# mountaindust/Parasitoids

Hardware: AMD Instinct MI355X
Metric: grid-days/sec on 4096^2 fp64 domain (higher is better)
Workload: dtype f64; 1 GPU; C3 synthetic stack: N=4097 (nominal 4096^2), 30 Gaussian day kernels K=2049, reference torus P=5121, FFT size 5184 (fast mode), prob model, one replica stack per GPU; dom_len=4097, ndays=30, P=5121, fft_len=5184, kernels_direct=False, full_column_pipeline=True

## Files before the change

### include/parasitoid_hip.h

```cpp
#ifndef PARASITOID_HIP_H
#define PARASITOID_HIP_H
#include <stdint.h>

#ifdef __cplusplus
extern "C" {
#endif

#define PS_OK 0
#define PS_ERR_NO_DEVICE (-1)
#define PS_ERR_OOM (-2)
#define PS_ERR_BAD_SHAPE (-3)
#define PS_ERR_BAD_ARG (-4)
#define PS_ERR_UNSUPPORTED (-5)
#define PS_ERR_HIP (-6)
#define PS_ERR_HPROB_BOUNDS (-7)
#define PS_ERR_PMF_NEGATIVE (-8)
#define PS_ERR_FLIGHT_PROB (-9)
#define PS_ERR_STATE (-10)
#define PS_ERR_EMPTY (-11)

#define PS_MODE_EXACT 0
#define PS_MODE_FAST 1
#define PS_MODE_FOLD 2
#define PS_MODE_AUTO 3

typedef struct ps_solver ps_solver;
typedef struct ps_model ps_model;

typedef struct ps_day_stats {
  int64_t nnz;
  double sum;
  double delta;
  double padmax;
  int32_t flag;
  int32_t pad_;
} ps_day_stats;

int ps_version(void);
int ps_device_count(void);
const char* ps_last_error(void);
int ps_device_info(int device, char* name, int n, int* cus, int64_t* hbm_bytes);


int ps_solver_create(ps_solver** out, int device, int dom_len, int max_shape, int mode);
int ps_fast_size(int dom_len, int max_shape);
int ps_solver_retarget(ps_solver* s, int max_shape);
int ps_solver_destroy(ps_solver* s);
int ps_solver_info(ps_solver* s, int* dom_len, int* P, int* Pfft, int* H);
int ps_solver_sync(ps_solver* s);
int ps_solver_set_option(ps_solver* s, const char* key, double value);
int ps_solver_get_option(ps_solver* s, const char* key, double* value);
int ps_solver_kernels_direct(ps_solver* s);
int ps_solver_pipeline(ps_solver* s);
int ps_solver_auto_info(ps_solver* s, int* first_fold_day, int* fold_fft);
int ps_solver_auto_route(ps_solver* s, int first, int count, int32_t* owner);

int ps_solver_set_state_coo(ps_solver* s, const int32_t* row, const int32_t* col,
                            const double* val, int64_t nnz);

int ps_solver_fftconv2_coo(ps_solver* s, const int32_t* row, const int32_t* col,
                           const double* val, int64_t nnz, int kshape);

int ps_solver_get_cursol(ps_solver* s, double negval, double stat_scale, int renorm,
                         ps_day_stats* stats);

int ps_solver_back_solve(ps_solver* s, int nfilt, const int64_t* off, const int32_t* row,
                         const int32_t* col, const double* val, double negval,
                         double stat_scale, ps_day_stats* stats);


int ps_chain_set_kernels(ps_solver* s, int nk, const int64_t* off, const int32_t* kshape,
                         const int32_t* row, const int32_t* col, const double* val);
int ps_chain_run(ps_solver* s, int first, int count, double negval, double stat_scale,
                 int renorm);
int ps_chain_stats(ps_solver* s, int first, int count, ps_day_stats* out);

int ps_chain_run_release(ps_solver* s, int first, int count, double negval, int nfilt, int nuse,
                         const double* weights, int* certified);

int ps_chain_block_prefix(ps_solver* s, int first, int count, const void** total_dev, int64_t* total_bytes);
int ps_chain_block_finish(ps_solver* s, int first, int count, int nprev, const void* const* prev_totals,
                          double negval, double stat_scale, int renorm, int* flagged);
int ps_device_copy(void* dst, const void* src, int64_t bytes);

#define PS_REC_CHAIN 0
#define PS_REC_BACK 1
#define PS_REC_STATE 2
#define PS_REC_WSUM 3
int ps_record_stats(ps_solver* s, int kind, int idx, double negval, double stat_scale,
                    int renorm, ps_day_stats* out);
int ps_record_fetch_coo(ps_solver* s, int kind, int idx, double negval, double stat_scale,
                        double delta, double post_scale, int32_t* row, int32_t* col,
                        double* val, int64_t cap, int64_t* nnz_out);
int ps_record_fetch_csr(ps_solver* s, int kind, int idx, double negval, double stat_scale,
                        double delta, double post_scale, int32_t* indptr ,
                        int32_t* indices, double* data, int64_t cap, int64_t* nnz_out);
int ps_record_fetch_dense(ps_solver* s, int kind, int idx, double* out );
int ps_record_gather(ps_solver* s, int kind, int idx, int64_t n, const int32_t* rows,
                     const int32_t* cols, double scale, double negval, double* out);
int ps_record_gather_multi(ps_solver* s, int nrec, const int32_t* kind, const int32_t* idx, int64_t n,
                           const int32_t* rows, const int32_t* cols, double scale, double negval,
                           double* out);
int ps_weighted_sum(ps_solver* s, int n, const int32_t* kind, const int32_t* idx,
                    const double* w);

#define PS_PROF_NCLS 16
int ps_prof_enable(ps_solver* s, int on);
int ps_prof_read(ps_solver* s, int ncls, double* total_ms, int64_t* count);
int ps_prof_read_days(ps_solver* s, int ncls, int64_t* days);
int ps_prof_read_launches(ps_solver* s, int ncls, int64_t* launches);
int ps_prof_read_owner(ps_solver* s, int owner, int ncls, double* total_ms, int64_t* count, int64_t* launches,
                       int64_t* days);
int ps_solver_owner_fft(ps_solver* s, int owner);

int ps_solver_get_spectrum(ps_solver* s, double* out );
int ps_solver_set_spectrum(ps_solver* s, const double* in );

int ps_model_create(ps_model** out, int device);
int ps_model_destroy(ps_model* m);
int ps_model_set_option(ps_model* m, const char* key, double value);
int ps_model_set_wind(ps_model* m, const double* wind, const int32_t* day_keys, int ndays_wind,
                      int T, int test_run);
int ps_model_prob_mass(ps_model* m, int nd, const int32_t* day_idx, const double* start_time,
                       const double* hparams, const double* Dparams, const double* Dlparams,
                       double mu_r, int n_periods, double rad_dist, int rad_res,
                       int32_t* kshape, int64_t* nnz, int32_t* warned, int32_t* status);
int ps_model_fetch_coo(ps_model* m, int i, int32_t* row, int32_t* col, double* val, int64_t cap);
int ps_model_fetch_debug(ps_model* m, int i, double* hprob, int32_t* Hs, double* loss,
                         double* pmfsum);
int ps_model_hflight(ps_model* m, int day_i, const double* hparams, double* out);
int ps_model_mvn_cdf_values(ps_model* m, double cell, double mu_x, double mu_y, double sig_x,
                            double sig_y, double rho, int32_t* H, double* out, int64_t cap);
int ps_chain_set_kernels_from_model(ps_solver* s, ps_model* m, int first, int count);
int ps_solver_set_state_from_model(ps_solver* s, ps_model* m, int i);

int ps_model_export_device(ps_model* m, int first, int count, void* row_dev, void* col_dev, void* val_dev,
                           int64_t cap);
int ps_chain_set_kernels_device(ps_solver* s, int nk, const int64_t* off, const int32_t* kshape,
                                const void* row_dev, const void* col_dev, const void* val_dev);
int ps_solver_set_state_device(ps_solver* s, const void* row_dev, const void* col_dev, const void* val_dev,
                               int64_t nnz, int kshape);

typedef struct ps_summary ps_summary;
int ps_summary_create(int device, int N, int nslot, int nthr, const double* thr, ps_summary** out);
int ps_summary_add(ps_summary* a, ps_solver* s, int nslot, const int32_t* kind, const int32_t* idx,
                   const double* stat_scale, const double* post_scale, const int32_t* use_delta,
                   double negval, uint32_t weight);
int ps_summary_merge(ps_summary* dst, ps_summary* src);
int ps_summary_info(ps_summary* a, double* total_weight, int64_t* members);
int ps_summary_fetch(ps_summary* a, int slot, int what, double* out );
int ps_summary_reset(ps_summary* a);
int ps_summary_prof(ps_summary* a, int enable, double* total_ms, int64_t* launches);
void ps_summary_destroy(ps_summary* a);

typedef struct ps_linspread ps_linspread;
int ps_linspread_create(int device, int N, int nslot, int nparam, int nthr, const double* thr, ps_linspread** out);
int ps_linspread_set_center(ps_linspread* h, ps_solver* s, int nslot, const int32_t* kind, const int32_t* idx,
                            const double* stat_scale, const double* post_scale, const int32_t* use_delta,
                            double negval);
int ps_linspread_add(ps_linspread* h, ps_solver* s, int param, double coef, int nslot, const int32_t* kind,
                     const int32_t* idx, const double* stat_scale, const double* post_scale,
                     const int32_t* use_delta, double negval);
int ps_linspread_finalize(ps_linspread* h, int nparam, int rank, const double* F);
int ps_linspread_fetch(ps_linspread* h, int slot, int what, double* out );
int ps_linspread_info(ps_linspread* h, int* centered, int* finalized, int64_t* adds);
int ps_linspread_reset(ps_linspread* h);
int ps_linspread_prof(ps_linspread* h, int enable, double* add_ms, int64_t* add_launches, double* fin_ms,
                      int64_t* fin_launches);
void ps_linspread_destroy(ps_linspread* h);

typedef struct ps_hist ps_hist;
int ps_hist_create(int device, int N, int nslot, int nedge, const double* edges, ps_hist** out);
int ps_hist_add(ps_hist* h, ps_solver* s, int nslot, const int32_t* kind, const int32_t* idx,
                const double* stat_scale, const double* post_scale, const int32_t* use_delta, double negval,
                uint32_t weight);
int ps_hist_merge(ps_hist* dst, ps_hist* src);
int ps_hist_info(ps_hist* h, double* total_weight, int64_t* members, int* nedge);
int ps_hist_quantile(ps_hist* h, int slot, double p, double* value, double* lower, double* upper);
int ps_hist_exceed(ps_hist* h, int slot, int k, double* out );
int ps_hist_fetch_counts(ps_hist* h, int slot, int b, uint32_t* out );
int ps_hist_reset(ps_hist* h);
int ps_hist_prof(ps_hist* h, int enable, double* add_ms, int64_t* add_launches, double* q_ms,
                 int64_t* q_launches);
void ps_hist_destroy(ps_hist* h);

typedef struct ps_arrival ps_arrival;
int ps_arrival_create(int device, int N, int nslot, int nthr, const double* thr, ps_arrival** out);
int ps_arrival_add(ps_arrival* a, ps_solver* s, int nslot, const int32_t* kind, const int32_t* idx,
                   const double* stat_scale, const double* post_scale, const int32_t* use_delta, double negval,
                   uint32_t weight);
int ps_arrival_merge(ps_arrival* dst, ps_arrival* src);
int ps_arrival_info(ps_arrival* a, double* total_weight, int64_t* members);
int ps_arrival_prob(ps_arrival* a, int k, int slot, double* out );
int ps_arrival_quantile(ps_arrival* a, int k, double p, int32_t* out );
int ps_arrival_fetch_counts(ps_arrival* a, int k, int slot, uint32_t* out );
int ps_arrival_fetch_reached(ps_arrival* a, int64_t first, int64_t count, uint32_t* cells, uint32_t* weights);
int ps_arrival_reset(ps_arrival* a);
int ps_arrival_prof(ps_arrival* a, int enable, double* add_ms, int64_t* adds, double* map_ms, int64_t* maps);
void ps_arrival_destroy(ps_arrival* a);

#ifdef __cplusplus
}
#endif
#endif
```

### parasitoids_amd/_lib.py

```python
import ctypes as C
import os

import numpy as np

_HERE = os.path.dirname(os.path.abspath(__file__))
LIB_PATH = os.path.join(_HERE, 'libparasitoid_hip.so')

PS_OK = 0
PS_ERR_NO_DEVICE = -1
PS_ERR_OOM = -2
PS_ERR_BAD_SHAPE = -3
PS_ERR_BAD_ARG = -4
PS_ERR_UNSUPPORTED = -5
PS_ERR_HIP = -6
PS_ERR_HPROB_BOUNDS = -7
PS_ERR_PMF_NEGATIVE = -8
PS_ERR_FLIGHT_PROB = -9
PS_ERR_STATE = -10
PS_ERR_EMPTY = -11

MODE_EXACT = 0
MODE_FAST = 1
MODE_FOLD = 2
MODE_AUTO = 3

REC_CHAIN, REC_BACK, REC_STATE, REC_WSUM = 0, 1, 2, 3


class DayStats(C.Structure):
    _fields_ = [('nnz', C.c_int64), ('sum', C.c_double), ('delta', C.c_double),
                ('padmax', C.c_double), ('flag', C.c_int32), ('pad_', C.c_int32)]


class HipError(RuntimeError):
    def __init__(self, code, msg):
        super().__init__('libparasitoid_hip error %d: %s' % (code, msg))
        self.code = code


_I32P = C.POINTER(C.c_int32)
_I64P = C.POINTER(C.c_int64)
_F64P = C.POINTER(C.c_double)
_VP = C.c_void_p

SIGNATURES = {
    'ps_version': (C.c_int, []),
    'ps_device_count': (C.c_int, []),
    'ps_last_error': (C.c_char_p, []),
    'ps_device_info': (C.c_int, [C.c_int, C.c_char_p, C.c_int, _I32P, _I64P]),
    'ps_solver_create': (C.c_int, [C.POINTER(_VP), C.c_int, C.c_int, C.c_int, C.c_int]),
    'ps_solver_destroy': (C.c_int, [_VP]),
    'ps_solver_info': (C.c_int, [_VP, _I32P, _I32P, _I32P, _I32P]),
    'ps_solver_sync': (C.c_int, [_VP]),
    'ps_solver_set_option': (C.c_int, [_VP, C.c_char_p, C.c_double]),
    'ps_solver_get_option': (C.c_int, [_VP, C.c_char_p, _F64P]),
    'ps_solver_set_state_coo': (C.c_int, [_VP, _I32P, _I32P, _F64P, C.c_int64]),
    'ps_solver_fftconv2_coo': (C.c_int, [_VP, _I32P, _I32P, _F64P, C.c_int64, C.c_int]),
    'ps_solver_get_cursol': (C.c_int, [_VP, C.c_double, C.c_double, C.c_int, C.POINTER(DayStats)]),
    'ps_solver_back_solve': (C.c_int, [_VP, C.c_int, _I64P, _I32P, _I32P, _F64P, C.c_double,
                                       C.c_double, C.POINTER(DayStats)]),
    'ps_chain_set_kernels': (C.c_int, [_VP, C.c_int, _I64P, _I32P, _I32P, _I32P, _F64P]),
    'ps_chain_run': (C.c_int, [_VP, C.c_int, C.c_int, C.c_double, C.c_double, C.c_int]),
    'ps_chain_stats': (C.c_int, [_VP, C.c_int, C.c_int, C.POINTER(DayStats)]),
    'ps_chain_run_release': (C.c_int, [_VP, C.c_int, C.c_int, C.c_double, C.c_int, C.c_int, _F64P,
                                       C.POINTER(C.c_int)]),
    'ps_record_stats': (C.c_int, [_VP, C.c_int, C.c_int, C.c_double, C.c_double, C.c_int,
                                  C.POINTER(DayStats)]),
    'ps_solver_retarget': (C.c_int, [_VP, C.c_int]),
    'ps_fast_size': (C.c_int, [C.c_int, C.c_int]),
    'ps_solver_kernels_direct': (C.c_int, [_VP]),
    'ps_solver_pipeline': (C.c_int, [_VP]),
    'ps_solver_auto_info': (C.c_int, [_VP, _I32P, _I32P]),
    'ps_solver_auto_route': (C.c_int, [_VP, C.c_int, C.c_int, _I32P]),
    'ps_record_fetch_coo': (C.c_int, [_VP, C.c_int, C.c_int, C.c_double, C.c_double, C.c_double,
                                      C.c_double, _I32P, _I32P, _F64P, C.c_int64, _I64P]),
    'ps_record_fetch_csr': (C.c_int, [_VP, C.c_int, C.c_int, C.c_double, C.c_double, C.c_double,
                                      C.c_double, _I32P, _I32P, _F64P, C.c_int64, _I64P]),
    'ps_record_fetch_dense': (C.c_int, [_VP, C.c_int, C.c_int, _F64P]),
    'ps_record_gather': (C.c_int, [_VP, C.c_int, C.c_int, C.c_int64, _I32P, _I32P, C.c_double,
                                   C.c_double, _F64P]),
    'ps_record_gather_multi': (C.c_int, [_VP, C.c_int, _I32P, _I32P, C.c_int64, _I32P, _I32P, C.c_double,
                                          C.c_double, _F64P]),
    'ps_weighted_sum': (C.c_int, [_VP, C.c_int, _I32P, _I32P, _F64P]),
    'ps_prof_enable': (C.c_int, [_VP, C.c_int]),
    'ps_prof_read': (C.c_int, [_VP, C.c_int, _F64P, _I64P]),
    'ps_prof_read_days': (C.c_int, [_VP, C.c_int, _I64P]),
    'ps_prof_read_launches': (C.c_int, [_VP, C.c_int, _I64P]),
    'ps_chain_block_prefix': (C.c_int, [_VP, C.c_int, C.c_int, C.POINTER(C.c_void_p), C.POINTER(C.c_int64)]),
    'ps_chain_block_finish': (C.c_int, [_VP, C.c_int, C.c_int, C.c_int, C.POINTER(C.c_void_p), C.c_double, C.c_double,
                                        C.c_int, C.POINTER(C.c_int)]),
    'ps_device_copy': (C.c_int, [C.c_void_p, C.c_void_p, C.c_int64]),
    'ps_prof_read_owner': (C.c_int, [_VP, C.c_int, C.c_int, _F64P, _I64P, _I64P, _I64P]),
    'ps_solver_owner_fft': (C.c_int, [_VP, C.c_int]),
    'ps_solver_get_spectrum': (C.c_int, [_VP, _F64P]),
    'ps_solver_set_spectrum': (C.c_int, [_VP, _F64P]),
    'ps_model_create': (C.c_int, [C.POINTER(_VP), C.c_int]),
    'ps_model_destroy': (C.c_int, [_VP]),
    'ps_model_set_option': (C.c_int, [_VP, C.c_char_p, C.c_double]),
    'ps_model_set_wind': (C.c_int, [_VP, _F64P, _I32P, C.c_int, C.c_int, C.c_int]),
    'ps_model_prob_mass': (C.c_int, [_VP, C.c_int, _I32P, _F64P, _F64P, _F64P, _F64P, C.c_double,
                                     C.c_int, C.c_double, C.c_int, _I32P, _I64P, _I32P, _I32P]),
    'ps_model_fetch_coo': (C.c_int, [_VP, C.c_int, _I32P, _I32P, _F64P, C.c_int64]),
    'ps_model_fetch_debug': (C.c_int, [_VP, C.c_int, _F64P, _I32P, _F64P, _F64P]),
    'ps_model_hflight': (C.c_int, [_VP, C.c_int, _F64P, _F64P]),
    'ps_model_mvn_cdf_values': (C.c_int, [_VP, C.c_double, C.c_double, C.c_double, C.c_double,
                                          C.c_double, C.c_double, _I32P, _F64P, C.c_int64]),
    'ps_chain_set_kernels_from_model': (C.c_int, [_VP, _VP, C.c_int, C.c_int]),
    'ps_solver_set_state_from_model': (C.c_int, [_VP, _VP, C.c_int]),
    'ps_model_export_device': (C.c_int, [_VP, C.c_int, C.c_int, _VP, _VP, _VP, C.c_int64]),
    'ps_chain_set_kernels_device': (C.c_int, [_VP, C.c_int, _I64P, _I32P, _VP, _VP, _VP]),
    'ps_solver_set_state_device': (C.c_int, [_VP, _VP, _VP, _VP, C.c_int64, C.c_int]),
    'ps_summary_create': (C.c_int, [C.c_int, C.c_int, C.c_int, C.c_int, _F64P, C.POINTER(_VP)]),
    'ps_summary_add': (C.c_int, [_VP, _VP, C.c_int, _I32P, _I32P, _F64P, _F64P, _I32P, C.c_double,
                                 C.c_uint32]),
    'ps_summary_merge': (C.c_int, [_VP, _VP]),
    'ps_summary_info': (C.c_int, [_VP, _F64P, _I64P]),
    'ps_summary_fetch': (C.c_int, [_VP, C.c_int, C.c_int, _F64P]),
    'ps_summary_reset': (C.c_int, [_VP]),
    'ps_summary_prof': (C.c_int, [_VP, C.c_int, _F64P, _I64P]),
    'ps_summary_destroy': (None, [_VP]),
    'ps_linspread_create': (C.c_int, [C.c_int, C.c_int, C.c_int, C.c_int, C.c_int, _F64P, C.POINTER(_VP)]),
    'ps_linspread_set_center': (C.c_int, [_VP, _VP, C.c_int, _I32P, _I32P, _F64P, _F64P, _I32P, C.c_double]),
    'ps_linspread_add': (C.c_int, [_VP, _VP, C.c_int, C.c_double, C.c_int, _I32P, _I32P, _F64P, _F64P, _I32P,
                                   C.c_double]),
    'ps_linspread_finalize': (C.c_int, [_VP, C.c_int, C.c_int, _F64P]),
    'ps_linspread_fetch': (C.c_int, [_VP, C.c_int, C.c_int, _F64P]),
    'ps_linspread_info': (C.c_int, [_VP, _I32P, _I32P, _I64P]),
    'ps_linspread_reset': (C.c_int, [_VP]),
    'ps_linspread_prof': (C.c_int, [_VP, C.c_int, _F64P, _I64P, _F64P, _I64P]),
    'ps_linspread_destroy': (None, [_VP]),
    'ps_hist_create': (C.c_int, [C.c_int, C.c_int, C.c_int, C.c_int, _F64P, C.POINTER(_VP)]),
    'ps_hist_add': (C.c_int, [_VP, _VP, C.c_int, _I32P, _I32P, _F64P, _F64P, _I32P, C.c_double, C.c_uint32]),
    'ps_hist_merge': (C.c_int, [_VP, _VP]),
    'ps_hist_info': (C.c_int, [_VP, _F64P, _I64P, _I32P]),
    'ps_hist_quantile': (C.c_int, [_VP, C.c_int, C.c_double, _F64P, _F64P, _F64P]),
    'ps_hist_exceed': (C.c_int, [_VP, C.c_int, C.c_int, _F64P]),
    'ps_hist_fetch_counts': (C.c_int, [_VP, C.c_int, C.c_int, C.POINTER(C.c_uint32)]),
    'ps_hist_reset': (C.c_int, [_VP]),
    'ps_hist_prof': (C.c_int, [_VP, C.c_int, _F64P, _I64P, _F64P, _I64P]),
    'ps_hist_destroy': (None, [_VP]),
    'ps_arrival_create': (C.c_int, [C.c_int, C.c_int, C.c_int, C.c_int, _F64P, C.POINTER(_VP)]),
    'ps_arrival_add': (C.c_int, [_VP, _VP, C.c_int, _I32P, _I32P, _F64P, _F64P, _I32P, C.c_double, C.c_uint32]),
    'ps_arrival_merge': (C.c_int, [_VP, _VP]),
    'ps_arrival_info': (C.c_int, [_VP, _F64P, _I64P]),
    'ps_arrival_prob': (C.c_int, [_VP, C.c_int, C.c_int, _F64P]),
    'ps_arrival_quantile': (C.c_int, [_VP, C.c_int, C.c_double, _I32P]),
    'ps_arrival_fetch_counts': (C.c_int, [_VP, C.c_int, C.c_int, C.POINTER(C.c_uint32)]),
    'ps_arrival_fetch_reached': (C.c_int, [_VP, C.c_int64, C.c_int64, C.POINTER(C.c_uint32),
                                           C.POINTER(C.c_uint32)]),
    'ps_arrival_reset': (C.c_int, [_VP]),
    'ps_arrival_prof': (C.c_int, [_VP, C.c_int, _F64P, _I64P, _F64P, _I64P]),
    'ps_arrival_destroy': (None, [_VP]),
}

_lib = None


def load():
    global _lib
    if _lib is not None:
        return _lib
    if not os.path.exists(LIB_PATH):
        raise ImportError(
            'libparasitoid_hip.so not found at %s; build it with '
            '`python -c "import __graft_entry__ as g; g.build()"` or '
            '`make -C parasitoids_amd/csrc`' % LIB_PATH)
    try:
        lib = C.CDLL(LIB_PATH)
    except OSError as e:
        raise ImportError('cannot load %s: %s' % (LIB_PATH, e))
    for name, (res, args) in SIGNATURES.items():
        fn = getattr(lib, name)
        fn.restype = res
        fn.argtypes = args
    _lib = lib
    return lib


def check(rc):
    if rc != PS_OK:
        msg = load().ps_last_error()
        raise HipError(rc, msg.decode() if msg else '')


def require_device():
    lib = load()
    n = lib.ps_device_count()
    if n <= 0:
        msg = lib.ps_last_error()
        raise ImportError('no MI355X/HIP device available: %s' % (msg.decode() if msg else ''))
    return n


def default_device():
    return int(os.environ.get('PARASITOID_DEVICE', os.environ.get('LOCAL_RANK', '0')))


def i32(a):
    return np.ascontiguousarray(a, dtype=np.int32)


def f64(a):
    return np.ascontiguousarray(a, dtype=np.float64)


def p_i32(a):
    return a.ctypes.data_as(_I32P)


def p_i64(a):
    return a.ctypes.data_as(_I64P)


def p_f64(a):
    return a.ctypes.data_as(_F64P)
```

### parasitoids_amd/csrc/chain_kernels.h

```cpp
#pragma once
#include <hip/hip_runtime.h>
#include <stdint.h>

static __global__ void k_scatter_coo(const int* __restrict__ row, const int* __restrict__ col,
                              const double* __restrict__ val, int64_t nnz, double* dst, int ld,
                              int roff, int coff) {
  for (int64_t i = blockIdx.x * (int64_t)blockDim.x + threadIdx.x; i < nnz;
       i += (int64_t)gridDim.x * blockDim.x)
    atomicAdd(&dst[(int64_t)(row[i] + roff) * ld + col[i] + coff], val[i]);
}

static __global__ void k_zero_band(double* dst, int K, int r0, int r1) {
  double* base = dst + (int64_t)blockIdx.y * K * K + (int64_t)r0 * K;
  const int64_t n = (int64_t)(r1 - r0 + 1) * K;
  for (int64_t i = blockIdx.x * (int64_t)blockDim.x + threadIdx.x; i < n; i += (int64_t)gridDim.x * blockDim.x)
    base[i] = 0.0;
}

static __global__ void k_scatter_coo_batch(const int* __restrict__ row, const int* __restrict__ col,
                                           const double* __restrict__ val, const long long* __restrict__ koff,
                                           const int* __restrict__ kshape, int first, double* dst, int K) {
  const int d = first + blockIdx.y;
  const long long lo = koff[d], hi = koff[d + 1];
  const int off = K / 2 - kshape[d] / 2;
  double* out = dst + (int64_t)blockIdx.y * K * K;
  for (long long i = lo + blockIdx.x * (long long)blockDim.x + threadIdx.x; i < hi;
       i += (long long)gridDim.x * blockDim.x)
    atomicAdd(&out[(int64_t)(row[i] + off) * K + col[i] + off], val[i]);
}

struct DayStats {
  long long nnz;
  double sum;
  double delta;
  double padmax;
  int flag;
  int pad_;
};

static __global__ void k_day_finalize(const double* rowsum_, const long long* rowcnt_,
                               const unsigned long long* padmax_, int N, int renorm,
                               DayStats* out_) {
  const double* rowsum = rowsum_ + (int64_t)blockIdx.x * N;
  const long long* rowcnt = rowcnt_ + (int64_t)blockIdx.x * N;
  const unsigned long long* padmax = padmax_ + blockIdx.x;
  DayStats* out = out_ + blockIdx.x;
  __shared__ double ssum[256];
  __shared__ long long scnt[256];
  double s = 0.0;
  long long c = 0;
  for (int r = threadIdx.x; r < N; r += blockDim.x) {
    s += rowsum[r];
    c += rowcnt[r];
  }
  ssum[threadIdx.x] = s;
  scnt[threadIdx.x] = c;
  __syncthreads();
  for (int off = blockDim.x / 2; off > 0; off >>= 1) {
    if ((int)threadIdx.x < off) {
      ssum[threadIdx.x] += ssum[threadIdx.x + off];
      scnt[threadIdx.x] += scnt[threadIdx.x + off];
    }
    __syncthreads();
  }
  if (threadIdx.x == 0) {
    DayStats d;
    d.nnz = scnt[0];
    d.sum = ssum[0];
    d.delta = (renorm && scnt[0] > 0) ? (1.0 - ssum[0]) / (double)scnt[0] : 0.0;
    d.padmax = __longlong_as_double((long long)*padmax);
    d.flag = d.padmax > 1e-8 ? 1 : 0;
    d.pad_ = 0;
    *out = d;
  }
}

static __global__ void k_row_stats(const double* __restrict__ rec, int N, double scale, double negval,
                            double* rowsum, long long* rowcnt) {
  __shared__ double ssum[256];
  __shared__ int scnt[256];
  const int r = blockIdx.x;
  double s = 0.0;
  int c = 0;
  for (int i = threadIdx.x; i < N; i += blockDim.x) {
    const double t = rec[(int64_t)r * N + i] * scale;
    if (t != 0.0 && !(t < negval)) { s += t; ++c; }
  }
  ssum[threadIdx.x] = s;
  scnt[threadIdx.x] = c;
  __syncthreads();
  for (int off = blockDim.x / 2; off > 0; off >>= 1) {
    if ((int)threadIdx.x < off) {
      ssum[threadIdx.x] += ssum[threadIdx.x + off];
      scnt[threadIdx.x] += scnt[threadIdx.x + off];
    }
    __syncthreads();
  }
  if (threadIdx.x == 0) { rowsum[r] = ssum[0]; rowcnt[r] = scnt[0]; }
}

static __global__ void k_fold(const double* __restrict__ lin, int M, int P, int N, int m, double* torus,
                              double* rec, double negval, double stat_scale, double* rowsum,
                              long long* rowcnt, unsigned long long* padmax) {
  const int r = blockIdx.x;
  int yr[3], nr = 0;
  yr[nr++] = r;
  if (r < m) yr[nr++] = r + P;
  if (r >= P - m) yr[nr++] = r - P + M;
  __shared__ double ssum[256];
  __shared__ long long scnt[256];
  __shared__ double smax[256];
  double s = 0.0, pm = 0.0;
  long long cnt = 0;
  for (int c = threadIdx.x; c < P; c += blockDim.x) {
    int yc[3], nc = 0;
    yc[nc++] = c;
    if (c < m) yc[nc++] = c + P;
    if (c >= P - m) yc[nc++] = c - P + M;
    double v = 0.0;
    for (int i = 0; i < nr; ++i)
      for (int j = 0; j < nc; ++j) v += lin[(int64_t)yr[i] * M + yc[j]];
    torus[(int64_t)r * P + c] = v;
    if (r < N && c < N) {
      rec[(int64_t)r * N + c] = v;
      const double t = v * stat_scale;
      if (!(t < negval)) { s += t; ++cnt; }
    } else {
      pm = fmax(pm, v);
    }
  }
  ssum[threadIdx.x] = s;
  scnt[threadIdx.x] = cnt;
  smax[threadIdx.x] = pm;
  __syncthreads();
  for (int off = blockDim.x / 2; off > 0; off >>= 1) {
    if ((int)threadIdx.x < off) {
      ssum[threadIdx.x] += ssum[threadIdx.x + off];
      scnt[threadIdx.x] += scnt[threadIdx.x + off];
      smax[threadIdx.x] = fmax(smax[threadIdx.x], smax[threadIdx.x + off]);
    }
    __syncthreads();
  }
  if (threadIdx.x == 0) {
    if (r < N) { rowsum[r] = ssum[0]; rowcnt[r] = scnt[0]; }
    const double mx = smax[0];
    const unsigned long long bits = (unsigned long long)__double_as_longlong(mx);
    if (mx > 0.0 && bits > __hip_atomic_load(padmax, __ATOMIC_RELAXED, __HIP_MEMORY_SCOPE_AGENT))
      atomicMax(padmax, bits);
  }
}

static __global__ void k_truncate_if_flag(double* torus, int P, int N, const unsigned long long* padmax) {
  if (!(__longlong_as_double((long long)*padmax) > 1e-8)) return;
  const int r = blockIdx.x;
  for (int c = threadIdx.x; c < P; c += blockDim.x)
    if (r >= N || c >= N) torus[(int64_t)r * P + c] = 0.0;
}

static __global__ void k_scan_rows(const long long* rowcnt_, int N, long long* rowoff_) {
  const long long* rowcnt = rowcnt_ + (int64_t)blockIdx.x * N;
  long long* rowoff = rowoff_ + (int64_t)blockIdx.x * N;
  __shared__ long long part[1024];
  const int T = blockDim.x;
  const int per = (N + T - 1) / T;
  const int lo = threadIdx.x * per, hi = min(N, lo + per);
// ... 121 lines not shown
```

### parasitoids_amd/csrc/ps_config.h

```cpp
#pragma once
#include <cstdlib>
#include <cstring>

#define PS_OPTION_TABLE(X)                                                                          \
                                               \
  X("PS_NO_RS", no_rs, 0, FLAG, C)                                                                  \
  X("PS_NO_RS_FWD", no_rs_fwd, 0, FLAG, C)                                                          \
  X("PS_NO_BIG_RADIX", no_big_radix, 0, FLAG, C)                                                    \
  X("PS_NO_TPIPE", no_tpipe, 0, FLAG, C)                                                            \
  X("PS_NO_FOLD_TPIPE", no_fold_tpipe, 0, FLAG, C)                                                  \
  X("PS_COL_SINGLE_MAX", col_single_max, 1200, INT, C)                                              \
  X("PS_COL_L1", col_l1, 0, INT, C)                                                                 \
  X("PS_CHUNK_DAYS", chunk_days, 0, INT, C)                                                         \
  X("PS_FAST_SIZE", fast_size, 0, INT, C)                                                           \
  X("PS_RS_AREA", rs_area, 0.0, NUM, C)                                                             \
                                                                                 \
  X("PS_COL_WSH", col_wsh, -1, INT, R)                                                              \
  X("PS_COL_THREADS", col_threads, 256, INT, R)                                                     \
  X("PS_FUSED_WSH", fused_wsh, -1, INT, R)                                                          \
  X("PS_FUSED_THREADS", fused_threads, 0, INT, R)                                                   \
  X("PS_FUSED_G", fused_g, 2, INT, R)                                                               \
  X("PS_MULTI_WSH", multi_wsh, -1, INT, R)                                                          \
  X("PS_DUAL_WSH", dual_wsh, -1, INT, R)                                                            \
  X("PS_FUSED_DAYS", fused_days, 8, INT, R)                                                         \
  X("PS_DIRECT_DAYS", direct_days, 4, INT, R)                                                       \
  X("PS_DIRECT_MAX_TERMS", direct_max_terms, 8, INT, R)                                             \
  X("PS_TPIPE_DAYS", tpipe_days, 32, INT, R)                                                        \
  X("PS_DUAL_MIN_DAYS", dual_min_days, 6, INT, R)                                                   \
                                                   \
  X("PS_TINV", tinv, 0, INT, R)                                                                     \
  X("PS_RSP", rsp, -1, INT, R)                                                                      \
  X("PS_ROW2", row2, -1, INT, R)                                                                    \
  X("PS_TPIPE", tpipe, -1, INT, R)                                                                  \
  X("PS_NO_PAIR_ROWS", no_pair_rows, 0, FLAG, R)                                                    \
  X("PS_TPIPE_SPLIT", tpipe_split, 0, INT, R)                                                       \
  X("PS_NO_CONJ", no_conj, 0, FLAG, R)                                                              \
  X("PS_NO_DUAL", no_dual, 0, FLAG, R)                                                              \
  X("PS_NO_DIRECT", no_direct, 0, FLAG, R)                                                          \
  X("PS_NO_ROW_BATCH", no_row_batch, 0, FLAG, R)                                                    \
  X("PS_NO_PAD_QUIET", no_pad_quiet, 0, FLAG, R)                                                    \
  X("PS_NO_TAIL_SPLIT", no_tail_split, 0, FLAG, R)                                                  \
  X("PS_NO_DEFER_REFFT", no_defer_refft, 0, FLAG, R)                                                \
  X("PS_NO_FILTER_CACHE", no_filter_cache, 0, FLAG, R)                                              \
  X("PS_NO_FOLD_FUSE", no_fold_fuse, 0, FLAG, R)                                                    \
  X("PS_NO_FOLD_ALT", no_fold_alt, 0, FLAG, R)                                                      \
  X("PS_NO_FOLD_ROWS", no_fold_rows, 0, FLAG, R)                                                    \
                                                                                 \
  X("PS_NO_SPECULATION", no_speculation, 0, FLAG, R)                                                \
  X("PS_SPEC_DEPTH", spec_depth, 2, INT, R)                                                         \
  X("PS_NO_FLAG_HISTORY", no_flag_history, 0, FLAG, R)                                              \
  X("PS_NO_WINDOW_HINT", no_window_hint, 0, FLAG, R)                                                \
  X("PS_FIRST_WINDOW", first_window, -1, INT, R)                                                    \
  X("PS_KT_SPLIT", kt_split, -1, INT, R)                                                            \
  X("PS_NO_LAZY_KT", no_lazy_kt, 0, FLAG, R)                                                        \
  X("PS_NO_WIDE", no_wide, 0, FLAG, R)                                                              \
  X("PS_NO_ROUTE_HISTORY", no_route_history, 0, FLAG, R)                                            \
  X("PS_WIDE_MIN_N", wide_min_n, 1500, INT, R)                                                      \
  X("PS_AUTO_WINDOW", auto_window, 4, INT, R)                                                       \
                                                                  \
  X("PS_PM_SEG", pm_seg, 8, INT, R)                                                                 \
  X("PS_PM_SYNC", pm_sync, 0, FLAG, R)                                                              \
  X("PS_PM_NO_UNROLL", pm_no_unroll, 0, FLAG, R)

struct ps_config {
#define PS_CFG_FIELD_FLAG int
#define PS_CFG_FIELD_INT int
#define PS_CFG_FIELD_NUM double
#define X(key, field, dflt, kind, when) PS_CFG_FIELD_##kind field = dflt;
  PS_OPTION_TABLE(X)
#undef X
};

inline void ps_config_from_env(ps_config* c) {
  *c = ps_config();
#define PS_CFG_ENV_FLAG(field) c->field = (e[0] == '\0' || std::strcmp(e, "0") != 0) ? 1 : 0
#define PS_CFG_ENV_INT(field) c->field = std::atoi(e)
#define PS_CFG_ENV_NUM(field) c->field = std::atof(e)
#define X(key, field, dflt, kind, when) \
  if (const char* e = std::getenv(key)) { PS_CFG_ENV_##kind(field); }
  PS_OPTION_TABLE(X)
#undef X
}

inline int ps_config_set(ps_config* c, const char* key, double value, bool live) {
  if (!key) return -1;
#define PS_CFG_SET_FLAG(field) c->field = value != 0.0 ? 1 : 0
#define PS_CFG_SET_INT(field) c->field = (int)value
#define PS_CFG_SET_NUM(field) c->field = value
#define PS_CFG_WHEN_C true
#define PS_CFG_WHEN_R false
#define X(k, field, dflt, kind, when)         \
  if (std::strcmp(key, k) == 0) {             \
    if (live && PS_CFG_WHEN_##when) return -2; \
    PS_CFG_SET_##kind(field);                 \
    return 0;                                 \
  }
  PS_OPTION_TABLE(X)
#undef X
  return -1;
}

inline int ps_config_get(const ps_config* c, const char* key, double* value) {
  if (!key || !value) return -1;
#define X(k, field, dflt, kind, when) \
  if (std::strcmp(key, k) == 0) {     \
    *value = (double)c->field;        \
    return 0;                         \
  }
  PS_OPTION_TABLE(X)
#undef X
  return -1;
}
```

### parasitoids_amd/csrc/ps_solver.hip

```cpp
#include <deque>

#include "chain_kernels.h"
#include "fft_kernels.h"
#include "fft_colfull_kernels.h"
#include "rs_launch.h"
#include "ps_common.h"
#include "ps_config.h"

thread_local std::string ps_tls_error;

extern "C" const char* ps_last_error(void) { return ps_tls_error.c_str(); }
extern "C" int ps_version(void) { return 100; }

extern "C" int ps_device_count(void) {
  int n = 0;
  hipError_t e = hipGetDeviceCount(&n);
  if (e != hipSuccess) return ps_fail(PS_ERR_NO_DEVICE, "hipGetDeviceCount: %s", hipGetErrorString(e));
  return n;
}

extern "C" int ps_device_info(int device, char* name, int n, int* cus, int64_t* hbm_bytes) {
  hipDeviceProp_t p;
  PS_HIP(hipGetDeviceProperties(&p, device));
  if (name && n > 0) snprintf(name, n, "%s (%s)", p.name, p.gcnArchName);
  if (cus) *cus = p.multiProcessorCount;
  if (hbm_bytes) *hbm_bytes = (int64_t)p.totalGlobalMem;
  return PS_OK;
}

int ps_use_device(int device) {
  int n = 0;
  hipError_t e = hipGetDeviceCount(&n);
  if (e != hipSuccess || n <= 0)
    return ps_fail(PS_ERR_NO_DEVICE, "no HIP device available (%s)", hipGetErrorString(e));
  if (device < 0 || device >= n) return ps_fail(PS_ERR_NO_DEVICE, "device %d out of range (%d devices)", device, n);
  PS_HIP(hipSetDevice(device));
  return PS_OK;
}

static const int kMaxLds = 160 * 1024;

#include <map>
#include <mutex>
#include <unordered_map>
namespace {
struct DevPool {
  std::mutex mu;
  std::map<int, std::multimap<size_t, void*>> free_;
  std::unordered_map<void*, std::pair<int, size_t>> live;
  size_t cached = 0;
  size_t limit() {
    static const size_t gb = getenv("PS_POOL_GB") ? (size_t)atoi(getenv("PS_POOL_GB")) : 16;
    return gb << 30;
  }
  void flush_locked() {
    for (auto& dv : free_)
      for (auto& kv : dv.second) (void)hipFree(kv.second);
    free_.clear();
    cached = 0;
  }
};
DevPool& pool() {
  static DevPool* p = new DevPool();
  return *p;
}
size_t round_size(size_t b) {
  const size_t g = b >= (1u << 20) ? (size_t)1 << 20 : 256;
  return (b + g - 1) / g * g;
}
}

static hipError_t poison(void* p, size_t n) {
  static const bool on = getenv("PS_POISON") != nullptr;
  if (!on) return hipSuccess;
  hipError_t e = hipMemset(p, 0xFF, n);
  if (e == hipSuccess) e = hipDeviceSynchronize();
  return e;
}

hipError_t ps_dev_malloc(void** out, size_t bytes) {
  DevPool& P = pool();
  int dev = 0;
  (void)hipGetDevice(&dev);
  const size_t want = round_size(bytes ? bytes : 1);
  std::lock_guard<std::mutex> lk(P.mu);
  auto& fr = P.free_[dev];
  auto it = fr.lower_bound(want);
  if (it != fr.end() && it->first <= want + want / 4 + (1u << 20)) {
    *out = it->second;
    P.live[*out] = {dev, it->first};
    P.cached -= it->first;
    const size_t got = it->first;
    fr.erase(it);
    return poison(*out, got);
  }
  hipError_t e = hipMalloc(out, want);
  if (e != hipSuccess) {
    (void)hipGetLastError();
    P.flush_locked();
    e = hipMalloc(out, want);
  }
  if (e == hipSuccess) {
    P.live[*out] = {dev, want};
    e = poison(*out, want);
  }
  return e;
}

void ps_dev_free(void* p) {
  if (!p) return;
  DevPool& P = pool();
  std::lock_guard<std::mutex> lk(P.mu);
  auto it = P.live.find(p);
  if (it == P.live.end()) {
    (void)hipFree(p);
    return;
  }
  const int dev = it->second.first;
  const size_t sz = it->second.second;
  P.live.erase(it);
  if (P.cached + sz > P.limit()) {
    (void)hipFree(p);
    return;
  }
  P.free_[dev].emplace(sz, p);
  P.cached += sz;
}

void ps_dev_quiesce() { (void)hipDeviceSynchronize(); }
static const int kPredGrid = 512;
static const double kCleanEps = 1e-15;
#define PS_PROF_NCLS 16
enum { PS_PROF_ROW_FWD = 0, PS_PROF_COL_FWD_A = 1, PS_PROF_COL_FWD_B = 2, PS_PROF_COL_INV_A = 3,
       PS_PROF_COL_INV_B = 4, PS_PROF_ROW_INV = 5, PS_PROF_REFFT = 6, PS_PROF_COL_INV_A2 = 7,
       PS_PROF_COL_INV_A4 = 8, PS_PROF_COL_INV_A8 = 9, PS_PROF_ROW_INV2 = 10, PS_PROF_ROW_INV4 = 11,
       PS_PROF_ROW_INV8 = 12,
       PS_PROF_COL_INV_AN = 13,
       PS_PROF_ROW_INVN = 14,
       PS_PROF_COL_TAIL = 15 };
#define PS_MAX_GROUP_DAYS 32

struct ColPass {
  DevPlan* plan;
  int n_outer, in_base_mul, in_stride, out_base_mul, out_stride, tw_mode;
  bool second = false;
};

struct ps_solver {
  int device = 0;
  hipStream_t stream = nullptr;
  int N = 0, M = 0, Pref = 0, Pf = 0, H = 0, ld = 0, mode = 0;
  DevPlan row_plan, col_plan1, col_plan2;
  bool split = false;
  bool tpipe = false;
  bool tpipe_ok = false;
  bool tinv = false;
  ps_config cfg;
  bool spec_valid = false;
  bool row_big = false;
  int num_cu = 256;
  bool speculate = true;
  int fused_days = 8;
  int spec_window = 1;
  hipEvent_t spec_ev[2] = {nullptr, nullptr};
  hipStream_t stream2 = nullptr;
  hipEvent_t kt_ev = nullptr, kt_ev0 = nullptr;
  int kt_from = -1;
  int kt_lazy_from = -1, kt_lazy_c0 = 0, kt_lazy_cn = 0, kt_lazy_direct = 0;
  unsigned long long* hflags = nullptr;
  int hflags_n = 0;
  unsigned long long* hhist = nullptr;
  int hhist_n = 0, hist_first = -1, hist_count = 0;
  hipEvent_t hist_ev = nullptr;
  int rs_r2 = 0, rs_r3 = 0;
  int L1 = 0, L2 = 0;
  DevBuf<cplx> tp_lo, tp_hi;
  int tp_shift = 0;
  std::vector<ColPass> fwd_passes, inv_passes;
  DevBuf<cplx> Ahat, Chat, T1, T2, Bhat;
  int chunk_days = 1;
  DevBuf<int> srange;
  bool srange_valid = false;
  DevBuf<int> krow, kcol;
  DevBuf<double> kval;
  std::vector<int64_t> koff;
  std::vector<int> kshape;
  int nk = 0, Kmax = 0;
  bool kernels_on_device = false;
  DevBuf<double> kdense;
  DevBuf<long long> dkoff;
  DevBuf<int> dkshape;
  int bhat_first = -1, bhat_count = 0;
  std::vector<double*> recs[4];
  DevBuf<double> rowsum;
  DevBuf<long long> rowcnt;
  DevBuf<long long> rowoff;
  DevBuf<unsigned long long> padmax;
  DevBuf<DayStats> dstats;
  int nstat = 0;
  int last_renorm = 0;
  RowLive kt_live{0, {0, 0, 0, 0}, nullptr};
  bool kt_direct = false;
  DevBuf<int> krange;
  std::vector<int> hkrange;
  DevBuf<int> orow, ocol;
  DevBuf<double> oval;
  DevBuf<const double*> wptr;
  DevBuf<double> wval;
  bool have_state = false;
  bool auto_exact = false;
  double pad_floor = 0.5e-8;
  ps_solver* child = nullptr;
  ps_solver* wide = nullptr;
  ps_solver* narrow = nullptr;
  bool narrow_kernels = false;
  bool borrowed = false;
  bool child_kernels = false, wide_kernels = false;
  std::vector<signed char> owner;
  std::vector<signed char> route_hist;
  int route_first = -1, route_end = -1;
  int auto_first_regime = 2;
  int auto_first = -1;
  int auto_hint = -1;
  int noflag_hint = 0;
  long long auto_runs = 0;
  struct FiltKey { uint64_t h1, h2; int64_t n; };
  std::vector<FiltKey> filt_keys;
  DevBuf<cplx> Fhat;
  long long filt_hits = 0, filt_misses = 0;
  DevBuf<double> torus, lin, fold_rowsum;
  DevBuf<long long> fold_rowcnt;
  DevBuf<unsigned long long> fold_padmax;
  DevBuf<double> pad_energy;
  DevBuf<int> pad_quiet;
  DevBuf<cplx> tail_hat;
  DevBuf<cplx> Trow;
  DevBuf<cplx> blk;
  int blk_first = -1, blk_count = 0;
  DevBuf<unsigned long long> one_flag;
  const unsigned long long* refft_pending = nullptr;
  int ncu = 0;
  bool prof_on = false;
  struct ProfRec { int cls; hipEvent_t a, b; int days; };
  std::vector<ProfRec> prof_pending;
  std::vector<hipEvent_t> prof_pool;
  double prof_ms[PS_PROF_NCLS] = {0};
  long long prof_cnt[PS_PROF_NCLS] = {0};
  long long prof_seen[PS_PROF_NCLS] = {0};
  long long prof_days[PS_PROF_NCLS] = {0};
  int prof_every = 1;
};

static hipEvent_t prof_event(ps_solver* s) {
  if (!s->prof_pool.empty()) {
    hipEvent_t e = s->prof_pool.back();
    s->prof_pool.pop_back();
    return e;
  }
  hipEvent_t e = nullptr;
  (void)hipEventCreateWithFlags(&e, hipEventDisableSystemFence);
  return e;
}
struct ProfScope {
  ps_solver* s;
  ps_solver::ProfRec r;
  bool on;
  ProfScope(ps_solver* s_, int cls, int days = 1) : s(s_), on(false) {
    r.days = days;
    if (!s->prof_on) return;
    on = cls >= PS_PROF_COL_INV_A2 || (s->prof_seen[cls]++ % s->prof_every) == 0;
    if (!on) return;
    r.cls = cls;
    r.a = prof_event(s);
    r.b = prof_event(s);
    (void)hipEventRecord(r.a, s->stream);
  }
  ~ProfScope() {
    if (!on) return;
    (void)hipEventRecord(r.b, s->stream);
    s->prof_pending.push_back(r);
  }
};

static int row_threads(int L, bool big = false) { return L <= 1024 ? 256 : ((L <= 2560 || big) ? 512 : 1024); }
static int row_pairs(const FftProg& P) {
  int rp = 2048 / std::max(1, P.L);
  rp = std::max(1, std::min(8, rp));
  return rp;
}
static int col_wsh(const ps_solver* s, int L) {
  int w = 4096 / std::max(1, L);
  int sh = 2;
  while ((1 << (sh + 1)) <= w && sh < 5) ++sh;
  if (s->cfg.col_wsh >= 0) sh = s->cfg.col_wsh;
  return sh;
}
static int col_threads(const ps_solver* s) { return s->cfg.col_threads; }

static int set_lds_attr() {
  static bool done = false;
  if (done) return PS_OK;
  const void* ks[] = {(const void*)k_row_fwd<false, false>, (const void*)k_row_fwd<true, false>,
                      (const void*)k_row_fwd<false, true>,
                      (const void*)k_row_inv<false, false>, (const void*)k_row_inv<true, false>,
                      (const void*)k_row_inv<false, true>,
                      (const void*)k_col<PS_FWD, false>, (const void*)k_col<PS_FWD, true>,
                      (const void*)k_col<PS_INV, false>, (const void*)k_col<PS_INV, true>,
                      (const void*)k_col_fused<false>, (const void*)k_col_fused<true>,
                      (const void*)k_col_fused_dual<false>, (const void*)k_col_fused_dual<true>,
#define PS_MULTI_K(ND) \
  (const void*)k_col_fused_multi<false, ND, 1>, (const void*)k_col_fused_multi<true, ND, 1>, \
  (const void*)k_col_fused_multi<false, ND, 2>, (const void*)k_col_fused_multi<true, ND, 2>
                      PS_MULTI_K(1), PS_MULTI_K(2), PS_MULTI_K(4), PS_MULTI_K(8)};
#undef PS_MULTI_K
  for (const void* k : ks) PS_HIP(hipFuncSetAttribute(k, hipFuncAttributeMaxDynamicSharedMemorySize, kMaxLds));
  if (rs_rows_set_attrs() != 0 || rs_colfull_set_attrs() != 0 || rs_coldual_set_attrs() != 0) return ps_fail(PS_ERR_HIP, "hipFuncSetAttribute failed for a register-resident kernel");
  done = true;
  return PS_OK;
}

static int launch_row_fwd(ps_solver* s, const double* src, int64_t src_bstride, int src_ld,
                          SrcMap rmap, SrcMap cmap, cplx* dst, int batch,
                          const unsigned long long* pred, int skip_zero = 0, const int* rowrange = nullptr,
                          const unsigned long long* trunc_pred = nullptr, int trunc_n = 0) {
  RowFwdArgs a;
  if (trunc_pred && s->rs_r2 == 0) return ps_fail(PS_ERR_STATE, "row pass: only the register-resident kernels truncate on the fly");
  a.trunc_pred = trunc_pred; a.trunc_n = trunc_n;
  a.src = src; a.src_bstride = src_bstride; a.src_ld = src_ld;
  a.rmap = rmap; a.cmap = cmap;
  a.dst = dst; a.dst_bstride = (int64_t)s->Pf * s->ld;
  a.H = s->H; a.ld = s->ld; a.P = s->Pf;
  a.tstride = s->tpipe ? s->Pf : 0;
  a.prog = s->row_plan.prog;
  a.rp = row_pairs(a.prog);
  a.pred = pred;
  a.skip_zero = skip_zero;
  a.rowrange = rowrange;
  const int npairs = (s->Pf + 1) / 2;
  a.nblocks = (npairs + a.rp - 1) / a.rp;
  dim3 grid(pred ? std::min(a.nblocks, kPredGrid) : a.nblocks, batch);
  const int thr = row_threads(a.prog.L, s->row_big);
  const size_t lds = ((size_t)a.rp * row_pitch(a.prog) + a.prog.n_lo + a.prog.n_hi + a.prog.n_gen) * sizeof(cplx);
  if (lds > (size_t)kMaxLds) return ps_fail(PS_ERR_UNSUPPORTED, "row pass needs %zu B LDS", lds);
  ProfScope prof(s, pred ? PS_PROF_REFFT : PS_PROF_ROW_FWD);
  if (s->rs_r2 != 0 && !s->cfg.no_rs_fwd) {
    if (!rs_launch_row_fwd(s->rs_r2, s->rs_r3, a, npairs, batch, s->stream))
      return ps_fail(PS_ERR_STATE, "no register-resident row kernel for 16 x %d x %d", s->rs_r2, s->rs_r3);
  } else if (s->row_plan.generic)
    hipLaunchKernelGGL((k_row_fwd<true, false>), grid, dim3(thr), lds, s->stream, a);
  else if (s->row_big)
    hipLaunchKernelGGL((k_row_fwd<false, true>), grid, dim3(thr), lds, s->stream, a);
  else
    hipLaunchKernelGGL((k_row_fwd<false, false>), grid, dim3(thr), lds, s->stream, a);
  PS_HIP(hipGetLastError());
  return PS_OK;
}

template <int DIR>
static int launch_col(ps_solver* s, const ColPass& cp, const cplx* src, const cplx* src2,
                      cplx* prod, cplx* dst, int batch, int64_t src2_bstride,
                      const unsigned long long* pred, RowLive live = RowLive{0, {0, 0, 0, 0}, nullptr}) {
  ColArgs a;
  a.src = src; a.src2 = src2; a.prod_dst = prod; a.dst = dst;
  const int64_t bs = (int64_t)s->Pf * s->ld;
  a.src_bstride = bs; a.src2_bstride = src2_bstride; a.prod_bstride = bs; a.dst_bstride = bs;
  a.ld = s->ld; a.ncols = s->H;
  a.prog = cp.plan->prog;
  a.wsh = col_wsh(s, a.prog.L);
  a.n_outer = cp.n_outer;
  a.in_base_mul = cp.in_base_mul; a.in_stride = cp.in_stride;
  a.out_base_mul = cp.out_base_mul; a.out_stride = cp.out_stride;
  a.tw_mode = cp.tw_mode;
  a.tp_lo = s->tp_lo.p; a.tp_hi = s->tp_hi.p; a.tp_shift = s->tp_shift;
  a.pred = pred;
  a.live = live;
  const int W = 1 << a.wsh;
  const int ntiles = (s->H + W - 1) / W;
  dim3 grid((unsigned)(ntiles * cp.n_outer), batch);
  size_t lds = (((size_t)a.prog.L << a.wsh) + a.prog.n_lo + a.prog.n_hi + a.prog.n_gen + a.prog.L) * sizeof(cplx) + (size_t)a.prog.L * sizeof(int);
  while (lds > (size_t)kMaxLds && a.wsh > 0) {
    --a.wsh;
    lds = (((size_t)a.prog.L << a.wsh) + a.prog.n_lo + a.prog.n_hi + a.prog.n_gen + a.prog.L) * sizeof(cplx) + (size_t)a.prog.L * sizeof(int);
  }
  if (lds > (size_t)kMaxLds) return ps_fail(PS_ERR_UNSUPPORTED, "column pass needs %zu B LDS", lds);
  {
    const int W2 = 1 << a.wsh;
    a.nblocks = ((s->H + W2 - 1) / W2) * cp.n_outer;
    grid.x = (unsigned)(pred ? std::min(a.nblocks, kPredGrid) : a.nblocks);
  }
  ProfScope prof(s, pred ? PS_PROF_REFFT
                          : (DIR == PS_FWD ? PS_PROF_COL_FWD_A : PS_PROF_COL_INV_A) + (cp.second ? 1 : 0));
  if (cp.plan->generic)
    hipLaunchKernelGGL((k_col<DIR, true>), grid, dim3(col_threads(s)), lds, s->stream, a);
  else
    hipLaunchKernelGGL((k_col<DIR, false>), grid, dim3(col_threads(s)), lds, s->stream, a);
  PS_HIP(hipGetLastError());
  return PS_OK;
}

static bool row_inv_persistent(const ps_solver* s) {
  const int knob = s->cfg.rsp;
  RsInfo info;
  if (s->rs_r2 == 0 || !rs_info(s->rs_r2, s->rs_r3, &info) || !info.rsp || knob == 0) return false;
  return knob == 1 || (s->tpipe && s->Pf >= 1536);
}

static int inter_layout(const ps_solver* s) {
  if (!s->tpipe) return 0;
  if (s->tinv) return 1;
  return (s->mode != PS_MODE_FOLD && !s->cfg.no_pair_rows && s->Pf % 2 == 0) ? 2 : 0;
}

static int launch_row_inv(ps_solver* s, const cplx* src, double* rec, int stat_slot, int batch,
                          double negval, double stat_scale, bool full_field = false,
                          double* const* recs_multi = nullptr, const int* pad_quiet = nullptr) {
  RowInvArgs a;
  a.pad_quiet = pad_quiet;
  a.persistent = (row_inv_persistent(s) && !(s->tpipe && s->tinv && !full_field)) ? 1 : 0;
  if (a.persistent && (s->cfg.row2 > 0 || (s->cfg.row2 < 0 && s->Pf >= 4096))) a.persistent = 2;
  a.nrec = 0;
  for (int i = 0; i < PS_MAX_GROUP_DAYS; ++i) a.rec_multi[i] = nullptr;
  if (recs_multi) {
    if (!a.persistent || batch > PS_MAX_GROUP_DAYS) return ps_fail(PS_ERR_STATE, "row pass: a record table needs the persistent kernel and at most %d entries", PS_MAX_GROUP_DAYS);
    a.nrec = batch;
    for (int i = 0; i < batch; ++i) a.rec_multi[i] = recs_multi[i];
  }
  a.src = src; a.src_bstride = (int64_t)s->Pf * s->ld;
  a.H = s->H; a.ld = s->ld; a.P = s->Pf; a.N = s->N;
  a.tstride = (s->tpipe && s->tinv && !full_field) ? s->Pf : 0;
  a.pair_src = (!full_field && inter_layout(s) == 2) ? 1 : 0;
  a.prog = s->row_plan.prog;
  a.rp = row_pairs(a.prog);
  a.scale = 1.0 / ((double)s->Pf * (double)s->Pf);
  a.rec = rec; a.rec_bstride = (int64_t)s->N * s->N;
  a.negval = negval; a.stat_scale = stat_scale;
  a.rowsum = s->rowsum.p + (int64_t)stat_slot * s->N;
// ... 414 lines not shown
}

static int refft_rows_if_flag(ps_solver* s, const double* rec, int slot) {
  PS_TRY(s->Trow.ensure((size_t)s->Pf * s->ld));
  const SrcMap m = map_plain(s->N, s->Pf);
  PS_TRY(launch_row_fwd(s, rec, 0, s->N, m, m, s->Trow.p, 1, s->padmax.p + slot, 1, nullptr));
  s->refft_pending = s->padmax.p + slot;
  return PS_OK;
}
static int resolve_refft(ps_solver* s) {
  if (!s->refft_pending) return PS_OK;
  const unsigned long long* pred = s->refft_pending;
  s->refft_pending = nullptr;
  return launch_colfull(s, 1, s->Trow.p, s->Ahat.p, 0, nullptr, 1, RowLive{1, map_plain(s->N, s->Pf), nullptr}, pred);
}

static int fast_size(const ps_config& cfg, int Pref) {
  if (cfg.fast_size >= Pref) return cfg.fast_size;
  int Pf = ps_next_fast_len(Pref);
  if (!cfg.no_rs) {
    const int L = rs_next_size(Pref);
    const double area = cfg.rs_area > 0.0 ? cfg.rs_area : (Pf < 2048 ? 1.2 : 1.08);
    if (L > 0 && ((double)L * L <= area * (double)Pf * Pf || Pf > 9700)) Pf = L;
  }
  return Pf;
}

extern "C" int ps_fast_size(int dom_len, int max_shape) {
  if (dom_len < 1 || max_shape < 1) return 0;
  ps_config cfg;
  ps_config_from_env(&cfg);
  return fast_size(cfg, dom_len + max_shape / 2);
}

static int solver_create(ps_solver** out, int device, int dom_len, int max_shape, int mode, const ps_config& cfg);

extern "C" int ps_solver_create(ps_solver** out, int device, int dom_len, int max_shape, int mode) {
  ps_config cfg;
  ps_config_from_env(&cfg);
  return solver_create(out, device, dom_len, max_shape, mode, cfg);
}

static int solver_create(ps_solver** out, int device, int dom_len, int max_shape, int mode, const ps_config& cfg) {
  if (!out) return ps_fail(PS_ERR_BAD_ARG, "null output handle");
  *out = nullptr;
  if (dom_len < 1 || max_shape < 1) return ps_fail(PS_ERR_BAD_SHAPE, "dom_len=%d max_shape=%d", dom_len, max_shape);
  if (mode != PS_MODE_EXACT && mode != PS_MODE_FAST && mode != PS_MODE_FOLD && mode != PS_MODE_AUTO)
    return ps_fail(PS_ERR_BAD_ARG, "mode %d", mode);
  const bool auto_exact = mode == PS_MODE_AUTO;
  if (auto_exact) mode = PS_MODE_FAST;
  PS_TRY(ps_use_device(device));
  PS_TRY(set_lds_attr());
  ps_solver* s = new ps_solver();
  s->cfg = cfg;
  s->tinv = cfg.tinv != 0;
  s->fused_days = cfg.fused_days;
  s->device = device;
  s->N = dom_len;
  s->M = max_shape / 2;
  s->Pref = dom_len + s->M;
  s->mode = mode;
  s->auto_exact = auto_exact;
  if (auto_exact) s->pad_floor = 0.5 * kCleanEps;
  s->Pf = mode == PS_MODE_FAST ? fast_size(cfg, s->Pref) : s->Pref;
  if (mode == PS_MODE_FOLD) s->Pf = fast_size(cfg, s->Pref + 2 * s->M);
  s->H = s->Pf / 2 + 1;
  s->ld = (s->H + 7) & ~7;
  auto fail = [&](int rc) {
    ps_solver_destroy(s);
    return rc;
  };
  {
    HostFftPlan small, big;
    const bool ok_s = ps_build_plan(s->Pf, true, &small), ok_b = ps_build_plan(s->Pf, true, &big, true);
    if (ok_s && ok_b && small.max_prime <= 9 && s->Pf > 1024 && big.prog.ns < small.prog.ns &&
        !cfg.no_big_radix) {
      s->row_plan.host = big;
      s->row_big = true;
    }
  }
  if (!s->row_big && !ps_build_plan(s->Pf, true, &s->row_plan.host))
    return fail(ps_fail(PS_ERR_UNSUPPORTED, "cannot plan a length-%d FFT (prime factor > %d); use PS_MODE_FAST",
                        s->Pf, PS_MAX_GENERIC_RADIX));
  {
    int r2 = 0, r3 = 0;
    const bool rs = !cfg.no_rs && rs_lookup(s->Pf, &r2, &r3);
    if (!rs && (size_t)(row_pitch(s->row_plan.host.prog) + 512) * sizeof(cplx) > (size_t)kMaxLds)
      return fail(ps_fail(PS_ERR_UNSUPPORTED, "pad size %d exceeds the LDS-resident row limit", s->Pf));
  }
  int rc = s->row_plan.upload();
  if (rc) return fail(rc);
  if (cfg.no_rs || !rs_lookup(s->Pf, &s->rs_r2, &s->rs_r3)) s->rs_r2 = s->rs_r3 = 0;
  s->tpipe_ok = (mode == PS_MODE_FAST || mode == PS_MODE_FOLD) && s->rs_r2 != 0 && !cfg.no_rs &&
                !cfg.no_rs_fwd && !cfg.no_tpipe;
  if (mode == PS_MODE_FOLD && cfg.no_fold_tpipe) s->tpipe_ok = false;
  s->tpipe = s->tpipe_ok;
  {
    int ncu = 0;
    if (hipDeviceGetAttribute(&ncu, hipDeviceAttributeMultiprocessorCount, device) == hipSuccess && ncu > 0) s->num_cu = ncu;
  }
  {
    s->L1 = ps_choose_col_split(s->Pf, cfg.col_single_max);
  }
  if (cfg.col_l1 > 1 && cfg.col_l1 < s->Pf && s->Pf % cfg.col_l1 == 0) s->L1 = cfg.col_l1;
  s->split = s->L1 != s->Pf;
  if (s->split) {
    s->L2 = s->Pf / s->L1;
    if (!ps_build_plan(s->L1, false, &s->col_plan1.host) || !ps_build_plan(s->L2, false, &s->col_plan2.host))
      return fail(ps_fail(PS_ERR_UNSUPPORTED, "cannot plan column FFT %d = %d x %d", s->Pf, s->L1, s->L2));
    if ((rc = s->col_plan1.upload())) return fail(rc);
    if ((rc = s->col_plan2.upload())) return fail(rc);
    s->fwd_passes = {ColPass{&s->col_plan1, s->L2, 1, s->L2, 1, s->L2, 1},
                     ColPass{&s->col_plan2, s->L1, s->L2, 1, 1, s->L1, 0, true}};
    s->inv_passes = {ColPass{&s->col_plan2, s->L1, 1, s->L1, s->L2, 1, 0},
                     ColPass{&s->col_plan1, s->L2, 1, s->L2, 1, s->L2, 2, true}};
  } else {
    s->L2 = 1;
    if (!ps_build_plan(s->Pf, false, &s->col_plan1.host))
      return fail(ps_fail(PS_ERR_UNSUPPORTED, "cannot plan column FFT %d", s->Pf));
    if ((rc = s->col_plan1.upload())) return fail(rc);
    s->fwd_passes = {ColPass{&s->col_plan1, 1, 0, 1, 0, 1, 0}};
    s->inv_passes = {ColPass{&s->col_plan1, 1, 0, 1, 0, 1, 0}};
  }
  {
    HostTwiddle tw;
    ps_build_twiddle(s->Pf, &tw);
    s->tp_shift = tw.shift;
    if ((rc = s->tp_lo.ensure(tw.lo.size()))) return fail(rc);
    if ((rc = s->tp_hi.ensure(tw.hi.size()))) return fail(rc);
    hipError_t e1 = hipMemcpy(s->tp_lo.p, tw.lo.data(), tw.lo.size() * sizeof(cplx), hipMemcpyHostToDevice);
    hipError_t e2 = hipMemcpy(s->tp_hi.p, tw.hi.data(), tw.hi.size() * sizeof(cplx), hipMemcpyHostToDevice);
    if (e1 != hipSuccess || e2 != hipSuccess) return fail(ps_fail(PS_ERR_HIP, "twiddle upload failed"));
  }
  hipError_t e = hipStreamCreateWithFlags(&s->stream, hipStreamNonBlocking);
  if (e != hipSuccess) return fail(ps_fail(PS_ERR_HIP, "hipStreamCreate: %s", hipGetErrorString(e)));
  const size_t spec = (size_t)s->Pf * s->ld;
  size_t budget = (size_t)3 << 30;
  {
    size_t mfree = 0, mtotal = 0;
    if (hipMemGetInfo(&mfree, &mtotal) == hipSuccess && mtotal / 16 > budget) budget = mtotal / 16;
  }
  s->chunk_days = (int)std::max<size_t>(1, std::min<size_t>(64, budget / (spec * sizeof(cplx))));
  if (cfg.chunk_days > 0) s->chunk_days = cfg.chunk_days;
  if ((rc = s->Ahat.ensure(spec))) return fail(rc);
  if ((rc = s->rowoff.ensure(s->N))) return fail(rc);
  if ((rc = ensure_stats(s, 4))) return fail(rc);
  *out = s;
  return PS_OK;
}

extern "C" int ps_solver_destroy(ps_solver* s) {
  if (!s) return PS_OK;
  (void)hipSetDevice(s->device);
  if (s->stream) (void)hipStreamSynchronize(s->stream);
  if (s->child) {
    ps_solver_destroy(s->child);
    s->child = nullptr;
  }
  if (s->wide) {
    ps_solver_destroy(s->wide);
    s->wide = nullptr;
  }
  if (s->narrow) {
    ps_solver_destroy(s->narrow);
    s->narrow = nullptr;
  }
  if (s->borrowed) {
    s->stream = nullptr;
    for (auto& p : s->recs[PS_REC_CHAIN]) p = nullptr;
  }
  if (s->stream2) {
    (void)hipStreamSynchronize(s->stream2);
    (void)hipStreamDestroy(s->stream2);
  }
  if (s->kt_ev) (void)hipEventDestroy(s->kt_ev);
  if (s->kt_ev0) (void)hipEventDestroy(s->kt_ev0);
  if (s->stream) (void)hipStreamDestroy(s->stream);
  ps_dev_quiesce();
  s->row_plan.release(); s->col_plan1.release(); s->col_plan2.release();
  s->tp_lo.release(); s->tp_hi.release();
  s->Ahat.release(); s->Chat.release(); s->T1.release(); s->T2.release(); s->Bhat.release(); s->Fhat.release();
  s->Trow.release(); s->blk.release(); s->one_flag.release(); s->tail_hat.release(); s->pad_energy.release(); s->pad_quiet.release();
  s->srange.release();
  s->krow.release(); s->kcol.release(); s->kval.release(); s->kdense.release(); s->krange.release();
  for (auto& v : s->recs)
    for (double* p : v)
      if (p) ps_dev_free(p);
  s->rowsum.release(); s->rowcnt.release(); s->rowoff.release(); s->padmax.release();
  s->dstats.release();
  s->orow.release(); s->ocol.release(); s->oval.release(); s->wptr.release(); s->wval.release();
  for (auto& r : s->prof_pending) { (void)hipEventDestroy(r.a); (void)hipEventDestroy(r.b); }
  for (auto e : s->prof_pool) (void)hipEventDestroy(e);
  for (auto e : s->spec_ev) if (e) (void)hipEventDestroy(e);
  if (s->hflags) (void)hipHostFree(s->hflags);
  if (s->hhist) (void)hipHostFree(s->hhist);
  if (s->hist_ev) (void)hipEventDestroy(s->hist_ev);
  s->dkoff.release(); s->dkshape.release();
  s->torus.release(); s->lin.release(); s->fold_rowsum.release(); s->fold_rowcnt.release(); s->fold_padmax.release();
  delete s;
  return PS_OK;
}

extern "C" int ps_solver_retarget(ps_solver* s, int max_shape) {
  if (!s || max_shape < 1) return ps_fail(PS_ERR_BAD_ARG, "retarget: bad arguments");
  if (s->auto_exact) {
    const int m = max_shape / 2;
    if (s->N + m > s->Pf)
      return ps_fail(PS_ERR_BAD_SHAPE, "retarget: max_shape %d needs an FFT size >= %d, the solver has %d", max_shape,
                     s->N + m, s->Pf);
    PS_HIP(hipSetDevice(s->device));
    PS_HIP(hipStreamSynchronize(s->stream));
    if (s->child && ps_solver_retarget(s->child, max_shape) != PS_OK) {
      ps_solver_destroy(s->child);
      s->child = nullptr;
    }
    if (s->wide) {
      ps_solver_destroy(s->wide);
      s->wide = nullptr;
    }
    if (s->narrow) {
      ps_solver_destroy(s->narrow);
      s->narrow = nullptr;
    }
    s->narrow_kernels = false;
    s->child_kernels = false;
    s->wide_kernels = false;
    s->route_first = s->route_end = -1;
    s->M = m;
    s->Pref = s->N + m;
    s->have_state = false;
    s->bhat_first = -1;
    s->bhat_count = 0;
    return PS_OK;
  }
  if (s->mode != PS_MODE_FOLD) return ps_fail(PS_ERR_UNSUPPORTED, "retarget: only PS_MODE_FOLD solvers can change their torus");
  const int m = max_shape / 2;
  if (s->N + 3 * m > s->Pf)
    return ps_fail(PS_ERR_BAD_SHAPE, "retarget: max_shape %d needs an FFT size >= %d, the solver has %d", max_shape,
                   s->N + 3 * m, s->Pf);
  PS_HIP(hipSetDevice(s->device));
  PS_HIP(hipStreamSynchronize(s->stream));
  s->M = m;
  s->Pref = s->N + m;
  s->have_state = false;
  s->bhat_first = -1;
  s->bhat_count = 0;
  return PS_OK;
}

extern "C" int ps_solver_info(ps_solver* s, int* dom_len, int* P, int* Pfft, int* H) {
  if (!s) return ps_fail(PS_ERR_BAD_ARG, "null solver");
  if (dom_len) *dom_len = s->N;
  if (P) *P = s->Pref;
  if (Pfft) *Pfft = s->Pf;
  if (H) *H = s->H;
  return PS_OK;
}

extern "C" int ps_solver_sync(ps_solver* s) {
  if (!s) return ps_fail(PS_ERR_BAD_ARG, "null solver");
  PS_HIP(hipSetDevice(s->device));
  PS_HIP(hipStreamSynchronize(s->stream));
  return PS_OK;
}

static int ensure_temps(ps_solver* s, int batch) {
  const size_t spec = (size_t)s->Pf * s->ld;
  PS_TRY(s->T1.ensure(spec * batch));
  if (s->split) PS_TRY(s->T2.ensure(spec * batch));
  return PS_OK;
}

static int check_coo(const int32_t* row, const int32_t* col, int64_t nnz, int lim, const char* what) {
  for (int64_t i = 0; i < nnz; ++i)
    if (row[i] < 0 || row[i] >= lim || col[i] < 0 || col[i] >= lim)
      return ps_fail(PS_ERR_BAD_SHAPE, "%s: entry %lld (%d,%d) outside %d x %d", what, (long long)i, row[i],
                     col[i], lim, lim);
  return PS_OK;
}

static int scatter_from_device(ps_solver* s, const int* row, const int* col, const double* val,
                               int64_t nnz, double* dst, int ld, int off) {
  if (nnz <= 0) return PS_OK;
  const int thr = 256;
  const int blocks = (int)std::min<int64_t>((nnz + thr - 1) / thr, 4096);
  hipLaunchKernelGGL(k_scatter_coo, dim3(blocks), dim3(thr), 0, s->stream, row, col, val, nnz, dst, ld, off, off);
  PS_HIP(hipGetLastError());
  return PS_OK;
}

static int upload_coo(ps_solver* s, const int32_t* row, const int32_t* col, const double* val, int64_t nnz) {
  PS_TRY(s->orow.ensure(std::max<int64_t>(nnz, 1)));
  PS_TRY(s->ocol.ensure(std::max<int64_t>(nnz, 1)));
  PS_TRY(s->oval.ensure(std::max<int64_t>(nnz, 1)));
  if (nnz > 0) {
    PS_HIP(hipMemcpyAsync(s->orow.p, row, nnz * 4, hipMemcpyHostToDevice, s->stream));
    PS_HIP(hipMemcpyAsync(s->ocol.p, col, nnz * 4, hipMemcpyHostToDevice, s->stream));
    PS_HIP(hipMemcpyAsync(s->oval.p, val, nnz * 8, hipMemcpyHostToDevice, s->stream));
    PS_HIP(hipStreamSynchronize(s->stream));
  }
  return PS_OK;
}

int ps_solver_set_state_device_coo(ps_solver* s, const int* row, const int* col, const double* val,
                                   int64_t nnz, int off) {
  PS_TRY(ensure_record(s, PS_REC_STATE, 0));
  PS_TRY(ensure_temps(s, 1));
  s->srange_valid = false;
  double* rec = s->recs[PS_REC_STATE][0];
  PS_HIP(hipMemsetAsync(rec, 0, (size_t)s->N * s->N * sizeof(double), s->stream));
  PS_TRY(scatter_from_device(s, row, col, val, nnz, rec, s->N, off));
  if (s->mode == PS_MODE_FOLD) {
    PS_TRY(s->torus.ensure((size_t)s->Pref * s->Pref));
    PS_HIP(hipMemsetAsync(s->torus.p, 0, (size_t)s->Pref * s->Pref * sizeof(double), s->stream));
    PS_HIP(hipMemcpy2DAsync(s->torus.p, (size_t)s->Pref * sizeof(double), rec, (size_t)s->N * sizeof(double),
                            (size_t)s->N * sizeof(double), (size_t)s->N, hipMemcpyDeviceToDevice, s->stream));
    s->have_state = true;
    return PS_OK;
  }
  s->spec_valid = false;
  s->have_state = true;
  return PS_OK;
}

static int ensure_spectrum(ps_solver* s) {
  if (s->spec_valid || s->mode == PS_MODE_FOLD) return PS_OK;
  if (s->recs[PS_REC_STATE].empty() || !s->recs[PS_REC_STATE][0]) return ps_fail(PS_ERR_STATE, "no state record");
  PS_TRY(ensure_temps(s, 1));
  PS_TRY(fwd2d(s, s->recs[PS_REC_STATE][0], 0, s->N, map_plain(s->N, s->Pf), map_plain(s->N, s->Pf), s->Ahat.p, 1, nullptr,
               s->srange_valid ? s->srange.p : nullptr));
  s->spec_valid = true;
  return PS_OK;
}

static void set_pipeline(ps_solver* s, bool tpipe) {
  if (!s->tpipe_ok) tpipe = false;
  if (s->tpipe == tpipe) return;
  s->tpipe = tpipe;
  s->bhat_first = -1;
  s->bhat_count = 0;
  s->filt_keys.clear();
}

extern "C" int ps_solver_set_state_coo(ps_solver* s, const int32_t* row, const int32_t* col,
                                       const double* val, int64_t nnz) {
  if (!s || nnz < 0 || (nnz > 0 && (!row || !col || !val))) return ps_fail(PS_ERR_BAD_ARG, "set_state_coo: bad arguments");
  PS_HIP(hipSetDevice(s->device));
  PS_TRY(check_coo(row, col, nnz, s->N, "state"));
  PS_TRY(upload_coo(s, row, col, val, nnz));
  PS_TRY(ps_solver_set_state_device_coo(s, s->orow.p, s->ocol.p, s->oval.p, nnz, 0));
  int range[2] = {1, 0};
  for (int64_t i = 0; i < nnz; ++i) {
    if (range[0] > range[1]) range[0] = range[1] = row[i];
    range[0] = std::min(range[0], (int)row[i]);
    range[1] = std::max(range[1], (int)row[i]);
  }
  PS_TRY(s->srange.ensure(2));
  hipLaunchKernelGGL(k_set_int2, dim3(1), dim3(64), 0, s->stream, s->srange.p, range[0], range[1]);
  PS_HIP(hipGetLastError());
  s->srange_valid = true;
  return PS_OK;
}

static bool direct_possible(const ps_solver* s) {
  return s->split && s->mode != PS_MODE_FOLD && !s->cfg.no_direct &&
         s->L1 <= 255 && s->L2 <= 255;
}
static bool day_is_compact(const ps_solver* s, int d) {
  const int max_terms = s->cfg.direct_max_terms;
  const int M = s->Kmax / 2;
  const int lo = s->hkrange[2 * d], hi = s->hkrange[2 * d + 1];
  if (lo > hi) return true;
  const int below = std::max(0, std::min(hi, M - 1) - lo + 1), above = std::max(0, hi - std::max(lo, M) + 1);
  const int terms = (below + s->L2 - 1) / s->L2 + (above + s->L2 - 1) / s->L2;
  return terms <= max_terms;
}

static int transform_kernels(ps_solver* s, int first, int count, int slot0, int total, int direct_chunk) {
  const int K = s->Kmax, M = K / 2;
  const size_t spec = (size_t)s->Pf * s->ld;
  if (total < 0) total = count;
  PS_TRY(s->kdense.ensure((size_t)total * K * K));
  PS_TRY(s->Bhat.ensure(spec * total));
  PS_TRY(ensure_temps(s, total));
  double* kd = s->kdense.p + (size_t)slot0 * K * K;
  int blo = K, bhi = -1;
  int64_t maxn = 0;
  for (int d = first; d < first + count; ++d) {
    if (s->hkrange[2 * d] <= s->hkrange[2 * d + 1]) {
      blo = std::min(blo, s->hkrange[2 * d]);
      bhi = std::max(bhi, s->hkrange[2 * d + 1]);
    }
    maxn = std::max<int64_t>(maxn, s->koff[d + 1] - s->koff[d]);
  }
  if (bhi >= blo) {
    blo = std::max(blo, 0);
    bhi = std::min(bhi, K - 1);
    const int64_t n = (int64_t)(bhi - blo + 1) * K;
    const int blocks = (int)std::min<int64_t>((n + 255) / 256, 2048);
    hipLaunchKernelGGL(k_zero_band, dim3(blocks, count), dim3(256), 0, s->stream, kd, K, blo, bhi);
    PS_HIP(hipGetLastError());
  }
  if (maxn > 0) {
    const int thr = 256;
    const int blocks = (int)std::min<int64_t>((maxn + thr - 1) / thr, 1024);
    hipLaunchKernelGGL(k_scatter_coo_batch, dim3(blocks, count), dim3(thr), 0, s->stream, s->krow.p, s->kcol.p,
                       s->kval.p, s->dkoff.p, s->dkshape.p, first, kd, K);
    PS_HIP(hipGetLastError());
  }
  bool direct = direct_possible(s);
  if (direct_chunk >= 0) direct = direct && direct_chunk != 0;
  else for (int d = first; d < first + count && direct; ++d) direct = day_is_compact(s, d);
  PS_TRY(fwd2d_partial(s, kd, (int64_t)K * K, K, map_wrap(M, s->Pf), map_wrap(M, s->Pf), s->Bhat.p + (size_t)slot0 * spec, count,
                       s->krange.p + 2 * first, direct));
  s->bhat_first = first - slot0;
  s->bhat_count = slot0 + count;
  return PS_OK;
}

static int transform_kernels(ps_solver* s, int first, int count, int slot0 = 0, int total = -1, int direct_chunk = -1);
static int kernels_ready(ps_solver* s, int d) {
  if (s->kt_lazy_from >= 0 && d >= s->kt_lazy_from) {
    const int from = s->kt_lazy_from, done = from - s->kt_lazy_c0;
    s->kt_lazy_from = -1;
    PS_TRY(transform_kernels(s, from, s->kt_lazy_cn - done, done, s->kt_lazy_cn, s->kt_lazy_direct));
  }
  if (s->kt_from >= 0 && d >= s->kt_from) {
    PS_HIP(hipStreamWaitEvent(s->stream, s->kt_ev, 0));
    s->kt_from = -1;
  }
  return PS_OK;
}

static int drain_kernel_readers(ps_solver* s) {
  if (s->stream2) PS_HIP(hipStreamSynchronize(s->stream2));
  PS_HIP(hipStreamSynchronize(s->stream));
  return PS_OK;
}

static int set_kernels_common(ps_solver* s, int nk, const int64_t* off, const int32_t* kshape,
                              const int32_t* rows) {
  s->koff.assign(off, off + nk + 1);
  s->kshape.assign(kshape, kshape + nk);
  s->nk = nk;
  s->Kmax = 1;
  for (int d = 0; d < nk; ++d) {
    if (kshape[d] < 1 || kshape[d] % 2 == 0)
      return ps_fail(PS_ERR_BAD_SHAPE, "kernel %d has even/invalid shape %d (CalcSol.py:58)", d, kshape[d]);
    if (kshape[d] / 2 > s->M)
      return ps_fail(PS_ERR_BAD_SHAPE, "kernel %d shape %d exceeds max_shape %d", d, kshape[d], 2 * s->M + 1);
    s->Kmax = std::max(s->Kmax, kshape[d]);
  }
  if (2 * (s->Kmax / 2) + 1 > s->Pf) return ps_fail(PS_ERR_BAD_SHAPE, "kernel larger than the pad");
  s->hkrange.assign(2 * (size_t)std::max(nk, 1), 0);
  const int M = s->Kmax / 2;
  for (int d = 0; d < nk; ++d) {
    const int o = M - kshape[d] / 2;
    int lo = 0, hi = kshape[d] - 1;
    if (rows && off[d + 1] > off[d]) {
      lo = kshape[d];
      hi = -1;
      for (int64_t i = off[d]; i < off[d + 1]; ++i) {
        lo = std::min(lo, (int)rows[i]);
        hi = std::max(hi, (int)rows[i]);
      }
    } else if (rows) {
      lo = 1;
      hi = 0;
    }
    s->hkrange[2 * d] = lo + o;
    s->hkrange[2 * d + 1] = hi + o;
  }
  PS_TRY(s->krange.ensure(s->hkrange.size()));
  PS_TRY(s->dkoff.ensure((size_t)nk + 1));
  PS_TRY(s->dkshape.ensure((size_t)std::max(nk, 1)));
  {
    std::vector<long long> o64(off, off + nk + 1);
    PS_HIP(hipMemcpy(s->dkoff.p, o64.data(), o64.size() * sizeof(long long), hipMemcpyHostToDevice));
    if (nk > 0) PS_HIP(hipMemcpy(s->dkshape.p, kshape, (size_t)nk * sizeof(int), hipMemcpyHostToDevice));
  }
  PS_HIP(hipMemcpyAsync(s->krange.p, s->hkrange.data(), s->hkrange.size() * sizeof(int), hipMemcpyHostToDevice, s->stream));
  PS_HIP(hipStreamSynchronize(s->stream));
  s->bhat_first = -1;
  s->bhat_count = 0;
  s->kernels_on_device = true;
  s->child_kernels = false;
  s->wide_kernels = false;
  s->narrow_kernels = false;
  return PS_OK;
}

extern "C" int ps_chain_set_kernels(ps_solver* s, int nk, const int64_t* off, const int32_t* kshape,
                                    const int32_t* row, const int32_t* col, const double* val) {
  if (!s || nk < 0 || !off || (nk > 0 && !kshape)) return ps_fail(PS_ERR_BAD_ARG, "set_kernels: bad arguments");
  PS_HIP(hipSetDevice(s->device));
  const int64_t tot = off[nk];
  for (int d = 0; d < nk; ++d) {
    if (off[d + 1] < off[d]) return ps_fail(PS_ERR_BAD_ARG, "offsets not monotone");
    PS_TRY(check_coo(row + off[d], col + off[d], off[d + 1] - off[d], kshape[d], "kernel"));
  }
  PS_TRY(drain_kernel_readers(s));
  PS_TRY(s->krow.ensure(std::max<int64_t>(tot, 1)));
  PS_TRY(s->kcol.ensure(std::max<int64_t>(tot, 1)));
  PS_TRY(s->kval.ensure(std::max<int64_t>(tot, 1)));
  if (tot > 0) {
    PS_HIP(hipMemcpyAsync(s->krow.p, row, tot * 4, hipMemcpyHostToDevice, s->stream));
    PS_HIP(hipMemcpyAsync(s->kcol.p, col, tot * 4, hipMemcpyHostToDevice, s->stream));
    PS_HIP(hipMemcpyAsync(s->kval.p, val, tot * 8, hipMemcpyHostToDevice, s->stream));
    PS_HIP(hipStreamSynchronize(s->stream));
  }
  return set_kernels_common(s, nk, off, kshape, row);
}

int ps_chain_adopt_device_kernels(ps_solver* s, int nk, const int64_t* off, const int32_t* kshape,
                                  const int* row, const int* col, const double* val) {
  const int64_t tot = off[nk];
  PS_TRY(drain_kernel_readers(s));
  PS_TRY(s->krow.ensure(std::max<int64_t>(tot, 1)));
  PS_TRY(s->kcol.ensure(std::max<int64_t>(tot, 1)));
  PS_TRY(s->kval.ensure(std::max<int64_t>(tot, 1)));
  if (tot > 0) {
    PS_HIP(hipMemcpyAsync(s->krow.p, row, tot * 4, hipMemcpyDeviceToDevice, s->stream));
    PS_HIP(hipMemcpyAsync(s->kcol.p, col, tot * 4, hipMemcpyDeviceToDevice, s->stream));
    PS_HIP(hipMemcpyAsync(s->kval.p, val, tot * 8, hipMemcpyDeviceToDevice, s->stream));
  }
  return set_kernels_common(s, nk, off, kshape, nullptr);
}

static int auto_attach(ps_solver* s, ps_solver** slot, int mode, int max_shape, bool* kernels_ok, int end) {
  if (!*slot) {
    ps_solver* c = nullptr;
    PS_TRY(solver_create(&c, s->device, s->N, max_shape, mode, s->cfg));
    (void)hipStreamSynchronize(c->stream);
    (void)hipStreamDestroy(c->stream);
    c->stream = s->stream;
    c->borrowed = true;
    c->speculate = false;
    c->pad_floor = 0.5 * kCleanEps;
    c->prof_on = s->prof_on;
    c->prof_every = s->prof_every;
    *slot = c;
    *kernels_ok = false;
  }
  ps_solver* c = *slot;
  if (!*kernels_ok) {
    PS_TRY(ps_chain_adopt_device_kernels(c, s->nk, s->koff.data(), s->kshape.data(), s->krow.p, s->kcol.p, s->kval.p));
    c->hkrange = s->hkrange;
    PS_HIP(hipMemcpyAsync(c->krange.p, c->hkrange.data(), c->hkrange.size() * sizeof(int), hipMemcpyHostToDevice, c->stream));
    PS_HIP(hipStreamSynchronize(c->stream));
    *kernels_ok = true;
  }
  PS_TRY(ensure_stats(c, std::max(4, end)));
  return PS_OK;
}

static const double* auto_prev_field(ps_solver* s, int first, int d) {
  if (d > 0 && d - 1 < (int)s->recs[PS_REC_CHAIN].size() && s->recs[PS_REC_CHAIN][d - 1] && (d > first || first > 0))
    return s->recs[PS_REC_CHAIN][d - 1];
  if (d == first && first == 0 && !s->recs[PS_REC_STATE].empty()) return s->recs[PS_REC_STATE][0];
  return nullptr;
}

static int auto_alias_records(ps_solver* s, ps_solver* c, int lo, int hi) {
  auto& cr = c->recs[PS_REC_CHAIN];
  if ((int)cr.size() < hi) cr.resize(hi, nullptr);
  for (int d = lo; d < hi; ++d) {
    PS_TRY(ensure_record(s, PS_REC_CHAIN, d));
    cr[d] = s->recs[PS_REC_CHAIN][d];
  }
  return PS_OK;
}

static int auto_read_padmax(ps_solver* s, ps_solver* c, int d, int w, double* out) {
  if (s->hflags_n < d + w) {
    if (s->hflags) (void)hipHostFree(s->hflags);
    s->hflags = nullptr;
    s->hflags_n = 0;
    PS_HIP(hipHostMalloc((void**)&s->hflags, (size_t)(d + w + 64) * sizeof(unsigned long long), hipHostMallocDefault));
    s->hflags_n = d + w + 64;
  }
  PS_HIP(hipMemcpyAsync(s->hflags + d, c->padmax.p + d, (size_t)w * sizeof(unsigned long long), hipMemcpyDeviceToHost, s->stream));
  PS_HIP(hipStreamSynchronize(s->stream));
  for (int i = 0; i < w; ++i) __builtin_memcpy(&out[i], &s->hflags[d + i], sizeof(double));
  return PS_OK;
}

static int auto_handover(ps_solver* s, int first, int f, int end, double negval, double stat_scale, int renorm,
                         double m_front) {
  const int wide_min_n = s->cfg.wide_min_n;
  const bool no_wide = s->cfg.no_wide || s->N < wide_min_n;
  const int kWin = std::min(64, std::max(1, s->cfg.auto_window));
  std::vector<signed char> hist;
  if (!s->cfg.no_route_history && s->route_first == first && s->route_end == end) hist = s->route_hist;
  if ((int)s->owner.size() < end) s->owner.resize(end, 0);
  for (int d = first; d < f; ++d) s->owner[d] = 0;
  enum { WIDE = 1, CHILD = 2, NARROW = 3 };
  std::vector<signed char> hint((size_t)end, 0);
  auto hist_owner = [&](int q) { return q >= 0 && q < (int)hist.size() && q < end ? (int)hist[q] : -1; };
  auto stretch = [&](int q, int who) {
    int e = q;
    while (e < end && e - q < 64 && hist_owner(e) == who) ++e;
    return e - q;
  };
  int regime = (no_wide || !(m_front > 1e-8)) ? CHILD : WIDE;
  s->auto_first_regime = regime;
  bool wide_live = false, child_live = false, narrow_live = false;
  int no_narrow_day = -1;
  int d = f;
  while (d < end) {
    const double* prev = auto_prev_field(s, first, d);
    if (regime == NARROW && hist_owner(d) != NARROW) {
      regime = WIDE;
      narrow_live = false;
    }
    if (regime == WIDE && hist_owner(d) == NARROW && d != no_narrow_day) {
      regime = NARROW;
      wide_live = false;
    }
    if (regime == WIDE && hist_owner(d) == CHILD) {
      regime = CHILD;
      wide_live = false;
      continue;
    }
    if (regime == NARROW) {
      PS_TRY(auto_attach(s, &s->narrow, PS_MODE_FAST, 2 * s->M + 1, &s->narrow_kernels, end));
      ps_solver* c = s->narrow;
      if (!narrow_live) {
        if (!prev) return ps_fail(PS_ERR_STATE, "auto mode: no field to continue day %d from", d);
        PS_TRY(ensure_record(c, PS_REC_STATE, 0));
        PS_HIP(hipMemcpyAsync(c->recs[PS_REC_STATE][0], prev, (size_t)s->N * s->N * sizeof(double), hipMemcpyDeviceToDevice, c->stream));
        c->spec_valid = false;
        c->srange_valid = false;
        c->have_state = true;
        narrow_live = true;
        wide_live = child_live = false;
      }
      const int w = std::min(std::max(1, stretch(d, NARROW)), end - d);
      PS_TRY(auto_alias_records(s, c, d, d + w));
      PS_TRY(ps_chain_run(c, d, w, negval, stat_scale, renorm));
      double m[64];
      PS_TRY(auto_read_padmax(s, c, d, std::min(w, 64), m));
      int x = -1;
      for (int i = 0; i < w && x < 0; ++i)
        if (m[i] >= kCleanEps && !(m[i] > 4e-8)) x = d + i;
      const int keep = x < 0 ? d + w : x;
      for (int q = d; q < keep; ++q) s->owner[q] = hint[q] = NARROW;
      d = keep;
      if (x >= 0) {
        regime = WIDE;
        narrow_live = false;
        no_narrow_day = x;
      }
      continue;
    }
    if (regime == WIDE) {
      PS_TRY(auto_attach(s, &s->wide, PS_MODE_FAST, 4 * s->M + 1, &s->wide_kernels, end));
      ps_solver* c = s->wide;
      if (!wide_live) {
        if (!prev) return ps_fail(PS_ERR_STATE, "auto mode: no field to continue day %d from", d);
        PS_TRY(ensure_record(c, PS_REC_STATE, 0));
        PS_HIP(hipMemcpyAsync(c->recs[PS_REC_STATE][0], prev, (size_t)s->N * s->N * sizeof(double), hipMemcpyDeviceToDevice, c->stream));
        c->spec_valid = false;
        c->srange_valid = false;
        c->have_state = true;
        wide_live = true;
        child_live = narrow_live = false;
      }
      const int hw = stretch(d, WIDE);
      const int w = std::min(hw > 0 ? hw : kWin, end - d);
      PS_TRY(auto_alias_records(s, c, d, d + w));
      PS_TRY(ps_chain_run(c, d, w, negval, stat_scale, renorm));
      double m[64];
      PS_TRY(auto_read_padmax(s, c, d, std::min(w, 64), m));
      int x = -1;
      for (int i = 0; i < w && x < 0; ++i)
        if (m[i] >= kCleanEps && !(m[i] > 1e-8)) x = d + i;
      const int keep = x < 0 ? d + w : x;
      for (int q = d; q < keep; ++q) {
        s->owner[q] = WIDE;
        const double mq = m[q - d];
        hint[q] = (mq > 4e-8 || mq < 0.25 * kCleanEps) ? NARROW : WIDE;
      }
      d = keep;
      if (x >= 0) {
        regime = CHILD;
        wide_live = false;
      }
    } else {
      PS_TRY(auto_attach(s, &s->child, PS_MODE_FOLD, 2 * s->M + 1, &s->child_kernels, end));
      ps_solver* c = s->child;
      if (!child_live) {
        if (!prev) return ps_fail(PS_ERR_STATE, "auto mode: no field to continue day %d from", d);
        PS_TRY(c->torus.ensure((size_t)c->Pref * c->Pref));
        PS_HIP(hipMemsetAsync(c->torus.p, 0, (size_t)c->Pref * c->Pref * sizeof(double), c->stream));
        PS_HIP(hipMemcpy2DAsync(c->torus.p, (size_t)c->Pref * sizeof(double), prev, (size_t)s->N * sizeof(double),
                                (size_t)s->N * sizeof(double), (size_t)s->N, hipMemcpyDeviceToDevice, c->stream));
        c->have_state = true;
        child_live = true;
        wide_live = narrow_live = false;
      }
      const int hc = stretch(d, CHILD);
      const int w = no_wide ? end - d : std::min(hc > 0 ? hc : kWin, end - d);
      PS_TRY(auto_alias_records(s, c, d, d + w));
      PS_TRY(ps_chain_run(c, d, w, negval, stat_scale, renorm));
      int g = -1;
      if (!no_wide) {
        double m[64];
        PS_TRY(auto_read_padmax(s, c, d, std::min(w, 64), m));
        for (int i = 0; i < w && g < 0; ++i)
          if (m[i] > 1e-8 && hist_owner(d + i + 1) != CHILD) g = d + i;
      }
      const int keep = g < 0 ? d + w : g + 1;
      for (int q = d; q < keep; ++q) s->owner[q] = hint[q] = CHILD;
      d = keep;
      if (g >= 0) {
        regime = WIDE;
        child_live = false;
      }
    }
  }
  s->auto_first = f;
  s->auto_hint = f - first;
  s->route_hist.assign(hint.begin(), hint.end());
  s->route_first = first;
  s->route_end = end;
  s->have_state = false;
  return PS_OK;
}

static int chain_run_body(ps_solver* s, int first, int count, double negval, double stat_scale, int renorm);

extern "C" int ps_chain_run(ps_solver* s, int first, int count, double negval, double stat_scale,
                            int renorm) {
  const int rc = chain_run_body(s, first, count, negval, stat_scale, renorm);
  if (s && s->kt_from >= 0) {
    (void)hipStreamWaitEvent(s->stream, s->kt_ev, 0);
    s->kt_from = -1;
  }
  if (s) s->kt_lazy_from = -1;
  if (s && s->refft_pending) {
    if (rc == PS_OK) return resolve_refft(s);
    s->refft_pending = nullptr;
  }
  return rc;
}

static int chain_run_body(ps_solver* s, int first, int count, double negval, double stat_scale, int renorm) {
  if (!s) return ps_fail(PS_ERR_BAD_ARG, "null solver");
  if (!s->have_state)
    return ps_fail(PS_ERR_STATE, s->auto_exact && s->auto_first >= 0
                                     ? "auto mode: set the state before every chain run (the previous run handed days over to the "
                                       "exact-torus helpers, the front solver's spectrum is void)"
                                     : "chain_run before set_state");
  if (!s->kernels_on_device || first < 0 || count < 0 || first + count > s->nk)
    return ps_fail(PS_ERR_STATE, "chain_run: days [%d,%d) not uploaded (nk=%d)", first, first + count, s->nk);
  PS_HIP(hipSetDevice(s->device));
  PS_TRY(ensure_stats(s, std::max(4, s->nk)));
  for (int d = first; d < first + count; ++d) PS_TRY(ensure_record(s, PS_REC_CHAIN, d));
  PS_HIP(hipMemsetAsync(s->padmax.p + first, 0, (size_t)count * sizeof(unsigned long long), s->stream));
  s->last_renorm = renorm;
  if (s->mode == PS_MODE_FOLD) {
    const size_t spec = (size_t)s->Pf * s->ld;
    PS_TRY(s->Ahat.ensure(spec));
    PS_TRY(s->fold_rowsum.ensure((size_t)s->Pf));
    PS_TRY(s->fold_rowcnt.ensure((size_t)s->Pf));
    PS_TRY(s->fold_padmax.ensure(1));
    PS_TRY(ensure_temps(s, 1));
    PS_TRY(s->T2.ensure(spec));
    const bool fuse = s->tpipe && s->rs_r2 != 0 && !s->cfg.no_fold_fuse;
    const bool fuse_alt = fuse && rs_colfull_alt_ok(s->rs_r2, s->rs_r3) && !s->cfg.no_fold_alt;
    const bool fold_rows = fuse && s->Pref >= 2 * s->M && !s->cfg.no_fold_rows;
    if (!fold_rows) PS_TRY(s->lin.ensure((size_t)s->Pf * s->Pf));
    if (fuse_alt && !s->one_flag.p) {
      PS_TRY(s->one_flag.ensure(1));
      const double one = 1.0;
      PS_HIP(hipMemcpyAsync(s->one_flag.p, &one, sizeof(double), hipMemcpyHostToDevice, s->stream));
      PS_HIP(hipStreamSynchronize(s->stream));
    }
    for (int c0 = first; c0 < first + count; c0 += s->chunk_days) {
      const int cn = std::min(s->chunk_days, first + count - c0);
      PS_TRY(transform_kernels(s, c0, cn));
      for (int d = c0; d < c0 + cn; ++d) {
        const cplx* B = s->Bhat.p + (size_t)(d - s->bhat_first) * s->Pf * s->ld;
        const SrcMap tmap = map_plain(s->Pref, s->Pf);
        if (fuse) {
          PS_TRY(launch_row_fwd(s, s->torus.p, 0, s->Pref, tmap, tmap, s->T1.p, 1, nullptr, 1, nullptr,
                                d > first ? s->padmax.p + d - 1 : nullptr, s->N));
          RowLive klive = s->kt_live;
          klive.range = s->krange.p + 2 * d;
          if (fuse_alt) {
            const ColAlt alt{s->T1.p, s->one_flag.p, RowLive{1, tmap, nullptr}};
            PS_TRY(launch_colfull(s, 0, B, s->Ahat.p, 0, s->T2.p, 1, klive, nullptr, 1, nullptr, 0, -1, -1, true, &alt));
          } else {
            PS_TRY(launch_colfull(s, 1, s->T1.p, s->Ahat.p, 0, nullptr, 1, RowLive{1, tmap, nullptr}, nullptr));
            PS_TRY(launch_colfull(s, 0, B, s->Ahat.p, 0, s->T2.p, 1, klive, nullptr));
          }
          if (fold_rows) {
            RowFoldArgs fa;
            fa.src = s->T2.p; fa.ld = s->ld; fa.M = s->Pf; fa.P = s->Pref; fa.N = s->N; fa.m = s->M;
            fa.scale = 1.0 / ((double)s->Pf * (double)s->Pf); fa.negval = negval; fa.stat_scale = stat_scale;
            fa.torus = s->torus.p; fa.rec = s->recs[PS_REC_CHAIN][d];
            fa.rowsum = s->rowsum.p + (int64_t)d * s->N; fa.rowcnt = s->rowcnt.p + (int64_t)d * s->N;
            fa.padmax = s->padmax.p + d;
            fa.prog = s->row_plan.prog;
            const int units = 2 * s->M + (s->Pref - 2 * s->M + 1) / 2;
            ProfScope prof(s, PS_PROF_ROW_INV);
            if (!rs_launch_row_fold(s->rs_r2, s->rs_r3, fa, units, s->stream))
              return ps_fail(PS_ERR_STATE, "no fold row kernel for 16 x %d x %d", s->rs_r2, s->rs_r3);
            PS_HIP(hipGetLastError());
          } else {
            PS_TRY(launch_row_inv(s, s->T2.p, s->lin.p, d, 1, negval, stat_scale, true));
            hipLaunchKernelGGL(k_fold, dim3(s->Pref), dim3(256), 0, s->stream, s->lin.p, s->Pf, s->Pref, s->N, s->M,
                               s->torus.p, s->recs[PS_REC_CHAIN][d], negval, stat_scale,
                               s->rowsum.p + (int64_t)d * s->N, s->rowcnt.p + (int64_t)d * s->N, s->padmax.p + d);
            PS_HIP(hipGetLastError());
          }
          if (d == first + count - 1) {
            hipLaunchKernelGGL(k_truncate_if_flag, dim3(s->Pref), dim3(256), 0, s->stream, s->torus.p, s->Pref, s->N,
                               s->padmax.p + d);
            PS_HIP(hipGetLastError());
          }
          continue;
        }
        if (s->tpipe) {
          PS_TRY(launch_row_fwd(s, s->torus.p, 0, s->Pref, tmap, tmap, s->T1.p, 1, nullptr, 1));
          PS_TRY(launch_colfull(s, 1, s->T1.p, s->Ahat.p, 0, nullptr, 1, RowLive{1, tmap, nullptr}, nullptr));
          RowLive klive = s->kt_live;
          klive.range = s->krange.p + 2 * d;
          PS_TRY(launch_colfull(s, 0, B, s->Ahat.p, 0, s->T2.p, 1, klive, nullptr));
          PS_TRY(launch_row_inv(s, s->T2.p, s->lin.p, d, 1, negval, stat_scale, true));
          hipLaunchKernelGGL(k_fold, dim3(s->Pref), dim3(256), 0, s->stream, s->lin.p, s->Pf, s->Pref, s->N, s->M,
                             s->torus.p, s->recs[PS_REC_CHAIN][d], negval, stat_scale,
                             s->rowsum.p + (int64_t)d * s->N, s->rowcnt.p + (int64_t)d * s->N, s->padmax.p + d);
          PS_HIP(hipGetLastError());
          hipLaunchKernelGGL(k_truncate_if_flag, dim3(s->Pref), dim3(256), 0, s->stream, s->torus.p, s->Pref, s->N,
                             s->padmax.p + d);
          PS_HIP(hipGetLastError());
          continue;
        }
        PS_TRY(launch_row_fwd(s, s->torus.p, 0, s->Pref, tmap, tmap, s->T1.p, 1, nullptr, 1));
        const cplx* part = s->T1.p;
        cplx* fused_out = s->T2.p;
        RowLive part_live{1, tmap, nullptr};
        if (s->split) {
          PS_TRY(launch_col<PS_FWD>(s, s->fwd_passes[0], s->T1.p, nullptr, nullptr, s->T2.p, 1, 0, nullptr, part_live));
          part = s->T2.p;
          fused_out = s->T1.p;
          part_live = RowLive{0, {0, 0, 0, 0}, nullptr};
        }
        int dual = 0;
        PS_TRY(launch_col_fused_dual(s, B, part, part_live, fused_out, s->krange.p + 2 * d, &dual));
        if (!dual) {
          const ColPass& last = s->fwd_passes.back();
          PS_TRY(launch_col<PS_FWD>(s, last, part, nullptr, nullptr, s->Ahat.p, 1, 0, nullptr, part_live));
          PS_TRY(launch_col_fused(s, B, s->Ahat.p, 0, fused_out, s->krange.p + 2 * d));
        }
        if (s->split) {
          PS_TRY(launch_col<PS_INV>(s, s->inv_passes[1], s->T1.p, nullptr, nullptr, s->T2.p, 1, 0, nullptr));
          PS_TRY(launch_row_inv(s, s->T2.p, s->lin.p, d, 1, negval, stat_scale, true));
        } else {
          PS_TRY(launch_row_inv(s, s->T2.p, s->lin.p, d, 1, negval, stat_scale, true));
        }
        hipLaunchKernelGGL(k_fold, dim3(s->Pref), dim3(256), 0, s->stream, s->lin.p, s->Pf, s->Pref, s->N, s->M,
                           s->torus.p, s->recs[PS_REC_CHAIN][d], negval, stat_scale,
                           s->rowsum.p + (int64_t)d * s->N, s->rowcnt.p + (int64_t)d * s->N, s->padmax.p + d);
        PS_HIP(hipGetLastError());
        hipLaunchKernelGGL(k_truncate_if_flag, dim3(s->Pref), dim3(256), 0, s->stream, s->torus.p, s->Pref, s->N,
                           s->padmax.p + d);
        PS_HIP(hipGetLastError());
      }
    }
    return PS_OK;
  }
  s->spec_window = 2;
  if (s->cfg.no_speculation) s->speculate = false;
  const int hint = s->noflag_hint;
  s->noflag_hint = 0;
  bool hinted = false;
  int flagged_at = -1;
  const double flag_thr = s->auto_exact ? kCleanEps : 1e-8;
  int hint_abs = -1;
  if (s->auto_exact) {
    s->speculate = true;
    s->auto_first = -1;
    ++s->auto_runs;
    if (count > 0 && s->auto_hint == 0 && s->auto_runs % 16 != 0)
      return auto_handover(s, first, first, first + count, negval, stat_scale, renorm,
                           s->auto_first_regime == 1 ? 1.0 : 0.0);
    if (s->auto_hint > 0) hint_abs = first + s->auto_hint;
  }
  std::vector<char> hist;
  if (!s->auto_exact && !s->speculate && s->hist_count == count && s->hist_first == first && count >= 2 &&
      !s->cfg.no_flag_history && !s->cfg.no_speculation) {
    PS_HIP(hipEventSynchronize(s->hist_ev));
    hist.resize(count);
    for (int i = 0; i < count; ++i) {
      double m;
      __builtin_memcpy(&m, &s->hhist[i], sizeof(double));
      hist[i] = !(m <= 1e-8);
    }
  }
  s->hist_count = 0;
  if (s->speculate || !hist.empty()) {
    for (int i = 0; i < 2; ++i)
      if (!s->spec_ev[i]) PS_HIP(hipEventCreateWithFlags(&s->spec_ev[i], hipEventDisableTiming));
    if (s->hflags_n < first + count) {
      if (s->hflags) (void)hipHostFree(s->hflags);
      s->hflags = nullptr;
      s->hflags_n = 0;
      PS_HIP(hipHostMalloc((void**)&s->hflags, (size_t)(first + count) * sizeof(unsigned long long), hipHostMallocDefault));
      s->hflags_n = first + count;
    }
  }
  if (s->tpipe_ok && !s->spec_valid) {
    bool compact = direct_possible(s);
    for (int d = first; d < first + count && compact; ++d) compact = day_is_compact(s, d);
    bool want = !(s->split && compact) || colfull_chains(s);
    if (s->cfg.tpipe >= 0) want = s->cfg.tpipe != 0;
    set_pipeline(s, want);
  }
  PS_TRY(ensure_spectrum(s));
  if (s->speculate && s->tpipe && colfull_chains(s) && hint >= count && count >= 4 && !s->cfg.no_window_hint) {
    int w0 = s->cfg.first_window > 0 ? s->cfg.first_window : count;
    w0 = std::max(2, std::min(std::min(w0, count), PS_MAX_GROUP_DAYS));
    s->spec_window = w0;
    hinted = true;
  }
  bool guided = false;
  if (!hist.empty() && s->tpipe && colfull_chains(s))
    for (int i = 0; i + 1 < count && !guided; ++i) guided = !hist[i] && !hist[i + 1];
  for (int c0 = first; c0 < first + count; c0 += s->chunk_days) {
    const int cn = std::min(s->chunk_days, first + count - c0);
    const int split_days = s->cfg.kt_split >= 0 ? s->cfg.kt_split : (hinted ? s->spec_window : 14);
    const bool lazy_tail = s->auto_exact && hint_abs >= c0 && hint_abs + 2 < c0 + cn &&
                           !s->cfg.no_lazy_kt;
    if (!lazy_tail && s->tpipe && s->speculate && split_days > 0 && cn >= split_days + (hinted ? 4 : 8)) {
      if (!s->stream2) {
        int lo = 0, hi = 0;
        (void)hipDeviceGetStreamPriorityRange(&lo, &hi);
        PS_HIP(hipStreamCreateWithPriority(&s->stream2, hipStreamNonBlocking, lo));
        PS_HIP(hipEventCreateWithFlags(&s->kt_ev, hipEventDisableTiming));
        PS_HIP(hipEventCreateWithFlags(&s->kt_ev0, hipEventDisableTiming));
      }
      PS_TRY(transform_kernels(s, c0, split_days, 0, cn));
      PS_HIP(hipEventRecord(s->kt_ev0, s->stream));
      PS_HIP(hipStreamWaitEvent(s->stream2, s->kt_ev0, 0));
      hipStream_t main_stream = s->stream;
      s->stream = s->stream2;
      const int rc2 = transform_kernels(s, c0 + split_days, cn - split_days, split_days, cn);
      s->stream = main_stream;
      if (rc2 != PS_OK) return rc2;
      PS_HIP(hipEventRecord(s->kt_ev, s->stream2));
      s->kt_from = c0 + split_days;
    } else if (lazy_tail) {
      const int now = hint_abs + 2 - c0;
      bool direct_all = direct_possible(s);
      for (int q = c0; q < c0 + cn && direct_all; ++q) direct_all = day_is_compact(s, q);
      s->kt_lazy_direct = direct_all ? 1 : 0;
      PS_TRY(transform_kernels(s, c0, now, 0, cn, s->kt_lazy_direct));
      s->kt_lazy_from = c0 + now;
      s->kt_lazy_c0 = c0;
      s->kt_lazy_cn = cn;
    } else {
      PS_TRY(transform_kernels(s, c0, cn));
    }
    auto day = [&](int d, bool with_refft) -> int {
      PS_TRY(kernels_ready(s, d));
      const cplx* B = s->Bhat.p + (size_t)(d - s->bhat_first) * s->Pf * s->ld;
      double* rec = s->recs[PS_REC_CHAIN][d];
      PS_TRY(conv_inv(s, B, s->Ahat.p, 1, rec, d, negval, stat_scale, s->krange.p + 2 * d));
      if (with_refft) {
        const bool defer = !s->cfg.no_defer_refft && !s->cfg.tpipe_split;
        if (s->tpipe && defer && rs_colfull_alt_ok(s->rs_r2, s->rs_r3)) PS_TRY(refft_rows_if_flag(s, rec, d));
        else PS_TRY(refft_if_flag(s, rec, s->Ahat.p, d));
      }
      return PS_OK;
    };
    struct Win { int d0, w, ev; };
    std::deque<Win> q;
    (void)flagged_at;
    int d = c0, nev = 0;
    while (true) {
      if (!s->speculate && !guided) {
        for (; d < c0 + cn; ++d) PS_TRY(day(d, true));
        break;
      }
      const size_t depth = (size_t)std::max(1, s->cfg.spec_depth);
      while (q.size() < depth && d < c0 + cn && !(hint_abs >= 0 && d == hint_abs + 1 && !q.empty())) {
        int w = std::min(s->spec_window, c0 + cn - d);
        if (hint_abs >= d) w = std::min(w, hint_abs - d + 1);
        if (guided) {
          int g = 0;
          while (d + g < c0 + cn && g < PS_MAX_GROUP_DAYS && !hist[d + g - first]) ++g;
          if (g < 2) {
            PS_TRY(day(d, true));
            ++d;
            continue;
          }
          w = g;
          PS_TRY(resolve_refft(s));
        }
        for (int i = 0; i < w;) {
          int g = 0;
          const int direct_days = s->cfg.direct_days;
          const int tpipe_days = std::min(PS_MAX_GROUP_DAYS, std::max(1, s->cfg.tpipe_days));
          const int maxd = s->tpipe ? std::min(s->fused_days >= 8 ? PS_MAX_GROUP_DAYS : s->fused_days, tpipe_days)
                                    : (s->kt_direct ? std::min(s->fused_days, direct_days) : s->fused_days);
          if (maxd > 1 && w - i >= 2) {
            int nd = s->tpipe ? std::min(maxd, w - i)
                              : (maxd >= 8 && w - i >= 8) ? 8 : (maxd >= 4 && w - i >= 4) ? 4 : 2;
            while (nd > 2 && s->T1.ensure((size_t)s->Pf * s->ld * nd) == PS_ERR_OOM) {
              (void)hipGetLastError();
              nd = std::max(2, nd / 2);
              s->cfg.tpipe_days = std::min(s->cfg.tpipe_days, nd);
            }
            PS_TRY(kernels_ready(s, d + i + nd - 1));
            const cplx* B = s->Bhat.p + (size_t)(d + i - s->bhat_first) * s->Pf * s->ld;
            PS_TRY(conv_inv_multi(s, B, nd, s->Ahat.p, &s->recs[PS_REC_CHAIN][d + i], d + i, negval, stat_scale,
                                  s->krange.p + 2 * (d + i), &g));
            if (g) g = nd;
            else s->fused_days = 1;
          }
          if (!g) {
            PS_TRY(day(d + i, false));
            g = 1;
          }
          i += g;
        }
        PS_HIP(hipMemcpyAsync(s->hflags + d, s->padmax.p + d, (size_t)w * sizeof(unsigned long long),
                              hipMemcpyDeviceToHost, s->stream));
        PS_HIP(hipEventRecord(s->spec_ev[nev & 1], s->stream));
        q.push_back(Win{d, w, nev & 1});
        ++nev;
        d += w;
        s->spec_window = hinted ? PS_MAX_GROUP_DAYS : std::min(64, 2 * s->spec_window);
      }
      if (q.empty()) break;
      const Win x = q.front();
      q.pop_front();
      PS_HIP(hipEventSynchronize(s->spec_ev[x.ev]));
      int f = -1;
      for (int i = 0; i < x.w && f < 0; ++i) {
        double m;
        __builtin_memcpy(&m, &s->hflags[x.d0 + i], sizeof(double));
        if (m > flag_thr) f = x.d0 + i;
      }
      if (f < 0) continue;
      q.clear();
      flagged_at = f;
      if (s->auto_exact) {
        double mf;
        __builtin_memcpy(&mf, &s->hflags[f], sizeof(double));
        return auto_handover(s, first, f, first + count, negval, stat_scale, renorm, mf);
      }
      s->refft_pending = nullptr;
      guided = false;
      PS_TRY(fwd2d(s, s->recs[PS_REC_CHAIN][f], 0, s->N, map_plain(s->N, s->Pf), map_plain(s->N, s->Pf),
                   s->Ahat.p, 1, nullptr));
      if (d - f - 1 > 0)
        PS_HIP(hipMemsetAsync(s->padmax.p + f + 1, 0, (size_t)(d - f - 1) * sizeof(unsigned long long), s->stream));
      s->speculate = false;
      d = f + 1;
    }
  }
  if (s->speculate && flagged_at < 0) s->noflag_hint = count;
  if (!s->auto_exact && !s->speculate && count >= 2 && !s->cfg.no_flag_history) {
    if (s->hhist_n < count) {
      if (s->hist_ev) PS_HIP(hipEventSynchronize(s->hist_ev));
      if (s->hhist) (void)hipHostFree(s->hhist);
      s->hhist = nullptr;
      s->hhist_n = 0;
      PS_HIP(hipHostMalloc((void**)&s->hhist, (size_t)(count + 32) * sizeof(unsigned long long), hipHostMallocDefault));
      s->hhist_n = count + 32;
    }
    if (!s->hist_ev) PS_HIP(hipEventCreateWithFlags(&s->hist_ev, hipEventDisableTiming));
    PS_HIP(hipMemcpyAsync(s->hhist, s->padmax.p + first, (size_t)count * sizeof(unsigned long long), hipMemcpyDeviceToHost, s->stream));
    PS_HIP(hipEventRecord(s->hist_ev, s->stream));
    s->hist_first = first;
    s->hist_count = count;
  }
  return PS_OK;
}

extern "C" int ps_chain_stats(ps_solver* s, int first, int count, ps_day_stats* out) {
  if (!s || !out || first < 0 || count < 0 || first + count > s->nstat) return ps_fail(PS_ERR_BAD_ARG, "chain_stats: bad range");
  PS_HIP(hipSetDevice(s->device));
  if (s->auto_exact && s->auto_first >= 0 && first + count > s->auto_first) {
    int d = first;
    while (d < first + count) {
      const int o = d < (int)s->owner.size() ? s->owner[d] : 0;
      int e = d + 1;
      while (e < first + count && (e < (int)s->owner.size() ? s->owner[e] : 0) == o) ++e;
      ps_solver* c = o == 1 ? s->wide : (o == 2 ? s->child : (o == 3 ? s->narrow : s));
      if (!c) return ps_fail(PS_ERR_STATE, "auto mode: day %d has no owner", d);
      if (c == s) {
        PS_TRY(finalize_days(s, d, e - d, s->last_renorm));
        PS_HIP(hipStreamSynchronize(s->stream));
        PS_HIP(hipMemcpy(out + (d - first), s->dstats.p + d, (size_t)(e - d) * sizeof(DayStats), hipMemcpyDeviceToHost));
      } else {
        PS_TRY(ps_chain_stats(c, d, e - d, out + (d - first)));
      }
      d = e;
    }
    return PS_OK;
  }
  PS_TRY(finalize_days(s, first, count, s->last_renorm));
  PS_HIP(hipStreamSynchronize(s->stream));
  static_assert(sizeof(ps_day_stats) == sizeof(DayStats), "stats layout");
  PS_HIP(hipMemcpy(out, s->dstats.p + first, (size_t)count * sizeof(DayStats), hipMemcpyDeviceToHost));
  return PS_OK;
}

__global__ void k_cmul_inplace(cplx* a, const cplx* b, int64_t n) {
  for (int64_t i = blockIdx.x * (int64_t)blockDim.x + threadIdx.x; i < n; i += (int64_t)gridDim.x * blockDim.x)
    a[i] = cmul(a[i], b[i]);
}

extern "C" int ps_solver_fftconv2_coo(ps_solver* s, const int32_t* row, const int32_t* col,
                                      const double* val, int64_t nnz, int kshape) {
  if (!s || nnz < 0) return ps_fail(PS_ERR_BAD_ARG, "fftconv2: bad arguments");
  if (s->mode == PS_MODE_FOLD) return ps_fail(PS_ERR_UNSUPPORTED, "fftconv2: PS_MODE_FOLD offers the chain API only");
  if (!s->have_state) return ps_fail(PS_ERR_STATE, "fftconv2 before set_state");
  if (kshape < 1 || kshape % 2 == 0) return ps_fail(PS_ERR_BAD_SHAPE, "kernel shape %d must be odd (CalcSol.py:58)", kshape);
  if (kshape > s->Pf) return ps_fail(PS_ERR_BAD_SHAPE, "kernel shape %d larger than the pad %d", kshape, s->Pf);
  PS_HIP(hipSetDevice(s->device));
  PS_TRY(check_coo(row, col, nnz, kshape, "kernel"));
  PS_TRY(ensure_spectrum(s));
  PS_TRY(upload_coo(s, row, col, val, nnz));
  const int K = kshape, M = K / 2;
  const size_t spec = (size_t)s->Pf * s->ld;
  PS_TRY(s->kdense.ensure((size_t)K * K));
  PS_TRY(s->Bhat.ensure(spec));
  PS_TRY(ensure_temps(s, 1));
  s->bhat_first = -1;
  PS_HIP(hipMemsetAsync(s->kdense.p, 0, (size_t)K * K * sizeof(double), s->stream));
  PS_TRY(scatter_from_device(s, s->orow.p, s->ocol.p, s->oval.p, nnz, s->kdense.p, K, 0));
  PS_TRY(fwd2d(s, s->kdense.p, 0, K, map_wrap(M, s->Pf), map_wrap(M, s->Pf), s->Bhat.p, 1, nullptr));
  hipLaunchKernelGGL(k_cmul_inplace, dim3(2048), dim3(256), 0, s->stream, s->Ahat.p, s->Bhat.p, (int64_t)spec);
  PS_HIP(hipGetLastError());
  return PS_OK;
}

extern "C" int ps_solver_get_cursol(ps_solver* s, double negval, double stat_scale, int renorm,
                                    ps_day_stats* stats) {
  if (!s) return ps_fail(PS_ERR_BAD_ARG, "null solver");
  if (s->mode == PS_MODE_FOLD) return ps_fail(PS_ERR_UNSUPPORTED, "get_cursol: PS_MODE_FOLD offers the chain API only");
  if (!s->have_state) return ps_fail(PS_ERR_STATE, "get_cursol before set_state");
  PS_HIP(hipSetDevice(s->device));
  PS_TRY(ensure_record(s, PS_REC_CHAIN, 0));
  PS_TRY(ensure_temps(s, 1));
  PS_TRY(ensure_spectrum(s));
  PS_HIP(hipMemsetAsync(s->padmax.p, 0, sizeof(unsigned long long), s->stream));
  double* rec = s->recs[PS_REC_CHAIN][0];
  PS_TRY(inv2d(s, s->Ahat.p, nullptr, nullptr, rec, 0, negval, stat_scale));
  s->last_renorm = renorm;
  PS_TRY(refft_if_flag(s, rec, s->Ahat.p, 0));
  if (stats) PS_TRY(ps_chain_stats(s, 0, 1, stats));
  return PS_OK;
}

extern "C" int ps_solver_back_solve(ps_solver* s, int nfilt, const int64_t* off, const int32_t* row,
                                    const int32_t* col, const double* val, double negval,
                                    double stat_scale, ps_day_stats* stats) {
  if (!s || nfilt < 0 || !off) return ps_fail(PS_ERR_BAD_ARG, "back_solve: bad arguments");
  if (s->mode == PS_MODE_FOLD) return ps_fail(PS_ERR_UNSUPPORTED, "back_solve: PS_MODE_FOLD offers the chain API only");
  if (!s->have_state) return ps_fail(PS_ERR_STATE, "back_solve before set_state");
  if (s->N % 2 == 0) return ps_fail(PS_ERR_BAD_SHAPE, "back_solve needs an odd domain (filters are N x N)");
  if (2 * (s->N / 2) + 1 > s->Pf) return ps_fail(PS_ERR_BAD_SHAPE, "filter larger than the pad");
  PS_HIP(hipSetDevice(s->device));
  const size_t spec = (size_t)s->Pf * s->ld;
  const int K = s->N, M = K / 2;
  PS_TRY(s->Chat.ensure(spec));
  PS_TRY(s->Bhat.ensure(spec));
  PS_TRY(s->kdense.ensure((size_t)K * K));
  PS_TRY(ensure_temps(s, 1));
  PS_TRY(ensure_stats(s, std::max(4, nfilt)));
  PS_TRY(ensure_spectrum(s));
  s->bhat_first = -1;
  PS_HIP(hipMemcpyAsync(s->Chat.p, s->Ahat.p, spec * sizeof(cplx), hipMemcpyDeviceToDevice, s->stream));
  PS_HIP(hipMemsetAsync(s->padmax.p, 0, (size_t)std::max(1, nfilt) * sizeof(unsigned long long), s->stream));
  const bool no_cache = s->cfg.no_filter_cache != 0;
  const size_t kMaxFilt = std::max<size_t>(4, std::min<size_t>(32, ((size_t)4 << 30) / (spec * sizeof(cplx))));
  for (int i = nfilt - 1; i >= 0; --i) {
    const int64_t o = off[i], n = off[i + 1] - o;
    PS_TRY(check_coo(row + o, col + o, n, K, "filter"));
    PS_TRY(ensure_record(s, PS_REC_BACK, i));
    ps_solver::FiltKey key{1469598103934665603ull, 0x9E3779B97F4A7C15ull, n};
    {
      auto mix = [&](const void* p, size_t bytes) {
        const unsigned char* b = (const unsigned char*)p;
        size_t q = 0;
        for (; q + 8 <= bytes; q += 8) {
          uint64_t w;
          __builtin_memcpy(&w, b + q, 8);
          key.h1 = (key.h1 ^ w) * 1099511628211ull;
          key.h2 = (key.h2 + w) * 0xD6E8FEB86659FD93ull;
          key.h2 ^= key.h2 >> 32;
        }
        for (; q < bytes; ++q) {
          key.h1 = (key.h1 ^ b[q]) * 1099511628211ull;
          key.h2 = (key.h2 + b[q]) * 0xD6E8FEB86659FD93ull;
        }
      };
      mix(row + o, (size_t)n * 4);
      mix(col + o, (size_t)n * 4);
      mix(val + o, (size_t)n * 8);
    }
    int slot = -1;
    if (!no_cache)
      for (size_t q = 0; q < s->filt_keys.size(); ++q)
        if (s->filt_keys[q].h1 == key.h1 && s->filt_keys[q].h2 == key.h2 && s->filt_keys[q].n == n) slot = (int)q;
    const cplx* B = nullptr;
    if (slot >= 0) {
      ++s->filt_hits;
      B = s->Fhat.p + (size_t)slot * spec;
      s->kt_direct = false;
      s->kt_live = (s->split && !s->tpipe) ? RowLive{0, {0, 0, 0, 0}, nullptr} : RowLive{1, map_wrap(M, s->Pf), nullptr};
    } else {
      ++s->filt_misses;
      cplx* dst = s->Bhat.p;
      if (!no_cache) {
        if (s->filt_keys.size() >= kMaxFilt) s->filt_keys.clear();
        if (!s->Fhat.p) PS_TRY(s->Fhat.ensure(spec * kMaxFilt));
        dst = s->Fhat.p + s->filt_keys.size() * spec;
        s->filt_keys.push_back(key);
      }
      PS_TRY(upload_coo(s, row + o, col + o, val + o, n));
      PS_HIP(hipMemsetAsync(s->kdense.p, 0, (size_t)K * K * sizeof(double), s->stream));
      PS_TRY(scatter_from_device(s, s->orow.p, s->ocol.p, s->oval.p, n, s->kdense.p, K, 0));
      PS_TRY(fwd2d_partial(s, s->kdense.p, 0, K, map_wrap(M, s->Pf), map_wrap(M, s->Pf), dst, 1));
      B = dst;
    }
    double* rec = s->recs[PS_REC_BACK][i];
    PS_TRY(conv_inv(s, B, s->Chat.p, 1, rec, i, negval, stat_scale));
    PS_TRY(refft_if_flag(s, rec, s->Chat.p, i));
  }
  s->last_renorm = 0;
  if (stats && nfilt > 0) PS_TRY(ps_chain_stats(s, 0, nfilt, stats));
  return PS_OK;
}

extern "C" int ps_chain_run_release(ps_solver* s, int first, int count, double negval, int nfilt, int nuse,
                                    const double* weights, int* certified) {
  if (!s || !weights || nfilt < 0 || nuse < 0 || nuse > nfilt || count < 0 || first < 0)
    return ps_fail(PS_ERR_BAD_ARG, "run_release: bad arguments");
  if (s->mode == PS_MODE_FOLD) return ps_fail(PS_ERR_UNSUPPORTED, "run_release: not offered in PS_MODE_FOLD");
  if (!s->have_state) return ps_fail(PS_ERR_STATE, "run_release before set_state");
  const int ndays = s->nk - nfilt;
  if (!s->kernels_on_device || ndays < 0 || first + count > ndays)
    return ps_fail(PS_ERR_STATE, "run_release: days [%d,%d) + %d filters not uploaded (nk=%d)", first, first + count, nfilt, s->nk);
  PS_HIP(hipSetDevice(s->device));
  if (certified) *certified = 1;
  const size_t spec = (size_t)s->Pf * s->ld;
  const int per = nuse + 1;
  const int units = std::max(1, count);
  const int slot0 = std::max(4, s->nk);
  PS_TRY(ensure_stats(s, slot0 + units * per));
  PS_TRY(ensure_temps(s, 1));
  PS_TRY(s->Chat.ensure(spec));
  PS_TRY(ensure_record(s, PS_REC_STATE, 1));
  for (int i = 0; i < nuse; ++i) PS_TRY(ensure_record(s, PS_REC_BACK, i));
  for (int d = first; d < first + count; ++d) PS_TRY(ensure_record(s, PS_REC_CHAIN, d));
  if (count == 0) PS_TRY(ensure_record(s, PS_REC_WSUM, 0));
  PS_HIP(hipMemsetAsync(s->padmax.p + slot0, 0, (size_t)units * per * sizeof(unsigned long long), s->stream));
  if (count > 0) PS_HIP(hipMemsetAsync(s->padmax.p + first, 0, (size_t)count * sizeof(unsigned long long), s->stream));
  s->last_renorm = 0;
  PS_TRY(resolve_refft(s));
  if (s->tpipe_ok && !s->spec_valid) set_pipeline(s, true);
  PS_TRY(ensure_spectrum(s));
  const int cdays = std::max(1, s->chunk_days - nuse);
  {
    std::vector<const double*> ptrs(per);
    for (int i = 0; i < nuse; ++i) ptrs[i] = s->recs[PS_REC_BACK][i];
    ptrs[nuse] = count > 0 ? s->recs[PS_REC_STATE][1] : s->recs[PS_REC_STATE][0];
    PS_TRY(s->wptr.ensure(per));
    PS_TRY(s->wval.ensure(per));
    PS_HIP(hipMemcpyAsync(s->wptr.p, ptrs.data(), per * sizeof(double*), hipMemcpyHostToDevice, s->stream));
    PS_HIP(hipMemcpyAsync(s->wval.p, weights, per * sizeof(double), hipMemcpyHostToDevice, s->stream));
    PS_HIP(hipStreamSynchronize(s->stream));
  }
  const int64_t tot = (int64_t)s->N * s->N;
  int c0 = 0, cn = 0;
  for (int u = 0; u < units; ++u) {
    const int d = first + u, sl = slot0 + u * per;
    if (u >= c0 + cn) {
      c0 = u;
      cn = count > 0 ? std::min(cdays, count - c0) : 0;
      if (cn > 0) PS_TRY(transform_kernels(s, first + c0, cn, 0, cn + nuse, 0));
      if (nuse > 0) PS_TRY(transform_kernels(s, ndays, nuse, cn, cn + nuse, 0));
      s->bhat_first = -1;
      s->bhat_count = 0;
      if (count == 0) cn = 1;
    }
    if (count > 0) {
      const cplx* B = s->Bhat.p + (size_t)(u - c0) * spec;
      double* rec = s->recs[PS_REC_STATE][1];
      PS_TRY(conv_inv(s, B, s->Ahat.p, 1, rec, sl + nuse, negval, 1.0, s->krange.p + 2 * d));
      PS_TRY(refft_if_flag(s, rec, s->Ahat.p, sl + nuse));
    }
    if (nuse > 0) PS_HIP(hipMemcpyAsync(s->Chat.p, s->Ahat.p, spec * sizeof(cplx), hipMemcpyDeviceToDevice, s->stream));
    for (int i = nuse - 1; i >= 0; --i) {
      const cplx* F = s->Bhat.p + (size_t)((count > 0 ? cn : 0) + i) * spec;
      double* rec = s->recs[PS_REC_BACK][i];
      PS_TRY(conv_inv(s, F, s->Chat.p, 1, rec, sl + i, negval, 1.0, s->krange.p + 2 * (ndays + i)));
      PS_TRY(refft_if_flag(s, rec, s->Chat.p, sl + i));
    }
    double* out = count > 0 ? s->recs[PS_REC_CHAIN][d] : s->recs[PS_REC_WSUM][0];
    hipLaunchKernelGGL(k_weighted_sum, dim3(2048), dim3(256), 0, s->stream, (const double* const*)s->wptr.p,
                       s->wval.p, per, tot, out);
    PS_HIP(hipGetLastError());
    if (count > 0) {
      hipLaunchKernelGGL(k_row_stats, dim3(s->N), dim3(256), 0, s->stream, out, s->N, 1.0, negval,
                         s->rowsum.p + (int64_t)d * s->N, s->rowcnt.p + (int64_t)d * s->N);
      PS_HIP(hipGetLastError());
    }
  }
  s->noflag_hint = 0;
  s->hist_count = 0;
  if (s->auto_exact) {
    std::vector<unsigned long long> h((size_t)units * per);
    PS_HIP(hipMemcpyAsync(h.data(), s->padmax.p + slot0, h.size() * sizeof(unsigned long long), hipMemcpyDeviceToHost, s->stream));
    PS_HIP(hipStreamSynchronize(s->stream));
    int ok = 1;
    for (unsigned long long v : h) {
      double m;
      __builtin_memcpy(&m, &v, sizeof(double));
      if (!(m < kCleanEps)) ok = 0;
    }
    if (certified) *certified = ok;
    s->auto_first = -1;
  }
  return PS_OK;
}

extern "C" int ps_chain_block_prefix(ps_solver* s, int first, int count, const void** total_dev, int64_t* total_bytes) {
  if (!s || first < 0 || count < 1 || !total_dev) return ps_fail(PS_ERR_BAD_ARG, "block_prefix: bad arguments");
  if (s->mode != PS_MODE_FAST || !s->tpipe_ok)
    return ps_fail(PS_ERR_UNSUPPORTED, "block_prefix: fast mode on a register-resident FFT size only (this solver: mode %d, size %d)", s->mode, s->Pf);
  if (!s->have_state) return ps_fail(PS_ERR_STATE, "block_prefix before set_state");
  if (!s->kernels_on_device || first + count > s->nk)
    return ps_fail(PS_ERR_STATE, "block_prefix: days [%d,%d) not uploaded (nk=%d)", first, first + count, s->nk);
  PS_HIP(hipSetDevice(s->device));
  PS_TRY(resolve_refft(s));
  if (!s->spec_valid) set_pipeline(s, true);
  if (!s->tpipe) return ps_fail(PS_ERR_UNSUPPORTED, "block_prefix: the state's spectrum is held for the tiled pipeline; set the state again");
  PS_TRY(ensure_spectrum(s));
  const size_t spec = (size_t)s->Pf * s->ld;
  const int64_t n = (int64_t)s->H * s->Pf;
  PS_TRY(transform_kernels(s, first, count, 0, count, 0));
  s->bhat_first = -1;
  s->bhat_count = 0;
  PS_TRY(s->blk.ensure(spec * count));
  RowLive live = s->kt_live;
  live.range = s->krange.p + 2 * first;
  PS_TRY(launch_colfull(s, 1, s->Bhat.p, s->blk.p, 0, nullptr, count, live, nullptr));
  for (int i = 1; i < count; ++i) {
    hipLaunchKernelGGL(k_cmul_inplace, dim3(2048), dim3(256), 0, s->stream, s->blk.p + (size_t)i * spec,
                       s->blk.p + (size_t)(i - 1) * spec, n);
    PS_HIP(hipGetLastError());
  }
  s->blk_first = first;
  s->blk_count = count;
  *total_dev = s->blk.p + (size_t)(count - 1) * spec;
  if (total_bytes) *total_bytes = (int64_t)(spec * sizeof(cplx));
  PS_HIP(hipStreamSynchronize(s->stream));
  return PS_OK;
}

extern "C" int ps_chain_block_finish(ps_solver* s, int first, int count, int nprev, const void* const* prev_totals,
                                     double negval, double stat_scale, int renorm, int* flagged) {
  if (!s || nprev < 0 || (nprev > 0 && !prev_totals)) return ps_fail(PS_ERR_BAD_ARG, "block_finish: bad arguments");
  if (s->blk_first != first || s->blk_count != count || count < 1)
    return ps_fail(PS_ERR_STATE, "block_finish: days [%d,%d) were not prepared by block_prefix", first, first + count);
  PS_HIP(hipSetDevice(s->device));
  const size_t spec = (size_t)s->Pf * s->ld;
  const int64_t n = (int64_t)s->H * s->Pf;
  PS_TRY(ensure_stats(s, std::max(4, s->nk)));
  for (int d = first; d < first + count; ++d) PS_TRY(ensure_record(s, PS_REC_CHAIN, d));
  PS_HIP(hipMemsetAsync(s->padmax.p + first, 0, (size_t)count * sizeof(unsigned long long), s->stream));
  PS_TRY(s->Chat.ensure(spec));
  PS_HIP(hipMemcpyAsync(s->Chat.p, s->Ahat.p, spec * sizeof(cplx), hipMemcpyDeviceToDevice, s->stream));
  for (int j = 0; j < nprev; ++j) {
    if (!prev_totals[j]) return ps_fail(PS_ERR_BAD_ARG, "block_finish: block total %d is null", j);
    hipLaunchKernelGGL(k_cmul_inplace, dim3(2048), dim3(256), 0, s->stream, s->Chat.p, (const cplx*)prev_totals[j], n);
    PS_HIP(hipGetLastError());
  }
  for (int i = 0; i < count; ++i) {
    hipLaunchKernelGGL(k_cmul_inplace, dim3(2048), dim3(256), 0, s->stream, s->blk.p + (size_t)i * spec, s->Chat.p, n);
    PS_HIP(hipGetLastError());
  }
  s->blk_first = -1;
  s->blk_count = 0;
  PS_TRY(s->T1.ensure(spec * count));
  PS_TRY(launch_colfull(s, 2, nullptr, s->blk.p, 0, s->T1.p, count, RowLive{0, {0, 0, 0, 0}, nullptr}, nullptr));
  if (row_inv_persistent(s) && !s->tinv && count <= PS_MAX_GROUP_DAYS && !s->cfg.no_row_batch) {
    std::vector<double*> recs(count);
    for (int i = 0; i < count; ++i) recs[i] = s->recs[PS_REC_CHAIN][first + i];
    PS_TRY(launch_row_inv(s, s->T1.p, nullptr, first, count, negval, stat_scale, false, recs.data(), nullptr));
  } else {
    for (int i = 0; i < count; ++i)
      PS_TRY(launch_row_inv(s, s->T1.p + (size_t)i * spec, s->recs[PS_REC_CHAIN][first + i], first + i, 1, negval, stat_scale));
  }
  s->last_renorm = renorm;
  PS_TRY(finalize_days(s, first, count, renorm));
  PS_HIP(hipMemcpyAsync(s->Ahat.p, s->blk.p + (size_t)(count - 1) * spec, spec * sizeof(cplx), hipMemcpyDeviceToDevice, s->stream));
  s->noflag_hint = 0;
  s->hist_count = 0;
  std::vector<unsigned long long> h((size_t)count);
  PS_HIP(hipMemcpyAsync(h.data(), s->padmax.p + first, h.size() * sizeof(unsigned long long), hipMemcpyDeviceToHost, s->stream));
  PS_HIP(hipStreamSynchronize(s->stream));
  int any = 0;
  for (unsigned long long v : h) {
    double m;
    __builtin_memcpy(&m, &v, sizeof(double));
    if (!(m <= 1e-8)) any = 1;
  }
  if (flagged) *flagged = any;
  return PS_OK;
}

extern "C" int ps_device_copy(void* dst, const void* src, int64_t bytes) {
  if (!dst || !src || bytes < 0) return ps_fail(PS_ERR_BAD_ARG, "device_copy: bad arguments");
  PS_HIP(hipMemcpy(dst, src, (size_t)bytes, hipMemcpyDeviceToDevice));
  return PS_OK;
}

static int get_record(ps_solver* s, int kind, int idx, double** out) {
  if (kind < 0 || kind > 3 || idx < 0 || idx >= (int)s->recs[kind].size() || !s->recs[kind][idx])
    return ps_fail(PS_ERR_STATE, "record (%d,%d) does not exist", kind, idx);
  *out = s->recs[kind][idx];
  return PS_OK;
}

extern "C" int ps_record_stats(ps_solver* s, int kind, int idx, double negval, double stat_scale,
                               int renorm, ps_day_stats* out) {
  if (!s || !out) return ps_fail(PS_ERR_BAD_ARG, "record_stats: bad arguments");
  PS_HIP(hipSetDevice(s->device));
  double* rec;
  PS_TRY(get_record(s, kind, idx, &rec));
  PS_TRY(ensure_stats(s, 4));
  const int slot = s->nstat;
  PS_HIP(hipMemsetAsync(s->padmax.p + slot, 0, sizeof(unsigned long long), s->stream));
  hipLaunchKernelGGL(k_row_stats, dim3(s->N), dim3(256), 0, s->stream, rec, s->N, stat_scale, negval,
                     s->rowsum.p + (int64_t)slot * s->N, s->rowcnt.p + (int64_t)slot * s->N);
  PS_HIP(hipGetLastError());
  hipLaunchKernelGGL(k_day_finalize, dim3(1), dim3(256), 0, s->stream, s->rowsum.p + (int64_t)slot * s->N,
                     s->rowcnt.p + (int64_t)slot * s->N, s->padmax.p + slot, s->N, renorm,
                     s->dstats.p + slot);
  PS_HIP(hipGetLastError());
  PS_HIP(hipStreamSynchronize(s->stream));
  PS_HIP(hipMemcpy(out, s->dstats.p + slot, sizeof(DayStats), hipMemcpyDeviceToHost));
  return PS_OK;
}

static int fetch_sparse(ps_solver* s, int kind, int idx, double negval, double stat_scale, double delta,
                        double post_scale, int32_t* row, int32_t* indptr, int32_t* col, double* val,
                        int64_t cap, int64_t* nnz_out) {
  if (!s) return ps_fail(PS_ERR_BAD_ARG, "null solver");
  PS_HIP(hipSetDevice(s->device));
  double* rec;
  PS_TRY(get_record(s, kind, idx, &rec));
  PS_TRY(ensure_stats(s, 4));
  const int slot = s->nstat;
  double* rs = s->rowsum.p + (int64_t)slot * s->N;
  long long* rc = s->rowcnt.p + (int64_t)slot * s->N;
  hipLaunchKernelGGL(k_row_stats, dim3(s->N), dim3(256), 0, s->stream, rec, s->N, stat_scale, negval, rs, rc);
  PS_HIP(hipGetLastError());
  hipLaunchKernelGGL(k_scan_rows, dim3(1), dim3(1024), 0, s->stream, rc, s->N, s->rowoff.p);
  PS_HIP(hipGetLastError());
  PS_HIP(hipStreamSynchronize(s->stream));
  long long last_off = 0, last_cnt = 0;
  PS_HIP(hipMemcpy(&last_off, s->rowoff.p + (s->N - 1), sizeof(long long), hipMemcpyDeviceToHost));
  PS_HIP(hipMemcpy(&last_cnt, rc + (s->N - 1), sizeof(long long), hipMemcpyDeviceToHost));
  const int64_t nnz = last_off + last_cnt;
  if (nnz_out) *nnz_out = nnz;
  if ((!row && !indptr) || !col || !val) return PS_OK;
  if (cap < nnz) return ps_fail(PS_ERR_BAD_ARG, "fetch: capacity %lld < nnz %lld", (long long)cap, (long long)nnz);
  if (indptr) {
    if (nnz > 0x7fffffffLL) return ps_fail(PS_ERR_UNSUPPORTED, "fetch_csr: %lld entries do not fit int32 offsets", (long long)nnz);
    std::vector<long long> off((size_t)s->N);
    PS_HIP(hipMemcpy(off.data(), s->rowoff.p, (size_t)s->N * sizeof(long long), hipMemcpyDeviceToHost));
    for (int i = 0; i < s->N; ++i) indptr[i] = (int32_t)off[(size_t)i];
    indptr[s->N] = (int32_t)nnz;
  }
  if (nnz == 0) return PS_OK;
  PS_TRY(s->orow.ensure(nnz));
  PS_TRY(s->ocol.ensure(nnz));
  PS_TRY(s->oval.ensure(nnz));
  const int thr = 256;
  const int blocks = (s->N * 64 + thr - 1) / thr;
  hipLaunchKernelGGL(k_compact_rows, dim3(blocks), dim3(thr), 0, s->stream, rec, s->N, stat_scale, negval,
                     delta, post_scale, s->rowoff.p, s->orow.p, s->ocol.p, s->oval.p);
  PS_HIP(hipGetLastError());
  if (row) PS_HIP(hipMemcpyAsync(row, s->orow.p, nnz * 4, hipMemcpyDeviceToHost, s->stream));
  PS_HIP(hipMemcpyAsync(col, s->ocol.p, nnz * 4, hipMemcpyDeviceToHost, s->stream));
  PS_HIP(hipMemcpyAsync(val, s->oval.p, nnz * 8, hipMemcpyDeviceToHost, s->stream));
  PS_HIP(hipStreamSynchronize(s->stream));
  return PS_OK;
}

extern "C" int ps_record_fetch_coo(ps_solver* s, int kind, int idx, double negval, double stat_scale,
                                   double delta, double post_scale, int32_t* row, int32_t* col,
                                   double* val, int64_t cap, int64_t* nnz_out) {
  return fetch_sparse(s, kind, idx, negval, stat_scale, delta, post_scale, row, nullptr, col, val, cap, nnz_out);
}

extern "C" int ps_record_fetch_csr(ps_solver* s, int kind, int idx, double negval, double stat_scale,
                                   double delta, double post_scale, int32_t* indptr, int32_t* indices,
                                   double* data, int64_t cap, int64_t* nnz_out) {
  return fetch_sparse(s, kind, idx, negval, stat_scale, delta, post_scale, nullptr, indptr, indices, data, cap, nnz_out);
}

extern "C" int ps_record_fetch_dense(ps_solver* s, int kind, int idx, double* out) {
  if (!s || !out) return ps_fail(PS_ERR_BAD_ARG, "fetch_dense: bad arguments");
  PS_HIP(hipSetDevice(s->device));
  double* rec;
  PS_TRY(get_record(s, kind, idx, &rec));
  PS_HIP(hipMemcpyAsync(out, rec, (size_t)s->N * s->N * sizeof(double), hipMemcpyDeviceToHost, s->stream));
  PS_HIP(hipStreamSynchronize(s->stream));
  return PS_OK;
}

extern "C" int ps_record_gather(ps_solver* s, int kind, int idx, int64_t n, const int32_t* rows,
                                const int32_t* cols, double scale, double negval, double* out) {
  if (!s || n < 0 || (n > 0 && (!rows || !cols || !out))) return ps_fail(PS_ERR_BAD_ARG, "record_gather: bad arguments");
  if (n == 0) return PS_OK;
  PS_HIP(hipSetDevice(s->device));
  double* rec;
  PS_TRY(get_record(s, kind, idx, &rec));
  PS_TRY(check_coo(rows, cols, n, s->N, "gather point"));
  PS_TRY(s->orow.ensure(n));
  PS_TRY(s->ocol.ensure(n));
  PS_TRY(s->oval.ensure(n));
  PS_HIP(hipMemcpyAsync(s->orow.p, rows, n * 4, hipMemcpyHostToDevice, s->stream));
  PS_HIP(hipMemcpyAsync(s->ocol.p, cols, n * 4, hipMemcpyHostToDevice, s->stream));
  const int blocks = (int)std::min<int64_t>((n + 255) / 256, 1024);
  hipLaunchKernelGGL(k_gather_points, dim3(blocks), dim3(256), 0, s->stream, rec, s->N, s->orow.p, s->ocol.p, n,
                     scale, negval, s->oval.p);
  PS_HIP(hipGetLastError());
  PS_HIP(hipMemcpyAsync(out, s->oval.p, n * 8, hipMemcpyDeviceToHost, s->stream));
  PS_HIP(hipStreamSynchronize(s->stream));
  return PS_OK;
}

extern "C" int ps_record_gather_multi(ps_solver* s, int nrec, const int32_t* kind, const int32_t* idx, int64_t n,
                                      const int32_t* rows, const int32_t* cols, double scale, double negval,
                                      double* out) {
  if (!s || nrec < 0 || n < 0 || (nrec > 0 && (!kind || !idx)) || (n > 0 && nrec > 0 && (!rows || !cols || !out)))
    return ps_fail(PS_ERR_BAD_ARG, "record_gather_multi: bad arguments");
  if (n == 0 || nrec == 0) return PS_OK;
  PS_HIP(hipSetDevice(s->device));
  std::vector<const double*> ptrs(nrec);
  for (int r = 0; r < nrec; ++r) {
    double* rec;
    PS_TRY(get_record(s, kind[r], idx[r], &rec));
    ptrs[r] = rec;
  }
  PS_TRY(check_coo(rows, cols, n, s->N, "gather point"));
  PS_TRY(s->orow.ensure(n));
  PS_TRY(s->ocol.ensure(n));
  PS_TRY(s->oval.ensure((size_t)n * nrec));
  PS_TRY(s->wptr.ensure(nrec));
  PS_HIP(hipMemcpyAsync(s->orow.p, rows, n * 4, hipMemcpyHostToDevice, s->stream));
  PS_HIP(hipMemcpyAsync(s->ocol.p, cols, n * 4, hipMemcpyHostToDevice, s->stream));
  PS_HIP(hipMemcpyAsync(s->wptr.p, ptrs.data(), nrec * sizeof(double*), hipMemcpyHostToDevice, s->stream));
  PS_HIP(hipStreamSynchronize(s->stream));
  const int blocks = (int)std::min<int64_t>((n + 255) / 256, 1024);
  hipLaunchKernelGGL(k_gather_points_multi, dim3(blocks, nrec), dim3(256), 0, s->stream,
                     (const double* const*)s->wptr.p, s->N, s->orow.p, s->ocol.p, n, scale, negval, s->oval.p);
  PS_HIP(hipGetLastError());
  PS_HIP(hipMemcpyAsync(out, s->oval.p, (size_t)n * nrec * 8, hipMemcpyDeviceToHost, s->stream));
  PS_HIP(hipStreamSynchronize(s->stream));
  return PS_OK;
}

extern "C" int ps_weighted_sum(ps_solver* s, int n, const int32_t* kind, const int32_t* idx, const double* w) {
  if (!s || n < 1 || !kind || !idx || !w) return ps_fail(PS_ERR_BAD_ARG, "weighted_sum: bad arguments");
  PS_HIP(hipSetDevice(s->device));
  std::vector<const double*> ptrs(n);
  for (int d = 0; d < n; ++d) {
    double* r;
    PS_TRY(get_record(s, kind[d], idx[d], &r));
    ptrs[d] = r;
  }
  PS_TRY(ensure_record(s, PS_REC_WSUM, 0));
  PS_TRY(s->wptr.ensure(n));
  PS_TRY(s->wval.ensure(n));
  PS_HIP(hipMemcpyAsync(s->wptr.p, ptrs.data(), n * sizeof(double*), hipMemcpyHostToDevice, s->stream));
  PS_HIP(hipMemcpyAsync(s->wval.p, w, n * sizeof(double), hipMemcpyHostToDevice, s->stream));
  PS_HIP(hipStreamSynchronize(s->stream));
  const int64_t tot = (int64_t)s->N * s->N;
  hipLaunchKernelGGL(k_weighted_sum, dim3(2048), dim3(256), 0, s->stream, (const double* const*)s->wptr.p,
                     s->wval.p, n, tot, s->recs[PS_REC_WSUM][0]);
  PS_HIP(hipGetLastError());
  return PS_OK;
}

extern "C" int ps_solver_get_spectrum(ps_solver* s, double* out) {
  if (!s || !out) return ps_fail(PS_ERR_BAD_ARG, "get_spectrum: bad arguments");
  if (s->mode == PS_MODE_FOLD) return ps_fail(PS_ERR_UNSUPPORTED, "get_spectrum: PS_MODE_FOLD offers the chain API only");
  if (!s->have_state) return ps_fail(PS_ERR_STATE, "get_spectrum before set_state");
  PS_HIP(hipSetDevice(s->device));
  if (s->tpipe) {
    if (s->spec_valid) return ps_fail(PS_ERR_UNSUPPORTED, "get_spectrum: the state is held column-major (full-column pipeline)");
    set_pipeline(s, false);
  }
  PS_TRY(ensure_spectrum(s));
  const size_t full = (size_t)s->Pf * s->Pf;
  DevBuf<cplx> tmp;
  PS_TRY(tmp.ensure(full));
  hipLaunchKernelGGL(k_expand_spectrum, dim3(2048), dim3(256), 0, s->stream, s->Ahat.p, s->Pf, s->H, s->ld, tmp.p);
  hipError_t e = hipGetLastError();
  if (e == hipSuccess) e = hipMemcpyAsync(out, tmp.p, full * sizeof(cplx), hipMemcpyDeviceToHost, s->stream);
  if (e == hipSuccess) e = hipStreamSynchronize(s->stream);
  tmp.release();
  if (e != hipSuccess) return ps_fail(PS_ERR_HIP, "get_spectrum: %s", hipGetErrorString(e));
  return PS_OK;
}

extern "C" int ps_solver_set_spectrum(ps_solver* s, const double* in) {
  if (!s || !in) return ps_fail(PS_ERR_BAD_ARG, "set_spectrum: bad arguments");
  if (s->mode == PS_MODE_FOLD) return ps_fail(PS_ERR_UNSUPPORTED, "set_spectrum: PS_MODE_FOLD offers the chain API only");
  PS_HIP(hipSetDevice(s->device));
  set_pipeline(s, false);
  const size_t full = (size_t)s->Pf * s->Pf;
  DevBuf<cplx> tmp;
  PS_TRY(tmp.ensure(full));
  hipError_t e = hipMemcpyAsync(tmp.p, in, full * sizeof(cplx), hipMemcpyHostToDevice, s->stream);
  if (e == hipSuccess) {
    hipLaunchKernelGGL(k_take_half_spectrum, dim3(2048), dim3(256), 0, s->stream, tmp.p, s->Pf, s->H, s->ld, s->Ahat.p);
    e = hipGetLastError();
  }
  if (e == hipSuccess) e = hipStreamSynchronize(s->stream);
  tmp.release();
  if (e != hipSuccess) return ps_fail(PS_ERR_HIP, "set_spectrum: %s", hipGetErrorString(e));
  s->have_state = true;
  s->spec_valid = true;
  return PS_OK;
}

extern "C" int ps_solver_set_option(ps_solver* s, const char* key, double value) {
  if (!s || !key) return ps_fail(PS_ERR_BAD_ARG, "set_option: bad arguments");
  const int rc = ps_config_set(&s->cfg, key, value, true);
  if (rc == -1) return ps_fail(PS_ERR_BAD_ARG, "set_option: unknown option %s", key);
  if (rc == -2) return ps_fail(PS_ERR_STATE, "set_option: %s takes effect when a solver is created", key);
  s->tinv = s->cfg.tinv != 0;
  s->fused_days = s->cfg.fused_days;
  if (s->child) PS_TRY(ps_solver_set_option(s->child, key, value));
  if (s->wide) PS_TRY(ps_solver_set_option(s->wide, key, value));
  if (s->narrow) PS_TRY(ps_solver_set_option(s->narrow, key, value));
  return PS_OK;
}

extern "C" int ps_solver_get_option(ps_solver* s, const char* key, double* value) {
  if (!s || !key || !value) return ps_fail(PS_ERR_BAD_ARG, "get_option: bad arguments");
  if (ps_config_get(&s->cfg, key, value) != 0) return ps_fail(PS_ERR_BAD_ARG, "get_option: unknown option %s", key);
  return PS_OK;
}

static int prof_drain(ps_solver* s) {
  PS_HIP(hipStreamSynchronize(s->stream));
  for (auto& r : s->prof_pending) {
    float ms = 0.f;
    if (hipEventElapsedTime(&ms, r.a, r.b) == hipSuccess) {
      s->prof_ms[r.cls] += ms;
      s->prof_cnt[r.cls] += 1;
      s->prof_days[r.cls] += r.days;
    }
    s->prof_pool.push_back(r.a);
    s->prof_pool.push_back(r.b);
  }
  s->prof_pending.clear();
  return PS_OK;
}

extern "C" int ps_prof_enable(ps_solver* s, int on) {
  if (!s) return ps_fail(PS_ERR_BAD_ARG, "null solver");
  PS_HIP(hipSetDevice(s->device));
  PS_TRY(prof_drain(s));
  for (int i = 0; i < PS_PROF_NCLS; ++i) { s->prof_ms[i] = 0; s->prof_cnt[i] = 0; s->prof_seen[i] = 0; s->prof_days[i] = 0; }
  s->prof_on = on != 0;
  s->prof_every = on > 1 ? on : 1;
  for (ps_solver* c : {s->wide, s->child, s->narrow})
    if (c) PS_TRY(ps_prof_enable(c, on));
  return PS_OK;
}

extern "C" int ps_prof_read(ps_solver* s, int ncls, double* total_ms, int64_t* count) {
  if (!s || !total_ms || !count) return ps_fail(PS_ERR_BAD_ARG, "prof_read: bad arguments");
  PS_HIP(hipSetDevice(s->device));
  PS_TRY(prof_drain(s));
  for (int i = 0; i < ncls; ++i) {
    total_ms[i] = i < PS_PROF_NCLS ? s->prof_ms[i] : 0.0;
    count[i] = i < PS_PROF_NCLS ? s->prof_cnt[i] : 0;
  }
  return PS_OK;
}

extern "C" int ps_prof_read_days(ps_solver* s, int ncls, int64_t* days) {
  if (!s || !days) return ps_fail(PS_ERR_BAD_ARG, "prof_read_days: bad arguments");
  PS_HIP(hipSetDevice(s->device));
  PS_TRY(prof_drain(s));
  for (int i = 0; i < ncls; ++i) days[i] = i < PS_PROF_NCLS ? s->prof_days[i] : 0;
  return PS_OK;
}

extern "C" int ps_prof_read_launches(ps_solver* s, int ncls, int64_t* launches) {
  if (!s || !launches) return ps_fail(PS_ERR_BAD_ARG, "prof_read_launches: bad arguments");
  PS_HIP(hipSetDevice(s->device));
  PS_TRY(prof_drain(s));
  for (int i = 0; i < ncls; ++i)
    launches[i] = i >= PS_PROF_NCLS ? 0 : (i >= PS_PROF_COL_INV_A2 ? s->prof_cnt[i] : s->prof_seen[i]);
  return PS_OK;
}

extern "C" int ps_prof_read_owner(ps_solver* s, int owner, int ncls, double* total_ms, int64_t* count,
                                  int64_t* launches, int64_t* days) {
  if (!s || owner < 0 || owner > 3 || !total_ms || !count || !launches || !days)
    return ps_fail(PS_ERR_BAD_ARG, "prof_read_owner: bad arguments");
  ps_solver* c = owner == 1 ? s->wide : (owner == 2 ? s->child : (owner == 3 ? s->narrow : s));
  if (!c) {
    for (int i = 0; i < ncls; ++i) { total_ms[i] = 0.0; count[i] = 0; launches[i] = 0; days[i] = 0; }
    return PS_OK;
  }
  PS_TRY(ps_prof_read(c, ncls, total_ms, count));
  PS_TRY(ps_prof_read_launches(c, ncls, launches));
  return ps_prof_read_days(c, ncls, days);
}

extern "C" int ps_solver_kernels_direct(ps_solver* s) { return s && s->kt_direct ? 1 : 0; }

extern "C" int ps_solver_pipeline(ps_solver* s) { return s && s->tpipe ? 1 : 0; }

extern "C" int ps_solver_auto_route(ps_solver* s, int first, int count, int32_t* owner) {
  if (!s || !owner || first < 0 || count < 0) return ps_fail(PS_ERR_BAD_ARG, "auto_route: bad arguments");
  for (int i = 0; i < count; ++i) {
    const int d = first + i;
    owner[i] = (s->auto_exact && s->auto_first >= 0 && d >= s->auto_first && d < (int)s->owner.size()) ? s->owner[d] : 0;
  }
  return PS_OK;
}

extern "C" int ps_solver_auto_info(ps_solver* s, int* first_fold_day, int* fold_fft) {
  if (!s) return ps_fail(PS_ERR_BAD_ARG, "null solver");
  if (first_fold_day) *first_fold_day = s->auto_exact ? s->auto_first : -1;
  if (fold_fft) *fold_fft = s->child ? s->child->Pf : 0;
  return PS_OK;
}

extern "C" int ps_solver_owner_fft(ps_solver* s, int owner) {
  if (!s) return 0;
  ps_solver* c = owner == 1 ? s->wide : (owner == 2 ? s->child : (owner == 3 ? s->narrow : (owner == 0 ? s : nullptr)));
  return c ? c->Pf : 0;
}

int ps_solver_dom_len_internal(ps_solver* s) { return s->N; }
int ps_solver_device_internal(ps_solver* s) { return s->device; }

int ps_solver_record_internal(ps_solver* s, int kind, int idx, int want_stats, PsRecordView* out) {
  if (!s || !out) return ps_fail(PS_ERR_BAD_ARG, "record view: bad arguments");
  PS_HIP(hipSetDevice(s->device));
  double* rec;
  PS_TRY(get_record(s, kind, idx, &rec));
  out->rec = rec;
  out->stats = nullptr;
  out->stream = s->stream;
  out->N = s->N;
  out->device = s->device;
  if (!want_stats) return PS_OK;
  if (kind != PS_REC_CHAIN || idx >= s->nstat)
    return ps_fail(PS_ERR_STATE, "record (%d,%d) has no day statistics", kind, idx);
  ps_solver* c = s;
  if (s->auto_exact && s->auto_first >= 0 && idx < (int)s->owner.size()) {
    const int o = s->owner[idx];
    c = o == 1 ? s->wide : (o == 2 ? s->child : (o == 3 ? s->narrow : s));
    if (!c) return ps_fail(PS_ERR_STATE, "auto mode: day %d has no owner", idx);
    if (idx >= c->nstat) return ps_fail(PS_ERR_STATE, "auto mode: day %d has no statistics", idx);
  }
  PS_TRY(finalize_days(c, idx, 1, c->last_renorm));
  out->stats = reinterpret_cast<const ps_day_stats*>(c->dstats.p + idx);
  return PS_OK;
}
```

### parasitoids_amd/hip_lib.py

```python
import ctypes as C
import warnings

import numpy as np
from scipy import sparse

from . import _lib as L

L.load()
L.require_device()


def _coo_arrays(A):
    A = sparse.coo_matrix(A)
    return L.i32(A.row), L.i32(A.col), L.f64(A.data), A.shape


def _smooth7(n):
    for p in (2, 3, 5, 7):
        while n % p == 0:
            n //= p
    return n == 1


def _create_solver(lib, handle, dev, dom_len, max_shape, mode, chain_only=False):
# ... 143 lines not shown
        L.check(self._lib.ps_solver_fftconv2_coo(self._h, L.p_i32(row), L.p_i32(col),
                                                 L.p_f64(val), len(val), int(shape[0])))

    def get_cursol(self, dom_shape, negval=1e-8, fetch=True):
        self._check_dom(dom_shape)
        st = L.DayStats()
        L.check(self._lib.ps_solver_get_cursol(self._h, negval, 1.0, 0, C.byref(st)))
        self.last_flag = bool(st.flag)
        if not fetch:
            return None
        return self._fetch(L.REC_CHAIN, 0, negval, 1.0, 0.0, 1.0, st.nnz)

    def back_solve(self, prev_spread, dom_shape, negval=1e-8, fetch=True):
        self._check_dom(dom_shape)
        nf = len(prev_spread)
        if nf == 0:
            return []
        rows, cols, vals, off = [], [], [], [0]
        for B in prev_spread:
            r, c, v, shape = _coo_arrays(B)
            if shape != (self.dom_len, self.dom_len):
                raise ValueError('back_solve filters must be dom_len x dom_len')
            rows.append(r); cols.append(c); vals.append(v)
            off.append(off[-1] + len(v))
        row = L.i32(np.concatenate(rows)); col = L.i32(np.concatenate(cols))
        val = L.f64(np.concatenate(vals)); off = np.ascontiguousarray(off, dtype=np.int64)
        stats = (L.DayStats * nf)()
        L.check(self._lib.ps_solver_back_solve(self._h, nf, L.p_i64(off), L.p_i32(row),
                                               L.p_i32(col), L.p_f64(val), negval, 1.0, stats))
        self.last_back_flags = [bool(s.flag) for s in stats]
        if not fetch:
            return None
        return [self._fetch(L.REC_BACK, i, negval, 1.0, 0.0, 1.0, stats[i].nnz)
                for i in range(nf)]

    def set_kernels(self, pmf_list):
        rows, cols, vals, off, ks = [], [], [], [0], []
        for B in pmf_list:
            r, c, v, shape = _coo_arrays(B)
            if shape[0] != shape[1]:
                raise ValueError('kernel must be square, got {}'.format(shape))
            rows.append(r); cols.append(c); vals.append(v)
            off.append(off[-1] + len(v)); ks.append(shape[0])
        cat = lambda xs, dt: np.ascontiguousarray(
            np.concatenate(xs) if xs else np.zeros(0), dtype=dt)
        row, col, val = cat(rows, np.int32), cat(cols, np.int32), cat(vals, np.float64)
        off = np.ascontiguousarray(off, dtype=np.int64)
        ks = np.ascontiguousarray(ks, dtype=np.int32)
        L.check(self._lib.ps_chain_set_kernels(self._h, len(ks), L.p_i64(off), L.p_i32(ks),
                                               L.p_i32(row), L.p_i32(col), L.p_f64(val)))
        self._nk = len(ks)

    def set_release(self, pmf_days, r_spread):
        M = self.pad_shape[0] - self.dom_len
        mid = self.dom_len // 2
        filt = []
        for F in r_spread:
            F = sparse.coo_matrix(F)
            if F.shape != (self.dom_len, self.dom_len):
                raise ValueError('release filters must be dom_len x dom_len')
            h = int(max(np.abs(F.row - mid).max(), np.abs(F.col - mid).max())) if F.nnz else 0
            if h > M:
                return False
            filt.append(sparse.coo_matrix((F.data, (F.row - mid + h, F.col - mid + h)),
                                          shape=(2 * h + 1, 2 * h + 1)))
        self.set_kernels(list(pmf_days) + filt)
        self._nfilt = len(filt)
        return True

    def run_release(self, first, count, weights, nuse=None, negval=1e-8):
        nuse = self._nfilt if nuse is None else nuse
        w = L.f64(weights)
        if len(w) != nuse + 1:
            raise ValueError('need nuse + 1 weights')
        ok = C.c_int(1)
        L.check(self._lib.ps_chain_run_release(self._h, first, count, negval, self._nfilt, nuse,
                                               L.p_f64(w), C.byref(ok)))
        return bool(ok.value)

    def block_prefix(self, first, count):
        ptr, nbytes = C.c_void_p(), C.c_int64(0)
        L.check(self._lib.ps_chain_block_prefix(self._h, int(first), int(count), C.byref(ptr), C.byref(nbytes)))
        return ptr.value, nbytes.value

    def block_finish(self, first, count, prev_totals=(), negval=1e-8, scale=1.0, renorm=True):
        n = len(prev_totals)
        arr = (C.c_void_p * max(n, 1))(*[int(p) for p in prev_totals])
        flag = C.c_int(0)
        L.check(self._lib.ps_chain_block_finish(self._h, int(first), int(count), n, arr, negval, scale,
                                                int(bool(renorm)), C.byref(flag)))
        return bool(flag.value)

    def device_copy(self, dst_ptr, src_ptr, nbytes):
        L.check(self._lib.ps_device_copy(C.c_void_p(int(dst_ptr)), C.c_void_p(int(src_ptr)), int(nbytes)))

    def run_chain(self, first=0, count=None, negval=1e-8, scale=1.0, renorm=True):
        count = self._nk - first if count is None else count
        L.check(self._lib.ps_chain_run(self._h, first, count, negval, scale, int(bool(renorm))))

    def chain_stats(self, first, count):
        stats = (L.DayStats * count)()
        L.check(self._lib.ps_chain_stats(self._h, first, count, stats))
        return list(stats)

    def chain_solution(self, day, stats, negval=1e-8, scale=1.0, fmt='coo'):
        return self._fetch(L.REC_CHAIN, day, negval, scale, stats.delta, 1.0, stats.nnz, fmt)

    def record_stats(self, kind, idx, negval=1e-8, scale=1.0, renorm=False):
        st = L.DayStats()
        L.check(self._lib.ps_record_stats(self._h, kind, idx, negval, scale, int(renorm),
                                          C.byref(st)))
        return st

    def weighted_sum(self, kinds, idxs, weights):
        k = L.i32(kinds); i = L.i32(idxs); w = L.f64(weights)
        L.check(self._lib.ps_weighted_sum(self._h, len(w), L.p_i32(k), L.p_i32(i), L.p_f64(w)))

    def gather(self, kind, idx, rows, cols, scale=1.0, negval=1e-8):
        r, c = L.i32(rows), L.i32(cols)
        out = np.empty(len(r))
        L.check(self._lib.ps_record_gather(self._h, kind, idx, len(r), L.p_i32(r), L.p_i32(c),
                                           float(scale), float(negval), L.p_f64(out)))
        return out

    def gather_multi(self, kinds, idxs, rows, cols, scale=1.0, negval=1e-8):
        k, i = L.i32(kinds), L.i32(idxs)
        r, c = L.i32(rows), L.i32(cols)
        out = np.empty((len(k), len(r)))
        L.check(self._lib.ps_record_gather_multi(self._h, len(k), L.p_i32(k), L.p_i32(i), len(r),
                                                 L.p_i32(r), L.p_i32(c), float(scale), float(negval),
                                                 L.p_f64(out)))
        return out

    def dense(self, kind, idx):
        out = np.empty((self.dom_len, self.dom_len))
        L.check(self._lib.ps_record_fetch_dense(self._h, kind, idx, L.p_f64(out)))
        return out

    def sync(self):
        L.check(self._lib.ps_solver_sync(self._h))

    def set_option(self, key, value):
        L.check(self._lib.ps_solver_set_option(self._h, key.encode(), float(value)))

    def get_option(self, key):
        v = C.c_double()
        L.check(self._lib.ps_solver_get_option(self._h, key.encode(), C.byref(v)))
        return v.value

    @property
    def full_column(self):
        return bool(self._lib.ps_solver_pipeline(self._h))

    def auto_info(self):
        a, b = C.c_int32(-1), C.c_int32(0)
        L.check(self._lib.ps_solver_auto_info(self._h, C.byref(a), C.byref(b)))
        return a.value, b.value

    def auto_route(self, first, count):
        out = np.zeros(count, dtype=np.int32)
        L.check(self._lib.ps_solver_auto_route(self._h, int(first), int(count), L.p_i32(out)))
        return out

    @property
    def kernels_direct(self):
        return bool(self._lib.ps_solver_kernels_direct(self._h))

    PROF_CLASSES = ('row_fwd', 'col_fwd_a', 'col_fwd_b', 'col_inv_a', 'col_inv_b', 'row_inv',
                    'refft_pred', 'col_inv_a_x2', 'col_inv_a_x4', 'col_inv_a_x8',
                    'row_inv_x2', 'row_inv_x4', 'row_inv_x8', 'col_inv_a_xn', 'row_inv_xn', 'col_tail')

    def prof_enable(self, on=True, every=1):
        L.check(self._lib.ps_prof_enable(self._h, (max(1, int(every)) if on else 0)))

    def prof_read(self):
        n = len(self.PROF_CLASSES)
        ms = np.zeros(n)
        cnt = np.zeros(n, dtype=np.int64)
        L.check(self._lib.ps_prof_read(self._h, n, L.p_f64(ms), L.p_i64(cnt)))
        return {k: (float(ms[i]), int(cnt[i])) for i, k in enumerate(self.PROF_CLASSES)}

    def prof_days(self):
        n = len(self.PROF_CLASSES)
        days = np.zeros(n, dtype=np.int64)
        L.check(self._lib.ps_prof_read_days(self._h, n, L.p_i64(days)))
        return {k: int(days[i]) for i, k in enumerate(self.PROF_CLASSES)}

    def prof_launches(self):
        n = len(self.PROF_CLASSES)
        cnt = np.zeros(n, dtype=np.int64)
        L.check(self._lib.ps_prof_read_launches(self._h, n, L.p_i64(cnt)))
        return {k: int(cnt[i]) for i, k in enumerate(self.PROF_CLASSES)}

    PROF_OWNERS = ('front', 'wide', 'fold', 'narrow')

    def prof_owner(self, owner):
        o = self.PROF_OWNERS.index(owner) if isinstance(owner, str) else int(owner)
        n = len(self.PROF_CLASSES)
        ms = np.zeros(n)
        cnt, lau, days = (np.zeros(n, dtype=np.int64) for _ in range(3))
        L.check(self._lib.ps_prof_read_owner(self._h, o, n, L.p_f64(ms), L.p_i64(cnt), L.p_i64(lau), L.p_i64(days)))
        return {k: dict(ms=float(ms[i]), timed=int(cnt[i]), launches=int(lau[i]), days=int(days[i]))
                for i, k in enumerate(self.PROF_CLASSES) if lau[i] or cnt[i]}

    def helper_fft_len(self, owner):
        o = self.PROF_OWNERS.index(owner) if isinstance(owner, str) else int(owner)
        return int(self._lib.ps_solver_owner_fft(self._h, o))

    def get_spectrum(self):
        P = self.fft_len
        out = np.empty((P, P), dtype=np.complex128)
        L.check(self._lib.ps_solver_get_spectrum(self._h, out.ctypes.data_as(L._F64P)))
        return out

    def set_spectrum(self, A_hat):
        A_hat = np.ascontiguousarray(A_hat, dtype=np.complex128)
        if A_hat.shape != (self.fft_len, self.fft_len):
            raise ValueError('spectrum shape {} != pad shape'.format(A_hat.shape))
        L.check(self._lib.ps_solver_set_spectrum(self._h, A_hat.ctypes.data_as(L._F64P)))

    def _check_dom(self, dom_shape):
        if int(dom_shape[0]) != self.dom_len or int(dom_shape[1]) != self.dom_len:
            raise ValueError('dom_shape {} != solver domain {}'.format(
                tuple(dom_shape), self.dom_len))

    def _fetch(self, kind, idx, negval, scale, delta, post, nnz_hint, fmt='coo'):
        n = int(nnz_hint)
        cap = max(n, 1)
        N = self.dom_len
        while True:
            first = np.empty(cap if fmt == 'coo' else N + 1, dtype=np.int32)
            col = np.empty(cap, dtype=np.int32)
            val = np.empty(cap, dtype=np.float64)
            nnz = C.c_int64()
            fn = self._lib.ps_record_fetch_coo if fmt == 'coo' else self._lib.ps_record_fetch_csr
            rc = fn(self._h, kind, idx, negval, scale, delta, post, L.p_i32(first), L.p_i32(col),
                    L.p_f64(val), cap, C.byref(nnz))
            if rc == L.PS_ERR_BAD_ARG and nnz.value > cap:
                cap = nnz.value
                continue
            L.check(rc)
            n = nnz.value
            if fmt == 'coo':
                return sparse.coo_matrix((val[:n], (first[:n], col[:n])), shape=(N, N))
            return sparse.csr_matrix((val[:n], col[:n], first), shape=(N, N))
```

Measured before the change: 4313 grid-days/s.

## Defer speculative flag check across calls and stage COO uploads through pinned buffers

Adds a deferred-settlement mechanism: the speculative refft flag check at the end of a chain run is left pending and resolved at the next API entry. When the next call repeats the same day window, the kernel transforms are issued before waiting, so host work overlaps the device tail. State COO uploads now go through double-buffered pinned staging with events instead of a blocking stream sync, and the state clear and kernel band zeroing are limited to the rows actually touched. This adds complexity and risks correctness: late flags must be recovered by rerunning days, and every entry point has to settle first.

```diff
diff --git a/include/parasitoid_hip.h b/include/parasitoid_hip.h
--- a/include/parasitoid_hip.h
+++ b/include/parasitoid_hip.h
@@ -52,6 +52,7 @@
 int ps_solver_get_option(ps_solver* s, const char* key, double* value);
 int ps_solver_kernels_direct(ps_solver* s);
 int ps_solver_pipeline(ps_solver* s);
+int ps_solver_deferred_info(ps_solver* s, int* pending, int64_t* counts);
 int ps_solver_auto_info(ps_solver* s, int* first_fold_day, int* fold_fft);
 int ps_solver_auto_route(ps_solver* s, int first, int count, int32_t* owner);
 
diff --git a/parasitoids_amd/_lib.py b/parasitoids_amd/_lib.py
--- a/parasitoids_amd/_lib.py
+++ b/parasitoids_amd/_lib.py
@@ -70,6 +70,7 @@
     'ps_fast_size': (C.c_int, [C.c_int, C.c_int]),
     'ps_solver_kernels_direct': (C.c_int, [_VP]),
     'ps_solver_pipeline': (C.c_int, [_VP]),
+    'ps_solver_deferred_info': (C.c_int, [_VP, _I32P, _I64P]),
     'ps_solver_auto_info': (C.c_int, [_VP, _I32P, _I32P]),
     'ps_solver_auto_route': (C.c_int, [_VP, C.c_int, C.c_int, _I32P]),
     'ps_record_fetch_coo': (C.c_int, [_VP, C.c_int, C.c_int, C.c_double, C.c_double, C.c_double,
diff --git a/parasitoids_amd/csrc/chain_kernels.h b/parasitoids_amd/csrc/chain_kernels.h
--- a/parasitoids_amd/csrc/chain_kernels.h
+++ b/parasitoids_amd/csrc/chain_kernels.h
@@ -10,7 +10,9 @@
     atomicAdd(&dst[(int64_t)(row[i] + roff) * ld + col[i] + coff], val[i]);
 }
 
-static __global__ void k_zero_band(double* dst, int K, int r0, int r1) {
+static __global__ void k_zero_band(double* dst, int K, const int* __restrict__ range) {
+  const int r0 = max(range[2 * blockIdx.y], 0), r1 = min(range[2 * blockIdx.y + 1], K - 1);
+  if (r1 < r0) return;
   double* base = dst + (int64_t)blockIdx.y * K * K + (int64_t)r0 * K;
   const int64_t n = (int64_t)(r1 - r0 + 1) * K;
   for (int64_t i = blockIdx.x * (int64_t)blockDim.x + threadIdx.x; i < n; i += (int64_t)gridDim.x * blockDim.x)
diff --git a/parasitoids_amd/csrc/ps_config.h b/parasitoids_amd/csrc/ps_config.h
--- a/parasitoids_amd/csrc/ps_config.h
+++ b/parasitoids_amd/csrc/ps_config.h
@@ -50,6 +50,7 @@
   X("PS_SPEC_DEPTH", spec_depth, 2, INT, R)                                                         \
   X("PS_NO_FLAG_HISTORY", no_flag_history, 0, FLAG, R)                                              \
   X("PS_NO_WINDOW_HINT", no_window_hint, 0, FLAG, R)                                                \
+  X("PS_NO_DEFER_CHECK", no_defer_check, 0, FLAG, R)                                                \
   X("PS_FIRST_WINDOW", first_window, -1, INT, R)                                                    \
   X("PS_KT_SPLIT", kt_split, -1, INT, R)                                                            \
   X("PS_NO_LAZY_KT", no_lazy_kt, 0, FLAG, R)                                                        \
diff --git a/parasitoids_amd/csrc/ps_solver.hip b/parasitoids_amd/csrc/ps_solver.hip
--- a/parasitoids_amd/csrc/ps_solver.hip
+++ b/parasitoids_amd/csrc/ps_solver.hip
@@ -172,6 +172,18 @@
   unsigned long long* hhist = nullptr;
   int hhist_n = 0, hist_first = -1, hist_count = 0;
   hipEvent_t hist_ev = nullptr;
+  struct Pending {
+    bool on = false;
+    int first = 0, count = 0;
+    int d0 = 0, w = 0, ev = 0;
+    double negval = 0, stat_scale = 0;
+    double thr = 1e-8;
+  } pend;
+  long long n_deferred = 0, n_late_flags = 0, n_staged_early = 0, n_staged_uploads = 0;
+  bool kt_early = false;
+  struct Stage { char* p = nullptr; size_t cap = 0; hipEvent_t ev = nullptr; bool busy = false; } stage[2];
+  int stage_next = 0;
+  int hsrange[2] = {1, 0};
   int rs_r2 = 0, rs_r3 = 0;
   int L1 = 0, L2 = 0;
   DevBuf<cplx> tp_lo, tp_hi;
@@ -282,6 +294,12 @@
   }
 };
 
+static int settle(ps_solver* s);
+static int enter(ps_solver* s) {
+  PS_HIP(hipSetDevice(s->device));
+  return settle(s);
+}
+
 static int row_threads(int L, bool big = false) { return L <= 1024 ? 256 : ((L <= 2560 || big) ? 512 : 1024); }
 static int row_pairs(const FftProg& P) {
   int rp = 2048 / std::max(1, P.L);
@@ -1002,6 +1020,7 @@
 extern "C" int ps_solver_destroy(ps_solver* s) {
   if (!s) return PS_OK;
   (void)hipSetDevice(s->device);
+  s->pend.on = false;
   if (s->stream) (void)hipStreamSynchronize(s->stream);
   if (s->child) {
     ps_solver_destroy(s->child);
@@ -1043,6 +1062,10 @@
   for (auto e : s->prof_pool) (void)hipEventDestroy(e);
   for (auto e : s->spec_ev) if (e) (void)hipEventDestroy(e);
   if (s->hflags) (void)hipHostFree(s->hflags);
+  for (auto& st : s->stage) {
+    if (st.ev) (void)hipEventDestroy(st.ev);
+    if (st.p) (void)hipHostFree(st.p);
+  }
   if (s->hhist) (void)hipHostFree(s->hhist);
   if (s->hist_ev) (void)hipEventDestroy(s->hist_ev);
   s->dkoff.release(); s->dkshape.release();
@@ -1058,7 +1081,7 @@
     if (s->N + m > s->Pf)
       return ps_fail(PS_ERR_BAD_SHAPE, "retarget: max_shape %d needs an FFT size >= %d, the solver has %d", max_shape,
                      s->N + m, s->Pf);
-    PS_HIP(hipSetDevice(s->device));
+    PS_TRY(enter(s));
     PS_HIP(hipStreamSynchronize(s->stream));
     if (s->child && ps_solver_retarget(s->child, max_shape) != PS_OK) {
       ps_solver_destroy(s->child);
@@ -1088,7 +1111,7 @@
   if (s->N + 3 * m > s->Pf)
     return ps_fail(PS_ERR_BAD_SHAPE, "retarget: max_shape %d needs an FFT size >= %d, the solver has %d", max_shape,
                    s->N + 3 * m, s->Pf);
-  PS_HIP(hipSetDevice(s->device));
+  PS_TRY(enter(s));
   PS_HIP(hipStreamSynchronize(s->stream));
   s->M = m;
   s->Pref = s->N + m;
@@ -1109,7 +1132,7 @@
 
 extern "C" int ps_solver_sync(ps_solver* s) {
   if (!s) return ps_fail(PS_ERR_BAD_ARG, "null solver");
-  PS_HIP(hipSetDevice(s->device));
+  PS_TRY(enter(s));
   PS_HIP(hipStreamSynchronize(s->stream));
   return PS_OK;
 }
@@ -1143,22 +1166,56 @@
   PS_TRY(s->orow.ensure(std::max<int64_t>(nnz, 1)));
   PS_TRY(s->ocol.ensure(std::max<int64_t>(nnz, 1)));
   PS_TRY(s->oval.ensure(std::max<int64_t>(nnz, 1)));
-  if (nnz > 0) {
+  if (nnz <= 0) return PS_OK;
+  const size_t bytes = (size_t)nnz * 16;
+  ps_solver::Stage& st = s->stage[s->stage_next];
+  s->stage_next ^= 1;
+  if (st.busy) PS_HIP(hipEventSynchronize(st.ev));
+  st.busy = false;
+  if (st.cap < bytes) {
+    if (st.p) (void)hipHostFree(st.p);
+    st.p = nullptr;
+    st.cap = 0;
+    const size_t cap = std::max<size_t>(bytes + bytes / 2, 4096);
+    if (hipHostMalloc((void**)&st.p, cap, hipHostMallocDefault) == hipSuccess) st.cap = cap;
+    else { st.p = nullptr; (void)hipGetLastError(); }
+  }
+  if (!st.p) {
     PS_HIP(hipMemcpyAsync(s->orow.p, row, nnz * 4, hipMemcpyHostToDevice, s->stream));
     PS_HIP(hipMemcpyAsync(s->ocol.p, col, nnz * 4, hipMemcpyHostToDevice, s->stream));
     PS_HIP(hipMemcpyAsync(s->oval.p, val, nnz * 8, hipMemcpyHostToDevice, s->stream));
     PS_HIP(hipStreamSynchronize(s->stream));
-  }
-  return PS_OK;
-}
-
-int ps_solver_set_state_device_coo(ps_solver* s, const int* row, const int* col, const double* val,
-                                   int64_t nnz, int off) {
+    return PS_OK;
+  }
+  if (!st.ev) PS_HIP(hipEventCreateWithFlags(&st.ev, hipEventDisableTiming));
+  char* hv = st.p;
+  char* hr = hv + (size_t)nnz * 8;
+  char* hc = hr + (size_t)nnz * 4;
+  std::memcpy(hv, val, (size_t)nnz * 8);
+  std::memcpy(hr, row, (size_t)nnz * 4);
+  std::memcpy(hc, col, (size_t)nnz * 4);
+  PS_HIP(hipMemcpyAsync(s->orow.p, hr, nnz * 4, hipMemcpyHostToDevice, s->stream));
+  PS_HIP(hipMemcpyAsync(s->ocol.p, hc, nnz * 4, hipMemcpyHostToDevice, s->stream));
+  PS_HIP(hipMemcpyAsync(s->oval.p, hv, nnz * 8, hipMemcpyHostToDevice, s->stream));
+  PS_HIP(hipEventRecord(st.ev, s->stream));
+  st.busy = true;
+  ++s->n_staged_uploads;
+  return PS_OK;
+}
+
+static int set_state_scatter(ps_solver* s, const int* row, const int* col, const double* val, int64_t nnz, int off,
+                             bool known_rows) {
+  const bool fresh = s->recs[PS_REC_STATE].empty() || !s->recs[PS_REC_STATE][0];
   PS_TRY(ensure_record(s, PS_REC_STATE, 0));
   PS_TRY(ensure_temps(s, 1));
+  double* rec = s->recs[PS_REC_STATE][0];
+  if (known_rows && s->srange_valid && !fresh && s->mode != PS_MODE_FOLD) {
+    const int lo = std::max(s->hsrange[0], 0), hi = std::min(s->hsrange[1], s->N - 1);
+    if (lo <= hi) PS_HIP(hipMemsetAsync(rec + (size_t)lo * s->N, 0, (size_t)(hi - lo + 1) * s->N * sizeof(double), s->stream));
+  } else {
+    PS_HIP(hipMemsetAsync(rec, 0, (size_t)s->N * s->N * sizeof(double), s->stream));
+  }
   s->srange_valid = false;
-  double* rec = s->recs[PS_REC_STATE][0];
-  PS_HIP(hipMemsetAsync(rec, 0, (size_t)s->N * s->N * sizeof(double), s->stream));
   PS_TRY(scatter_from_device(s, row, col, val, nnz, rec, s->N, off));
   if (s->mode == PS_MODE_FOLD) {
     PS_TRY(s->torus.ensure((size_t)s->Pref * s->Pref));
@@ -1173,6 +1230,11 @@
   return PS_OK;
 }
 
+int ps_solver_set_state_device_coo(ps_solver* s, const int* row, const int* col, const double* val,
+                                   int64_t nnz, int off) {
+  return set_state_scatter(s, row, col, val, nnz, off, false);
+}
+
 static int ensure_spectrum(ps_solver* s) {
   if (s->spec_valid || s->mode == PS_MODE_FOLD) return PS_OK;
   if (s->recs[PS_REC_STATE].empty() || !s->recs[PS_REC_STATE][0]) return ps_fail(PS_ERR_STATE, "no state record");
@@ -1198,7 +1260,7 @@
   PS_HIP(hipSetDevice(s->device));
   PS_TRY(check_coo(row, col, nnz, s->N, "state"));
   PS_TRY(upload_coo(s, row, col, val, nnz));
-  PS_TRY(ps_solver_set_state_device_coo(s, s->orow.p, s->ocol.p, s->oval.p, nnz, 0));
+  PS_TRY(set_state_scatter(s, s->orow.p, s->ocol.p, s->oval.p, nnz, 0, true));
   int range[2] = {1, 0};
   for (int64_t i = 0; i < nnz; ++i) {
     if (range[0] > range[1]) range[0] = range[1] = row[i];
@@ -1208,6 +1270,8 @@
   PS_TRY(s->srange.ensure(2));
   hipLaunchKernelGGL(k_set_int2, dim3(1), dim3(64), 0, s->stream, s->srange.p, range[0], range[1]);
   PS_HIP(hipGetLastError());
+  s->hsrange[0] = range[0];
+  s->hsrange[1] = range[1];
   s->srange_valid = true;
   return PS_OK;
 }
@@ -1234,21 +1298,16 @@
   PS_TRY(s->Bhat.ensure(spec * total));
   PS_TRY(ensure_temps(s, total));
   double* kd = s->kdense.p + (size_t)slot0 * K * K;
-  int blo = K, bhi = -1;
+  int maxrows = 0;
   int64_t maxn = 0;
   for (int d = first; d < first + count; ++d) {
-    if (s->hkrange[2 * d] <= s->hkrange[2 * d + 1]) {
-      blo = std::min(blo, s->hkrange[2 * d]);
-      bhi = std::max(bhi, s->hkrange[2 * d + 1]);
-    }
+    maxrows = std::max(maxrows, std::min(s->hkrange[2 * d + 1], K - 1) - std::max(s->hkrange[2 * d], 0) + 1);
     maxn = std::max<int64_t>(maxn, s->koff[d + 1] - s->koff[d]);
   }
-  if (bhi >= blo) {
-    blo = std::max(blo, 0);
-    bhi = std::min(bhi, K - 1);
-    const int64_t n = (int64_t)(bhi - blo + 1) * K;
+  if (maxrows > 0) {
+    const int64_t n = (int64_t)maxrows * K;
     const int blocks = (int)std::min<int64_t>((n + 255) / 256, 2048);
-    hipLaunchKernelGGL(k_zero_band, dim3(blocks, count), dim3(256), 0, s->stream, kd, K, blo, bhi);
+    hipLaunchKernelGGL(k_zero_band, dim3(blocks, count), dim3(256), 0, s->stream, kd, K, s->krange.p + 2 * first);
     PS_HIP(hipGetLastError());
   }
   if (maxn > 0) {
@@ -1283,6 +1342,7 @@
 }
 
 static int drain_kernel_readers(ps_solver* s) {
+  PS_TRY(enter(s));
   if (s->stream2) PS_HIP(hipStreamSynchronize(s->stream2));
   PS_HIP(hipStreamSynchronize(s->stream));
   return PS_OK;
@@ -1343,7 +1403,7 @@
 extern "C" int ps_chain_set_kernels(ps_solver* s, int nk, const int64_t* off, const int32_t* kshape,
                                     const int32_t* row, const int32_t* col, const double* val) {
   if (!s || nk < 0 || !off || (nk > 0 && !kshape)) return ps_fail(PS_ERR_BAD_ARG, "set_kernels: bad arguments");
-  PS_HIP(hipSetDevice(s->device));
+  PS_TRY(enter(s));
   const int64_t tot = off[nk];
   for (int d = 0; d < nk; ++d) {
     if (off[d + 1] < off[d]) return ps_fail(PS_ERR_BAD_ARG, "offsets not monotone");
@@ -1578,6 +1638,82 @@
   return PS_OK;
 }
 
+static bool want_full_column(const ps_solver* s, int first, int count) {
+  bool compact = direct_possible(s);
+  for (int d = first; d < first + count && compact; ++d) compact = day_is_compact(s, d);
+  bool want = !(s->split && compact) || colfull_chains(s);
+  if (s->cfg.tpipe >= 0) want = s->cfg.tpipe != 0;
+  return want;
+}
+
+static int run_day(ps_solver* s, int d, bool with_refft, double negval, double stat_scale) {
+  PS_TRY(kernels_ready(s, d));
+  const cplx* B = s->Bhat.p + (size_t)(d - s->bhat_first) * s->Pf * s->ld;
+  double* rec = s->recs[PS_REC_CHAIN][d];
+  PS_TRY(conv_inv(s, B, s->Ahat.p, 1, rec, d, negval, stat_scale, s->krange.p + 2 * d));
+  if (with_refft) {
+    const bool defer = !s->cfg.no_defer_refft && !s->cfg.tpipe_split;
+    if (s->tpipe && defer && rs_colfull_alt_ok(s->rs_r2, s->rs_r3)) PS_TRY(refft_rows_if_flag(s, rec, d));
+    else PS_TRY(refft_if_flag(s, rec, s->Ahat.p, d));
+  }
+  return PS_OK;
+}
+
+static int recover_from_flag(ps_solver* s, int f, int end) {
+  s->refft_pending = nullptr;
+  PS_TRY(fwd2d(s, s->recs[PS_REC_CHAIN][f], 0, s->N, map_plain(s->N, s->Pf), map_plain(s->N, s->Pf),
+               s->Ahat.p, 1, nullptr));
+  if (end - f - 1 > 0)
+    PS_HIP(hipMemsetAsync(s->padmax.p + f + 1, 0, (size_t)(end - f - 1) * sizeof(unsigned long long), s->stream));
+  s->speculate = false;
+  return PS_OK;
+}
+
+static int finish_run(ps_solver* s, int first, int count, bool flagged) {
+  if (s->speculate && !flagged) s->noflag_hint = count;
+  if (!s->auto_exact && !s->speculate && count >= 2 && !s->cfg.no_flag_history) {
+    if (s->hhist_n < count) {
+      if (s->hist_ev) PS_HIP(hipEventSynchronize(s->hist_ev));
+      if (s->hhist) (void)hipHostFree(s->hhist);
+      s->hhist = nullptr;
+      s->hhist_n = 0;
+      PS_HIP(hipHostMalloc((void**)&s->hhist, (size_t)(count + 32) * sizeof(unsigned long long), hipHostMallocDefault));
+      s->hhist_n = count + 32;
+    }
+    if (!s->hist_ev) PS_HIP(hipEventCreateWithFlags(&s->hist_ev, hipEventDisableTiming));
+    PS_HIP(hipMemcpyAsync(s->hhist, s->padmax.p + first, (size_t)count * sizeof(unsigned long long), hipMemcpyDeviceToHost, s->stream));
+    PS_HIP(hipEventRecord(s->hist_ev, s->stream));
+    s->hist_first = first;
+    s->hist_count = count;
+  }
+  return PS_OK;
+}
+
+static int first_flagged_day(const ps_solver* s, int d0, int w, double thr) {
+  for (int i = 0; i < w; ++i) {
+    double m;
+    __builtin_memcpy(&m, &s->hflags[d0 + i], sizeof(double));
+    if (m > thr) return d0 + i;
+  }
+  return -1;
+}
+
+static int settle(ps_solver* s) {
+  if (!s->pend.on) return PS_OK;
+  const ps_solver::Pending p = s->pend;
+  s->pend.on = false;
+  PS_HIP(hipEventSynchronize(s->spec_ev[p.ev]));
+  const int f = first_flagged_day(s, p.d0, p.w, p.thr);
+  if (f >= 0) {
+    const int end = p.first + p.count;
+    ++s->n_late_flags;
+    PS_TRY(recover_from_flag(s, f, end));
+    for (int d = f + 1; d < end; ++d) PS_TRY(run_day(s, d, true, p.negval, p.stat_scale));
+  }
+  PS_TRY(finish_run(s, p.first, p.count, f >= 0));
+  return resolve_refft(s);
+}
+
 static int chain_run_body(ps_solver* s, int first, int count, double negval, double stat_scale, int renorm);
 
 extern "C" int ps_chain_run(ps_solver* s, int first, int count, double negval, double stat_scale,
@@ -1588,6 +1724,7 @@
     s->kt_from = -1;
   }
   if (s) s->kt_lazy_from = -1;
+  if (s) s->kt_early = false;
   if (s && s->refft_pending) {
     if (rc == PS_OK) return resolve_refft(s);
     s->refft_pending = nullptr;
@@ -1605,6 +1742,20 @@
   if (!s->kernels_on_device || first < 0 || count < 0 || first + count > s->nk)
     return ps_fail(PS_ERR_STATE, "chain_run: days [%d,%d) not uploaded (nk=%d)", first, first + count, s->nk);
   PS_HIP(hipSetDevice(s->device));
+  const int ks = s->cfg.kt_split;
+  const bool can_hint = count >= 4 && !s->cfg.no_window_hint && colfull_chains(s);
+  const bool whole_unhinted = ks == 0 || count < (ks > 0 ? ks : 14) + 8;
+  const bool whole_hinted = ks >= 0 ? (ks == 0 || count < ks + 4)
+                                    : (s->cfg.first_window <= 0 && count < PS_MAX_GROUP_DAYS + 4);
+  const bool stays_whole = can_hint ? whole_hinted : whole_unhinted;
+  if (s->pend.on && !s->cfg.no_defer_check && s->pend.first == first && s->pend.count == count &&
+      count <= s->chunk_days && s->tpipe && (s->spec_valid || want_full_column(s, first, count)) &&
+      stays_whole) {
+    PS_TRY(transform_kernels(s, first, count));
+    s->kt_early = true;
+    ++s->n_staged_early;
+  }
+  PS_TRY(settle(s));
   PS_TRY(ensure_stats(s, std::max(4, s->nk)));
   for (int d = first; d < first + count; ++d) PS_TRY(ensure_record(s, PS_REC_CHAIN, d));
   PS_HIP(hipMemsetAsync(s->padmax.p + first, 0, (size_t)count * sizeof(unsigned long long), s->stream));
@@ -1762,13 +1913,7 @@
       s->hflags_n = first + count;
     }
   }
-  if (s->tpipe_ok && !s->spec_valid) {
-    bool compact = direct_possible(s);
-    for (int d = first; d < first + count && compact; ++d) compact = day_is_compact(s, d);
-    bool want = !(s->split && compact) || colfull_chains(s);
-    if (s->cfg.tpipe >= 0) want = s->cfg.tpipe != 0;
-    set_pipeline(s, want);
-  }
+  if (s->tpipe_ok && !s->spec_valid) set_pipeline(s, want_full_column(s, first, count));
   PS_TRY(ensure_spectrum(s));
   if (s->speculate && s->tpipe && colfull_chains(s) && hint >= count && count >= 4 && !s->cfg.no_window_hint) {
     int w0 = s->cfg.first_window > 0 ? s->cfg.first_window : count;
@@ -1779,12 +1924,16 @@
   bool guided = false;
   if (!hist.empty() && s->tpipe && colfull_chains(s))
     for (int i = 0; i + 1 < count && !guided; ++i) guided = !hist[i] && !hist[i + 1];
+  const bool defer_ok = !s->cfg.no_defer_check && s->mode == PS_MODE_FAST && !s->auto_exact && !s->borrowed &&
+                        s->tpipe && s->speculate && !guided && count <= s->chunk_days;
   for (int c0 = first; c0 < first + count; c0 += s->chunk_days) {
     const int cn = std::min(s->chunk_days, first + count - c0);
     const int split_days = s->cfg.kt_split >= 0 ? s->cfg.kt_split : (hinted ? s->spec_window : 14);
     const bool lazy_tail = s->auto_exact && hint_abs >= c0 && hint_abs + 2 < c0 + cn &&
                            !s->cfg.no_lazy_kt;
-    if (!lazy_tail && s->tpipe && s->speculate && split_days > 0 && cn >= split_days + (hinted ? 4 : 8)) {
+    if (s->kt_early) {
+      s->kt_early = false;
+    } else if (!lazy_tail && s->tpipe && s->speculate && split_days > 0 && cn >= split_days + (hinted ? 4 : 8)) {
       if (!s->stream2) {
         int lo = 0, hi = 0;
         (void)hipDeviceGetStreamPriorityRange(&lo, &hi);
@@ -1814,18 +1963,7 @@
     } else {
       PS_TRY(transform_kernels(s, c0, cn));
     }
-    auto day = [&](int d, bool with_refft) -> int {
-      PS_TRY(kernels_ready(s, d));
-      const cplx* B = s->Bhat.p + (size_t)(d - s->bhat_first) * s->Pf * s->ld;
-      double* rec = s->recs[PS_REC_CHAIN][d];
-      PS_TRY(conv_inv(s, B, s->Ahat.p, 1, rec, d, negval, stat_scale, s->krange.p + 2 * d));
-      if (with_refft) {
-        const bool defer = !s->cfg.no_defer_refft && !s->cfg.tpipe_split;
-        if (s->tpipe && defer && rs_colfull_alt_ok(s->rs_r2, s->rs_r3)) PS_TRY(refft_rows_if_flag(s, rec, d));
-        else PS_TRY(refft_if_flag(s, rec, s->Ahat.p, d));
-      }
-      return PS_OK;
-    };
+    auto day = [&](int d, bool with_refft) -> int { return run_day(s, d, with_refft, negval, stat_scale); };
     struct Win { int d0, w, ev; };
     std::deque<Win> q;
     (void)flagged_at;
@@ -1887,14 +2025,18 @@
       }
       if (q.empty()) break;
       const Win x = q.front();
+      if (defer_ok && q.size() == 1 && d >= c0 + cn) {
+        s->pend.on = true;
+        s->pend.first = first; s->pend.count = count;
+        s->pend.d0 = x.d0; s->pend.w = x.w; s->pend.ev = x.ev;
+        s->pend.negval = negval; s->pend.stat_scale = stat_scale;
+        s->pend.thr = flag_thr;
+        ++s->n_deferred;
+        return PS_OK;
+      }
       q.pop_front();
       PS_HIP(hipEventSynchronize(s->spec_ev[x.ev]));
-      int f = -1;
-      for (int i = 0; i < x.w && f < 0; ++i) {
-        double m;
-        __builtin_memcpy(&m, &s->hflags[x.d0 + i], sizeof(double));
-        if (m > flag_thr) f = x.d0 + i;
-      }
+      const int f = first_flagged_day(s, x.d0, x.w, flag_thr);
       if (f < 0) continue;
       q.clear();
       flagged_at = f;
@@ -1903,38 +2045,17 @@
         __builtin_memcpy(&mf, &s->hflags[f], sizeof(double));
         return auto_handover(s, first, f, first + count, negval, stat_scale, renorm, mf);
       }
-      s->refft_pending = nullptr;
       guided = false;
-      PS_TRY(fwd2d(s, s->recs[PS_REC_CHAIN][f], 0, s->N, map_plain(s->N, s->Pf), map_plain(s->N, s->Pf),
-                   s->Ahat.p, 1, nullptr));
-      if (d - f - 1 > 0)
-        PS_HIP(hipMemsetAsync(s->padmax.p + f + 1, 0, (size_t)(d - f - 1) * sizeof(unsigned long long), s->stream));
-      s->speculate = false;
+      PS_TRY(recover_from_flag(s, f, d));
       d = f + 1;
     }
   }
-  if (s->speculate && flagged_at < 0) s->noflag_hint = count;
-  if (!s->auto_exact && !s->speculate && count >= 2 && !s->cfg.no_flag_history) {
-    if (s->hhist_n < count) {
-      if (s->hist_ev) PS_HIP(hipEventSynchronize(s->hist_ev));
-      if (s->hhist) (void)hipHostFree(s->hhist);
-      s->hhist = nullptr;
-      s->hhist_n = 0;
-      PS_HIP(hipHostMalloc((void**)&s->hhist, (size_t)(count + 32) * sizeof(unsigned long long), hipHostMallocDefault));
-      s->hhist_n = count + 32;
-    }
-    if (!s->hist_ev) PS_HIP(hipEventCreateWithFlags(&s->hist_ev, hipEventDisableTiming));
-    PS_HIP(hipMemcpyAsync(s->hhist, s->padmax.p + first, (size_t)count * sizeof(unsigned long long), hipMemcpyDeviceToHost, s->stream));
-    PS_HIP(hipEventRecord(s->hist_ev, s->stream));
-    s->hist_first = first;
-    s->hist_count = count;
-  }
-  return PS_OK;
+  return finish_run(s, first, count, flagged_at >= 0);
 }
 
 extern "C" int ps_chain_stats(ps_solver* s, int first, int count, ps_day_stats* out) {
   if (!s || !out || first < 0 || count < 0 || first + count > s->nstat) return ps_fail(PS_ERR_BAD_ARG, "chain_stats: bad range");
-  PS_HIP(hipSetDevice(s->device));
+  PS_TRY(enter(s));
   if (s->auto_exact && s->auto_first >= 0 && first + count > s->auto_first) {
     int d = first;
     while (d < first + count) {
@@ -1973,7 +2094,7 @@
   if (!s->have_state) return ps_fail(PS_ERR_STATE, "fftconv2 before set_state");
   if (kshape < 1 || kshape % 2 == 0) return ps_fail(PS_ERR_BAD_SHAPE, "kernel shape %d must be odd (CalcSol.py:58)", kshape);
   if (kshape > s->Pf) return ps_fail(PS_ERR_BAD_SHAPE, "kernel shape %d larger than the pad %d", kshape, s->Pf);
-  PS_HIP(hipSetDevice(s->device));
+  PS_TRY(enter(s));
   PS_TRY(check_coo(row, col, nnz, kshape, "kernel"));
   PS_TRY(ensure_spectrum(s));
   PS_TRY(upload_coo(s, row, col, val, nnz));
@@ -1996,7 +2117,7 @@
   if (!s) return ps_fail(PS_ERR_BAD_ARG, "null solver");
   if (s->mode == PS_MODE_FOLD) return ps_fail(PS_ERR_UNSUPPORTED, "get_cursol: PS_MODE_FOLD offers the chain API only");
   if (!s->have_state) return ps_fail(PS_ERR_STATE, "get_cursol before set_state");
-  PS_HIP(hipSetDevice(s->device));
+  PS_TRY(enter(s));
   PS_TRY(ensure_record(s, PS_REC_CHAIN, 0));
   PS_TRY(ensure_temps(s, 1));
   PS_TRY(ensure_spectrum(s));
@@ -2017,7 +2138,7 @@
   if (!s->have_state) return ps_fail(PS_ERR_STATE, "back_solve before set_state");
   if (s->N % 2 == 0) return ps_fail(PS_ERR_BAD_SHAPE, "back_solve needs an odd domain (filters are N x N)");
   if (2 * (s->N / 2) + 1 > s->Pf) return ps_fail(PS_ERR_BAD_SHAPE, "filter larger than the pad");
-  PS_HIP(hipSetDevice(s->device));
+  PS_TRY(enter(s));
   const size_t spec = (size_t)s->Pf * s->ld;
   const int K = s->N, M = K / 2;
   PS_TRY(s->Chat.ensure(spec));
@@ -2099,7 +2220,7 @@
   const int ndays = s->nk - nfilt;
   if (!s->kernels_on_device || ndays < 0 || first + count > ndays)
     return ps_fail(PS_ERR_STATE, "run_release: days [%d,%d) + %d filters not uploaded (nk=%d)", first, first + count, nfilt, s->nk);
-  PS_HIP(hipSetDevice(s->device));
+  PS_TRY(enter(s));
   if (certified) *certified = 1;
   const size_t spec = (size_t)s->Pf * s->ld;
   const int per = nuse + 1;
@@ -2190,7 +2311,7 @@
   if (!s->have_state) return ps_fail(PS_ERR_STATE, "block_prefix before set_state");
   if (!s->kernels_on_device || first + count > s->nk)
     return ps_fail(PS_ERR_STATE, "block_prefix: days [%d,%d) not uploaded (nk=%d)", first, first + count, s->nk);
-  PS_HIP(hipSetDevice(s->device));
+  PS_TRY(enter(s));
   PS_TRY(resolve_refft(s));
   if (!s->spec_valid) set_pipeline(s, true);
   if (!s->tpipe) return ps_fail(PS_ERR_UNSUPPORTED, "block_prefix: the state's spectrum is held for the tiled pipeline; set the state again");
@@ -2222,7 +2343,7 @@
   if (!s || nprev < 0 || (nprev > 0 && !prev_totals)) return ps_fail(PS_ERR_BAD_ARG, "block_finish: bad arguments");
   if (s->blk_first != first || s->blk_count != count || count < 1)
     return ps_fail(PS_ERR_STATE, "block_finish: days [%d,%d) were not prepared by block_prefix", first, first + count);
-  PS_HIP(hipSetDevice(s->device));
+  PS_TRY(enter(s));
   const size_t spec = (size_t)s->Pf * s->ld;
   const int64_t n = (int64_t)s->H * s->Pf;
   PS_TRY(ensure_stats(s, std::max(4, s->nk)));
@@ -2285,7 +2406,7 @@
 extern "C" int ps_record_stats(ps_solver* s, int kind, int idx, double negval, double stat_scale,
                                int renorm, ps_day_stats* out) {
   if (!s || !out) return ps_fail(PS_ERR_BAD_ARG, "record_stats: bad arguments");
-  PS_HIP(hipSetDevice(s->device));
+  PS_TRY(enter(s));
   double* rec;
   PS_TRY(get_record(s, kind, idx, &rec));
   PS_TRY(ensure_stats(s, 4));
@@ -2307,7 +2428,7 @@
                         double post_scale, int32_t* row, int32_t* indptr, int32_t* col, double* val,
                         int64_t cap, int64_t* nnz_out) {
   if (!s) return ps_fail(PS_ERR_BAD_ARG, "null solver");
-  PS_HIP(hipSetDevice(s->device));
+  PS_TRY(enter(s));
   double* rec;
   PS_TRY(get_record(s, kind, idx, &rec));
   PS_TRY(ensure_stats(s, 4));
@@ -2363,7 +2484,7 @@
 
 extern "C" int ps_record_fetch_dense(ps_solver* s, int kind, int idx, double* out) {
   if (!s || !out) return ps_fail(PS_ERR_BAD_ARG, "fetch_dense: bad arguments");
-  PS_HIP(hipSetDevice(s->device));
+  PS_TRY(enter(s));
   double* rec;
   PS_TRY(get_record(s, kind, idx, &rec));
   PS_HIP(hipMemcpyAsync(out, rec, (size_t)s->N * s->N * sizeof(double), hipMemcpyDeviceToHost, s->stream));
@@ -2375,7 +2496,7 @@
                                 const int32_t* cols, double scale, double negval, double* out) {
   if (!s || n < 0 || (n > 0 && (!rows || !cols || !out))) return ps_fail(PS_ERR_BAD_ARG, "record_gather: bad arguments");
   if (n == 0) return PS_OK;
-  PS_HIP(hipSetDevice(s->device));
+  PS_TRY(enter(s));
   double* rec;
   PS_TRY(get_record(s, kind, idx, &rec));
   PS_TRY(check_coo(rows, cols, n, s->N, "gather point"));
@@ -2399,7 +2520,7 @@
   if (!s || nrec < 0 || n < 0 || (nrec > 0 && (!kind || !idx)) || (n > 0 && nrec > 0 && (!rows || !cols || !out)))
     return ps_fail(PS_ERR_BAD_ARG, "record_gather_multi: bad arguments");
   if (n == 0 || nrec == 0) return PS_OK;
-  PS_HIP(hipSetDevice(s->device));
+  PS_TRY(enter(s));
   std::vector<const double*> ptrs(nrec);
   for (int r = 0; r < nrec; ++r) {
     double* rec;
@@ -2426,7 +2547,7 @@
 
 extern "C" int ps_weighted_sum(ps_solver* s, int n, const int32_t* kind, const int32_t* idx, const double* w) {
   if (!s || n < 1 || !kind || !idx || !w) return ps_fail(PS_ERR_BAD_ARG, "weighted_sum: bad arguments");
-  PS_HIP(hipSetDevice(s->device));
+  PS_TRY(enter(s));
   std::vector<const double*> ptrs(n);
   for (int d = 0; d < n; ++d) {
     double* r;
@@ -2450,7 +2571,7 @@
   if (!s || !out) return ps_fail(PS_ERR_BAD_ARG, "get_spectrum: bad arguments");
   if (s->mode == PS_MODE_FOLD) return ps_fail(PS_ERR_UNSUPPORTED, "get_spectrum: PS_MODE_FOLD offers the chain API only");
   if (!s->have_state) return ps_fail(PS_ERR_STATE, "get_spectrum before set_state");
-  PS_HIP(hipSetDevice(s->device));
+  PS_TRY(enter(s));
   if (s->tpipe) {
     if (s->spec_valid) return ps_fail(PS_ERR_UNSUPPORTED, "get_spectrum: the state is held column-major (full-column pipeline)");
     set_pipeline(s, false);
@@ -2471,7 +2592,7 @@
 extern "C" int ps_solver_set_spectrum(ps_solver* s, const double* in) {
   if (!s || !in) return ps_fail(PS_ERR_BAD_ARG, "set_spectrum: bad arguments");
   if (s->mode == PS_MODE_FOLD) return ps_fail(PS_ERR_UNSUPPORTED, "set_spectrum: PS_MODE_FOLD offers the chain API only");
-  PS_HIP(hipSetDevice(s->device));
+  PS_TRY(enter(s));
   set_pipeline(s, false);
   const size_t full = (size_t)s->Pf * s->Pf;
   DevBuf<cplx> tmp;
@@ -2491,6 +2612,7 @@
 
 extern "C" int ps_solver_set_option(ps_solver* s, const char* key, double value) {
   if (!s || !key) return ps_fail(PS_ERR_BAD_ARG, "set_option: bad arguments");
+  PS_TRY(enter(s));
   const int rc = ps_config_set(&s->cfg, key, value, true);
   if (rc == -1) return ps_fail(PS_ERR_BAD_ARG, "set_option: unknown option %s", key);
   if (rc == -2) return ps_fail(PS_ERR_STATE, "set_option: %s takes effect when a solver is created", key);
@@ -2526,7 +2648,7 @@
 
 extern "C" int ps_prof_enable(ps_solver* s, int on) {
   if (!s) return ps_fail(PS_ERR_BAD_ARG, "null solver");
-  PS_HIP(hipSetDevice(s->device));
+  PS_TRY(enter(s));
   PS_TRY(prof_drain(s));
   for (int i = 0; i < PS_PROF_NCLS; ++i) { s->prof_ms[i] = 0; s->prof_cnt[i] = 0; s->prof_seen[i] = 0; s->prof_days[i] = 0; }
   s->prof_on = on != 0;
@@ -2538,7 +2660,7 @@
 
 extern "C" int ps_prof_read(ps_solver* s, int ncls, double* total_ms, int64_t* count) {
   if (!s || !total_ms || !count) return ps_fail(PS_ERR_BAD_ARG, "prof_read: bad arguments");
-  PS_HIP(hipSetDevice(s->device));
+  PS_TRY(enter(s));
   PS_TRY(prof_drain(s));
   for (int i = 0; i < ncls; ++i) {
     total_ms[i] = i < PS_PROF_NCLS ? s->prof_ms[i] : 0.0;
@@ -2549,7 +2671,7 @@
 
 extern "C" int ps_prof_read_days(ps_solver* s, int ncls, int64_t* days) {
   if (!s || !days) return ps_fail(PS_ERR_BAD_ARG, "prof_read_days: bad arguments");
-  PS_HIP(hipSetDevice(s->device));
+  PS_TRY(enter(s));
   PS_TRY(prof_drain(s));
   for (int i = 0; i < ncls; ++i) days[i] = i < PS_PROF_NCLS ? s->prof_days[i] : 0;
   return PS_OK;
@@ -2557,7 +2679,7 @@
 
 extern "C" int ps_prof_read_launches(ps_solver* s, int ncls, int64_t* launches) {
   if (!s || !launches) return ps_fail(PS_ERR_BAD_ARG, "prof_read_launches: bad arguments");
-  PS_HIP(hipSetDevice(s->device));
+  PS_TRY(enter(s));
   PS_TRY(prof_drain(s));
   for (int i = 0; i < ncls; ++i)
     launches[i] = i >= PS_PROF_NCLS ? 0 : (i >= PS_PROF_COL_INV_A2 ? s->prof_cnt[i] : s->prof_seen[i]);
@@ -2582,6 +2704,18 @@
 
 extern "C" int ps_solver_pipeline(ps_solver* s) { return s && s->tpipe ? 1 : 0; }
 
+extern "C" int ps_solver_deferred_info(ps_solver* s, int* pending, int64_t* counts) {
+  if (!s) return ps_fail(PS_ERR_BAD_ARG, "null solver");
+  if (pending) *pending = s->pend.on ? 1 : 0;
+  if (counts) {
+    counts[0] = s->n_deferred;
+    counts[1] = s->n_late_flags;
+    counts[2] = s->n_staged_early;
+    counts[3] = s->n_staged_uploads;
+  }
+  return PS_OK;
+}
+
 extern "C" int ps_solver_auto_route(ps_solver* s, int first, int count, int32_t* owner) {
   if (!s || !owner || first < 0 || count < 0) return ps_fail(PS_ERR_BAD_ARG, "auto_route: bad arguments");
   for (int i = 0; i < count; ++i) {
@@ -2609,7 +2743,7 @@
 
 int ps_solver_record_internal(ps_solver* s, int kind, int idx, int want_stats, PsRecordView* out) {
   if (!s || !out) return ps_fail(PS_ERR_BAD_ARG, "record view: bad arguments");
-  PS_HIP(hipSetDevice(s->device));
+  PS_TRY(enter(s));
   double* rec;
   PS_TRY(get_record(s, kind, idx, &rec));
   out->rec = rec;
diff --git a/parasitoids_amd/hip_lib.py b/parasitoids_amd/hip_lib.py
--- a/parasitoids_amd/hip_lib.py
+++ b/parasitoids_amd/hip_lib.py
@@ -319,6 +319,13 @@
     def full_column(self):
         return bool(self._lib.ps_solver_pipeline(self._h))
 
+    def deferred_info(self):
+        pending = C.c_int32(0)
+        cnt = np.zeros(4, dtype=np.int64)
+        L.check(self._lib.ps_solver_deferred_info(self._h, C.byref(pending), L.p_i64(cnt)))
+        return {'pending': bool(pending.value), 'deferred': int(cnt[0]), 'late_flags': int(cnt[1]),
+                'staged_early': int(cnt[2]), 'staged_uploads': int(cnt[3])}
+
     def auto_info(self):
         a, b = C.c_int32(-1), C.c_int32(0)
         L.check(self._lib.ps_solver_auto_info(self._h, C.byref(a), C.byref(b)))
```

New measurement: 4366 grid-days/s, median of 6. 1.01x the previous value.
